# manasakani/DeviceKMC

Hardware: AMD Instinct MI355X
Metric: KMC steps/sec (higher is better)
Workload: dtype f64

## Files before the change

devicekmc_amd/csrc/common.h:

```cpp
#pragma once
#include <hip/hip_runtime.h>
#include <stdint.h>
#include <stdio.h>
#include <string.h>
#include <math.h>
#include "../../include/devicekmc_hip.h"
#include "../../include/devicekmc_hip_debug.h"

enum { DEFECT = 0, OXYGEN_DEFECT = 1, VACANCY = 2, O_EL = 3, Hf_EL = 4, Ni_EL = 5, Ti_EL = 6, Pt_EL = 7, N_EL = 8, NULL_ELEMENT = 9 };
enum { EV_GEN = 0, EV_REC = 1, EV_VDIFF = 2, EV_IDIFF = 3, EV_NULL = 4 };

#define DKMC_KB 8.617333262e-5
#define DKMC_Q 1.60217663e-19
#define DKMC_HBAR 1.054571817e-34
#define DKMC_MAX_LAYERS 5
#define WAVE 64

struct MetalSet { int n; const int *e; };

__device__ __forceinline__ bool is_metal(int el, const MetalSet &ms)
{
    bool r = false;
    for (int t = 0; t < ms.n; ++t) r |= (ms.e[t] == el);
    return r;
}

__device__ __forceinline__ double site_dist(double x1, double y1, double z1, double x2, double y2, double z2,
                                            double laty, double latz, int pbc)
{
    if (pbc) {
        double dx = x1 - x2;
        double fy = (y1 - y2) / laty; fy -= round(fy);
        double fz = (z1 - z2) / latz; fz -= round(fz);
        double dy = fy * laty, dz = fz * latz;
        return sqrt(dx * dx + dy * dy + dz * dz);
    }
    double dx = x2 - x1, dy = y2 - y1, dz = z2 - z1;
    return sqrt(dx * dx + dy * dy + dz * dz);
}

__device__ __forceinline__ double v_solve(double r, int charge, double sigma, double k)
{
    return (double)charge * erfc(r / (sigma * sqrt(2.0))) * k * DKMC_Q / r;
}

template <int OFF> __device__ __forceinline__ int xor_lane_i(int x)
{
    static_assert(OFF == 1 || OFF == 2 || OFF == 4 || OFF == 8 || OFF == 16 || OFF == 32, "xor_lane: power of two below the wave size");
    if constexpr (OFF == 1) return __builtin_amdgcn_update_dpp(0, x, 0xB1, 0xf, 0xf, false);
    else if constexpr (OFF == 2) return __builtin_amdgcn_update_dpp(0, x, 0x4E, 0xf, 0xf, false);
    else if constexpr (OFF == 4) {
        const int t = __builtin_amdgcn_update_dpp(0, x, 0x104, 0xf, 0x5, false);
        return __builtin_amdgcn_update_dpp(t, x, 0x114, 0xf, 0xa, false);
    }
    else if constexpr (OFF == 8) return __builtin_amdgcn_update_dpp(0, x, 0x128, 0xf, 0xf, false);
    else return __shfl_xor(x, OFF, WAVE);
}
template <int OFF> __device__ __forceinline__ double xor_lane(double x)
{
    if constexpr (OFF >= 16) return __shfl_xor(x, OFF, WAVE);
    else return __hiloint2double(xor_lane_i<OFF>(__double2hiint(x)), xor_lane_i<OFF>(__double2loint(x)));
}
template <int W> __device__ __forceinline__ double group_sum(double v)
{
    if constexpr (W >= 64) v += xor_lane<32>(v);
    if constexpr (W >= 32) v += xor_lane<16>(v);
    if constexpr (W >= 16) v += xor_lane<8>(v);
    if constexpr (W >= 8) v += xor_lane<4>(v);
    if constexpr (W >= 4) v += xor_lane<2>(v);
    if constexpr (W >= 2) v += xor_lane<1>(v);
    return v;
}
template <int W> __device__ __forceinline__ int group_sum_i(int v)
{
    if constexpr (W >= 64) v += xor_lane_i<32>(v);
    if constexpr (W >= 32) v += xor_lane_i<16>(v);
    if constexpr (W >= 16) v += xor_lane_i<8>(v);
    if constexpr (W >= 8) v += xor_lane_i<4>(v);
    if constexpr (W >= 4) v += xor_lane_i<2>(v);
    if constexpr (W >= 2) v += xor_lane_i<1>(v);
    return v;
}

__device__ __forceinline__ double wave_sum(double v) { return group_sum<WAVE>(v); }
__device__ __forceinline__ double wave_sum_all(double v) { return group_sum<WAVE>(v); }
__device__ __forceinline__ int wave_sum_all_i(int v) { return group_sum_i<WAVE>(v); }
template <class T> __device__ __forceinline__ T wave_min(T v)
{
#pragma unroll
    for (int off = 32; off > 0; off >>= 1) { const T t = __shfl_xor(v, off, WAVE); v = t < v ? t : v; }
    return v;
}
template <class T> __device__ __forceinline__ T wave_max(T v)
{
#pragma unroll
    for (int off = 32; off > 0; off >>= 1) { const T t = __shfl_xor(v, off, WAVE); v = t > v ? t : v; }
    return v;
}
__device__ __forceinline__ double wave_scan_incl(double v, int lane)
{
#pragma unroll
    for (int off = 1; off < WAVE; off <<= 1) { double t = __shfl_up(v, off, WAVE); if (lane >= off) v += t; }
    return v;
}
__device__ __forceinline__ int wave_scan_incl_i(int v, int lane)
{
#pragma unroll
    for (int off = 1; off < WAVE; off <<= 1) { int t = __shfl_up(v, off, WAVE); if (lane >= off) v += t; }
    return v;
}

template <int NT>
__device__ __forceinline__ double block_sum_all(double v, double *red)
{
    const int lane = threadIdx.x & 63, w = threadIdx.x >> 6;
    v = wave_sum(v);
    __syncthreads();
    if (lane == 0) red[w] = v;
    __syncthreads();
    double s = 0.0;
#pragma unroll
    for (int i = 0; i < NT / 64; ++i) s += red[i];
    return s;
}

__host__ __device__ __forceinline__ unsigned long long dbl_key(double v)
{
    const unsigned long long b = __builtin_bit_cast(unsigned long long, v);
    return (b >> 63) ? ~b : (b | 0x8000000000000000ull);
}
__host__ __device__ __forceinline__ double key_dbl(unsigned long long k)
{
    return __builtin_bit_cast(double, (k >> 63) ? (k & 0x7fffffffffffffffull) : ~k);
}
__device__ __forceinline__ int ld_agent(const int *p) { return __hip_atomic_load(p, __ATOMIC_RELAXED, __HIP_MEMORY_SCOPE_AGENT); }
__device__ __forceinline__ void st_agent(int *p, int v) { __hip_atomic_store(p, v, __ATOMIC_RELAXED, __HIP_MEMORY_SCOPE_AGENT); }
__device__ __forceinline__ int seed_bits(int i, int N, int n_left, int n_right) { return (i < n_left ? 1 : 0) | (i >= N - n_right ? 2 : 0); }
inline void clamp_seeds(int N, int &n_left, int &n_right)
{
    n_left = n_left < 0 ? 0 : (n_left > N ? N : n_left);
    n_right = n_right < 0 ? 0 : (n_right > N ? N : n_right);
}

struct KBlocked {
    int m, R, nb, total, maxwin, maxints;
    long long winsum;
    int *perm;
    int *pcol;
    int4 *blk;
    int form = 1;
    int maxseg = 0;
    long long segsum = 0;
    int4 *seg = nullptr;
    int word_bytes = 4;
};
constexpr int X_POLY_DEFAULT = 8;
struct Engine {
    hipStream_t stream = nullptr;
    int device = 0;
    double cg_tol = 1e-6;
    int current_warm_start = 1;
    int profiling = 0;
    int cb_edge_domain = 0;
    long long tcache_budget = -1;
    double pair_cut = 6.5;
    int pair_form = 0;
    int k_blocked = 1;
    int k_blocked_large = 0;
    int k_window_word_bytes = 4;
    int x_aux = 2;
    int x_slab = 1;
    int k_slab = 1;
    int x_poly = X_POLY_DEFAULT;
    int x_poly_auto = 1;
    int x_poly_rows[2] = {0, 0};
    int x_poly_form = 2;
    int x_poly1_degree = 0;
    int x_poly_form_used = 0, x_poly_products = 0;
    int x_slab_poly = 0;
    int x_aux_warm = 0;
    int x_items_kc = 0;
    int x_apply_form = 0;
    int x_tile_f32 = 1;
    double x_tile_drop = 0.0;
    int x_tile_drop_unit = 0;
    int x_tile_drop_auto = 1;
    long long x_tile_drop_gate = 0;
    double x_tile_drop_used = 0.0;
    int xtl_census_form = 1;
    int x_static_tiles = 2;
    int x_static_gate = 0;
    int x_static_nM = -1;
    int x_static_verify = 0;
    int x_tile_f32_fail_once = 0;
    int x_fold_form = 1;
    int x_fold_poison = 0;
    int x_nmul_form = 1;
    int x_nmul_lane_bytes = 16;
    int x_nmul_window = 2;
    int x_nmul_window_cap = 76 * 1024;
    int x_nmul_window_block = 320;
    int x_block = 16;
    int x_format = 1;
    int current_map = 0;
    int x_iter_hint = 0;
    int event_temperature = 0;
    int event_census = 0;
    int event_census_valid = 0;
    double event_census_info[16] = {0};
    dkmc_stats stats{};
    char err[512] = {0};
    int err_code = 0;
    double E_gen[DKMC_MAX_LAYERS] = {0}, E_rec[DKMC_MAX_LAYERS] = {0}, E_Vdiff[DKMC_MAX_LAYERS] = {0}, E_Odiff[DKMC_MAX_LAYERS] = {0};
    int num_layers = 0;
    static const int NBUF = 192;
    void *buf[NBUF] = {nullptr};
    size_t bufsz[NBUF] = {0};
};

constexpr int X_STATIC_GATE = 32768;
static inline int x_static_rule(int ns, int gate_override) { return ns >= (gate_override > 0 ? gate_override : X_STATIC_GATE) ? 1 : 0; }
Engine &eng();
int dkmc_fail(int code, const char *what, const char *file, int line);
void *scratch(int slot, size_t bytes);
void *scratch_try(int slot, size_t bytes);
static inline int grid_blocks(long long work, int per_block, int cap)
{
    long long b = (work + per_block - 1) / per_block;
    if (b < 1) b = 1;
    if (b > cap) b = cap;
    return (int)b;
}
inline MetalSet load_metals(const int *d_metals, int num_metals) { MetalSet ms; ms.n = num_metals; ms.e = d_metals; return ms; }

#define HIPCHK(x) do { hipError_t e__ = (x); if (e__ != hipSuccess) return dkmc_fail((int)e__, hipGetErrorString(e__), __FILE__, __LINE__); } while (0)
#define KCHK() do { hipError_t e__ = hipGetLastError(); if (e__ != hipSuccess) return dkmc_fail((int)e__, hipGetErrorString(e__), __FILE__, __LINE__); } while (0)

enum {
    S_CG_S = 0, S_CG_R, S_CG_P, S_CG_T, S_CG_PART, S_CG_CTRL, S_CG_RUNS, S_CG_REM, S_CG_NRUNS, S_CG_PS, S_CG_SEGOFF, S_CG_SEGS, S_CG_SEGPART, S_CG_XCHG, S_CG_PARTS,
    S_K_DATA, S_K_RHS,
    S_PW_LIST, S_PW_CNT, S_PW_CELLS, S_PW_PERM, S_PW_LIST2,
    S_EV_PROB, S_EV_ROWSUM, S_EV_G2, S_EV_G3, S_EV_CTRL, S_EV_UNI, S_EV_LOG,
    S_SCAN_TMP, S_SCAN_TMP2, S_SCAN_OFF64, S_SCAN_INTILE,
    S_AT_FLAG, S_AT_SITE, S_AT_OFSITE, S_AT_NEIGH,
    S_X_ROWPTR, S_X_COL, S_X_DATA, S_X_DATA2, S_X_CNT, S_X_SLIST, S_X_SCB, S_X_SFLAG, S_X_RHS, S_X_SRANK,
    S_P_IMACRO, S_HEAT, S_HEAT_A, S_HEAT_B, S_HEAT_Y,
    S_MISC0, S_MISC1, S_MISC2, S_MISC3,
    S_XT_DPOS, S_XT_SNODE_D, S_XT_SNODE_I, S_XT_CMASK, S_XT_ISTILE, S_XT_NSUBC, S_XT_TOFF, S_XT_SOFF, S_XT_TILES, S_XT_NITEMW, S_XT_WRANGE,
    S_XT_ITEMS, S_XT_SPLIT, S_XT_TVAL, S_XT_TVAL32, S_XT_ROWPART, S_XT_COLPART, S_XT_CNT, S_XT_Q,
    S_XT_T_NITEMW, S_XT_T_ITEMS, S_XT_T_SPLIT, S_XT_T_COLPART, S_XT_T_MISC,
    S_XTB_PANELS, S_XTB_QS, S_XTB_ROWPART, S_XTB_COLPART, S_XTB_GRAM, S_XTB_SMALL, S_XTB_XI,
    S_XTB_SLAB_BOX, S_XTB_SLAB_TAB, S_XTB_SLAB_OWNER, S_XTB_SLAB_LISTS, S_XTB_SLAB_SDST, S_XTB_SLAB_FLAG, S_XTB_SLAB_RLISTS, S_XTB_SLAB_GX, S_XTB_SLAB_S1, S_XTB_SLAB_S3, S_XTB_SLAB_R3,
    S_XTB_EMU_Y, S_XTB_EMU_CTRL, S_XTB_YPANEL, S_XTB_PRE_V, S_XTB_PRE_W1, S_XTB_PRE_W2, S_XTB_PRE_Z, S_XTB_PRE_U,
    S_XTB_NPACK_CNT, S_XTB_NPACK_OFF, S_XTB_NPACK_COL, S_XTB_NPACK_W,
    S_XTL_CELLS, S_XTL_TFLAG, S_XTL_TVAL32, S_XTL_TILES, S_XTL_WRANGE, S_XTL_NITEMW, S_XTL_ITEMS, S_XTL_SPLIT,
    S_XT_WLIST, S_XTL_WLIST,
    S_KS_TAB, S_KS_OWNER, S_KS_LISTS, S_KS_FLAG, S_KS_BOX, S_KS_RLISTS, S_KS_XA, S_KS_XB, S_KS_SEND, S_KS_RECV, S_KS_YBUF, S_KS_EMU,
    S_XTB_TEST_RP, S_XTB_TEST_CI, S_XTB_TEST_VAL, S_XTB_TEST_SC, S_XTB_TEST_NSR, S_XTB_TEST_LIST, S_XTB_TEST_IN, S_XTB_TEST_ADD, S_XTB_TEST_OUT,
    S_XTB_TEST_W1, S_XTB_TEST_W2, S_XTB_TEST_QS, S_XTB_TEST_CTRL, S_XTB_TEST_NPCNT, S_XTB_TEST_NPOFF, S_XTB_TEST_NPCOL, S_XTB_TEST_NPW,
    S_P_CMAP,
    S_XTB_ALG_PANELS, S_XTB_ALG_INTS, S_XTB_ALG_GRAM, S_XTB_ALG_QS, S_XTB_ALG_CTRL,
    S_CL_PARENT, S_CL_SUMS, S_CL_POS, S_CL_TABLE, S_CL_CTRL,
    S_EV_NBAD, S_EV_CENSUS_PART, S_EV_CENSUS_INFO,
    S_GAP_SITE, S_GAP_CTRL, S_GAP_CELLS, S_GAP_SORTED, S_GAP_NODES, S_GAP_EDGES,
    S_PT_HOP, S_PT_PRED, S_PT_ROWS, S_PT_CTRL,
    S_TR_HASH, S_TR_COMP, S_TR_SITE, S_TR_ROWS, S_TR_CTRL,
    S_CUT_SITE, S_CUT_TABLE, S_CUT_ROWS, S_CUT_CTRL,
    S_FL_SITE, S_FL_ROWS, S_FL_CTRL,
    S_NSLOTS
};
static_assert(S_NSLOTS <= Engine::NBUF, "scratch slots");

int comm_attached();
int comm_nranks();
int comm_rank();
int comm_allgather_f64(double *buf, size_t count);
int comm_alltoallv_f64(const double *sendbuf, double *recvbuf, const long long *cnt);
int comm_allreduce_sum_f64(double *buf, size_t count);
int comm_agree(int local_rc, const char *what);
int comm_agree_count();
int comm_peer_ready(size_t count);
double *comm_peer_slots(int parity);
void comm_peer_drop();
int comm_peer_exchange(int parity, size_t count, int *ctrl_done, int *ctrl_aborted, int *ctrl_timeout, int stamp);
int comm_bcast0_f64(double *buf, size_t count);

int ev_census_enqueue(int N, int nn, const int *neigh, const int *element, const double *temperature, const double *ev_prob, double **d_info16);

int dkmc_exclusive_scan_i32(const int *d_in, int *d_out, int n, int *d_total);
int dkmc_exclusive_scan_i32_i64(const int *d_in, long long *d_out, int n, long long *d_total);
```

devicekmc_amd/csrc/engine.hip:

```cpp
#include "common.h"
#include <stdlib.h>

int events_upload_layers();
void xstate_reset(const void *key);

static Engine g_engine;
Engine &eng() { return g_engine; }

int dkmc_fail(int code, const char *what, const char *file, int line)
{
    Engine &e = eng();
    snprintf(e.err, sizeof(e.err), "%s (%s:%d)", what, file, line);
    e.err_code = code ? code : -1;
    fprintf(stderr, "devicekmc_hip: %s\n", e.err);
    return e.err_code;
}

void *scratch(int slot, size_t bytes)
{
    Engine &e = eng();
    if (bytes == 0) bytes = 16;
    if (e.bufsz[slot] < bytes) {
        if (e.buf[slot]) { (void)hipStreamSynchronize(e.stream); (void)hipFree(e.buf[slot]); }
        size_t want = bytes + bytes / 8 + 256;
        hipError_t rc = hipMalloc(&e.buf[slot], want);
        if (rc != hipSuccess) {
            char msg[160]; snprintf(msg, sizeof(msg), "hipMalloc(%zu bytes) failed in scratch(slot %d): %s", want, slot, hipGetErrorString(rc));
            dkmc_fail(2, msg, __FILE__, __LINE__); e.buf[slot] = nullptr; e.bufsz[slot] = 0; return nullptr;
        }
        e.bufsz[slot] = want;
    }
    return e.buf[slot];
}

void *scratch_try(int slot, size_t bytes)
{
    Engine &e = eng();
    if (bytes == 0) bytes = 16;
    if (e.bufsz[slot] < bytes) {
        if (e.buf[slot]) { (void)hipStreamSynchronize(e.stream); (void)hipFree(e.buf[slot]); }
        e.buf[slot] = nullptr; e.bufsz[slot] = 0;
        const size_t want = bytes + bytes / 8 + 256;
        if (hipMalloc(&e.buf[slot], want) != hipSuccess) { (void)hipGetLastError(); e.buf[slot] = nullptr; return nullptr; }
        e.bufsz[slot] = want;
    }
    return e.buf[slot];
}

extern "C" {

const char *dkmc_last_error(void) { return eng().err; }
void dkmc_clear_error(void) { eng().err[0] = 0; eng().err_code = 0; }
const dkmc_stats *dkmc_get_stats(void) { return &eng().stats; }
void dkmc_set_cg_tolerance(double tol) { eng().cg_tol = tol; }
void dkmc_set_current_warm_start(int mode) { eng().current_warm_start = mode; }
int dkmc_get_current_warm_start(void) { return eng().current_warm_start; }
void dkmc_set_profiling(int on) { eng().profiling = on; }
void dkmc_set_x_format(int tiled) { eng().x_format = tiled ? 1 : 0; }
int dkmc_get_x_format(void) { return eng().x_format; }
void dkmc_set_current_map(int on) { eng().current_map = on ? 1 : 0; }
int dkmc_get_current_map(void) { return eng().current_map; }
void dkmc_set_tcache_budget(long long bytes) { eng().tcache_budget = bytes; }
void dkmc_set_pair_cutoff(double x_cut) { eng().pair_cut = x_cut > 0.0 ? x_cut : 0.0; }
void dkmc_set_pair_form(int form) { eng().pair_form = form == 1 ? 1 : 0; }
int dkmc_get_pair_form(void) { return eng().pair_form; }
void dkmc_set_k_slab(int on) { eng().k_slab = on ? 1 : 0; }
int dkmc_get_k_slab(void) { return eng().k_slab; }
void dkmc_set_x_aux_warm(int on) { eng().x_aux_warm = on ? 1 : 0; }
int dkmc_get_x_aux_warm(void) { return eng().x_aux_warm; }
void dkmc_set_x_items(int kc) { eng().x_items_kc = kc > 0 ? (kc < 256 ? kc : 256) : 0; }
void dkmc_set_x_poly(int degree) { eng().x_poly = degree < 0 ? 0 : (degree > 16 ? 16 : degree); eng().x_poly_auto = 0; }
int dkmc_get_x_poly(void) { return eng().x_poly; }
void dkmc_set_x_poly_auto(int on) { Engine &e = eng(); e.x_poly_auto = on ? 1 : 0; if (on && e.x_poly <= 0) e.x_poly = X_POLY_DEFAULT; }
int dkmc_get_x_poly_auto(void) { return eng().x_poly_auto; }
void dkmc_set_x_poly_form(int form) { eng().x_poly_form = form == 1 ? 1 : (form == 2 ? 2 : 0); }
int dkmc_get_x_poly_form(void) { return eng().x_poly_form; }
int dkmc_get_x_poly_form_used(void) { return eng().x_poly_form_used; }
int dkmc_get_x_poly_products(void) { return eng().x_poly_products; }
void dkmc_debug_set_x_poly1_degree(int n) { eng().x_poly1_degree = n < 0 ? 0 : (n > 20 ? 20 : n); }
void dkmc_set_x_poly_auto_rows(int n0, int n1) { Engine &e = eng(); e.x_poly_rows[0] = n0 > 0 ? n0 : 0; e.x_poly_rows[1] = n1 > e.x_poly_rows[0] ? n1 : e.x_poly_rows[0]; }
void dkmc_set_x_apply_form(int form) { eng().x_apply_form = form == 1 ? 1 : 0; }
int dkmc_get_x_apply_form(void) { return eng().x_apply_form; }
void dkmc_set_x_tile_f32(int mode) { eng().x_tile_f32 = mode == 0 ? 0 : 1; }
int dkmc_get_x_tile_f32(void) { return eng().x_tile_f32; }
void dkmc_set_x_tile_drop(double theta) { eng().x_tile_drop = theta > 0.0 ? (theta > 1e-4 ? 1e-4 : theta) : 0.0; }
double dkmc_get_x_tile_drop(void) { return eng().x_tile_drop; }
void dkmc_set_x_tile_drop_unit(int unit) { eng().x_tile_drop_unit = unit == 1 ? 1 : 0; }
int dkmc_get_x_tile_drop_unit(void) { return eng().x_tile_drop_unit; }
void dkmc_set_x_tile_drop_auto(int on) { eng().x_tile_drop_auto = on ? 1 : 0; }
int dkmc_get_x_tile_drop_auto(void) { return eng().x_tile_drop_auto; }
void dkmc_set_x_tile_drop_auto_subblocks(long long gate) { eng().x_tile_drop_gate = gate > 0 ? gate : 0; }
double dkmc_get_x_tile_drop_used(void) { return eng().x_tile_drop_used; }
void dkmc_debug_fail_true_residual_once(void) { eng().x_tile_f32_fail_once = 1; }
void dkmc_set_x_fold_form(int form) { eng().x_fold_form = form == 0 ? 0 : 1; }
int dkmc_get_x_fold_form(void) { return eng().x_fold_form; }
void dkmc_debug_poison_fold_cells(int on) { eng().x_fold_poison = on ? 1 : 0; }
void dkmc_set_x_static_tiles(int mode) { eng().x_static_tiles = (mode == 0 || mode == 1) ? mode : 2; }
int dkmc_get_x_static_tiles(void) { return eng().x_static_tiles; }
int dkmc_debug_x_static_verify(int on) { const int was = eng().x_static_verify; eng().x_static_verify = on ? 1 : 0; return was; }
void dkmc_debug_set_x_static_gate(int members) { eng().x_static_gate = members > 0 ? members : 0; }
int dkmc_x_static_rule(int members) { return x_static_rule(members, eng().x_static_gate); }
int dkmc_x_static_strips(int n_metals) { return n_metals > 0 ? n_metals / 256 : 0; }
void dkmc_set_x_nmul_form(int form) { eng().x_nmul_form = form == 0 ? 0 : 1; }
int dkmc_get_x_nmul_form(void) { return eng().x_nmul_form; }
void dkmc_set_x_nmul_lane_bytes(int bytes) { eng().x_nmul_lane_bytes = bytes == 8 ? 8 : 16; }
int dkmc_get_x_nmul_lane_bytes(void) { return eng().x_nmul_lane_bytes; }
void dkmc_set_x_nmul_window(int mode) { eng().x_nmul_window = (mode == 0 || mode == 1) ? mode : 2; }
int dkmc_get_x_nmul_window(void) { return eng().x_nmul_window; }
void dkmc_debug_set_x_nmul_window(int cap_bytes, int block_rows)
{
    Engine &e = eng();
    e.x_nmul_window_cap = cap_bytes < 0 ? 76 * 1024 : (cap_bytes > 76 * 1024 ? 76 * 1024 : cap_bytes);
    e.x_nmul_window_block = (block_rows >= 16 && block_rows <= 1024 && block_rows % 16 == 0) ? block_rows : 320;
}
void dkmc_set_x_slab(int on) { eng().x_slab = on ? 1 : 0; }
int dkmc_get_x_slab(void) { return eng().x_slab; }
void dkmc_set_x_slab_poly(int on) { eng().x_slab_poly = on ? 1 : 0; }
int dkmc_get_x_slab_poly(void) { return eng().x_slab_poly; }
void dkmc_set_x_block(int s) { eng().x_block = s < 1 ? 1 : (s > 16 ? 16 : s); }
int dkmc_get_x_block(void) { return eng().x_block; }
void dkmc_set_x_aux(int mode) { eng().x_aux = mode < 0 ? 0 : (mode > 3 ? 2 : mode); }
int dkmc_get_x_aux(void) { return eng().x_aux; }
void dkmc_set_k_blocked(int on) { eng().k_blocked = on ? 1 : 0; }
int dkmc_get_k_blocked(void) { return eng().k_blocked; }
void dkmc_set_k_blocked_large(int on) { eng().k_blocked_large = on ? 1 : 0; }
int dkmc_get_k_blocked_large(void) { return eng().k_blocked_large; }
void dkmc_set_k_window_word_bytes(int bytes) { eng().k_window_word_bytes = bytes == 2 ? 2 : 4; }
int dkmc_get_k_window_word_bytes(void) { return eng().k_window_word_bytes; }
void dkmc_set_cb_edge_domain(int atoms_only) { eng().cb_edge_domain = atoms_only ? 1 : 0; }

int dkmc_get_gpu_info(char *gpu_string, int capacity, int dev)
{
    hipDeviceProp_t prop;
    HIPCHK(hipSetDevice(dev));
    HIPCHK(hipGetDeviceProperties(&prop, dev));
    snprintf(gpu_string, capacity, "%s", prop.name);
    return 0;
}

int dkmc_set_gpu(int dev) { HIPCHK(hipSetDevice(dev)); eng().device = dev; return 0; }
int dkmc_set_stream(void *s) { eng().stream = (hipStream_t)s; return 0; }
int dkmc_synchronize(void) { HIPCHK(hipStreamSynchronize(eng().stream)); return 0; }

int dkmc_copy_to_const_memory(const double *E_gen, const double *E_rec, const double *E_Vdiff, const double *E_Odiff, int nl)
{
    Engine &e = eng();
    if (nl > DKMC_MAX_LAYERS) return dkmc_fail(3, "more than 5 layers (MAX_NUM_LAYERS, kmc_events.cu:7)", __FILE__, __LINE__);
    e.num_layers = nl;
    for (int i = 0; i < nl; ++i) { e.E_gen[i] = E_gen[i]; e.E_rec[i] = E_rec[i]; e.E_Vdiff[i] = E_Vdiff[i]; e.E_Odiff[i] = E_Odiff[i]; }
    return events_upload_layers();
}

#define ALLOC(field, n, T) HIPCHK(hipMalloc((void **)&buf->field, (size_t)(n) * sizeof(T)))
int dkmc_gpubuf_create(dkmc_gpubuf *buf, int N, int N_atom, int nn, int nmt,
                       const int *h_layer, const double *hx, const double *hy, const double *hz,
                       const int *h_neigh, const int *h_metals, double freq, double sigma, double k, const double *h_lattice)
{
    memset(buf, 0, sizeof(*buf));
    buf->N_ = N; buf->N_atom_ = N_atom; buf->nn_ = nn; buf->num_metal_types_ = nmt;
    ALLOC(site_layer, N, int); ALLOC(site_element, N, int); ALLOC(metal_types, nmt > 0 ? nmt : 1, int);
    ALLOC(site_x, N, double); ALLOC(site_y, N, double); ALLOC(site_z, N, double);
    ALLOC(site_power, N, double); ALLOC(site_CB_edge, N, double);
    ALLOC(site_potential_boundary, N, double); ALLOC(site_potential_charge, N, double);
    ALLOC(site_temperature, N, double); ALLOC(site_charge, N, int);
    ALLOC(neigh_idx, (size_t)N * nn, int);
    ALLOC(T_bg, 1, double); ALLOC(sigma, 1, double); ALLOC(k, 1, double); ALLOC(lattice, 3, double); ALLOC(freq, 1, double);
    ALLOC(atom_element, N, int); ALLOC(atom_x, N, double); ALLOC(atom_y, N, double); ALLOC(atom_z, N, double);
    ALLOC(atom_power, N, double); ALLOC(atom_CB_edge, N, double); ALLOC(atom_charge, N, int);
    ALLOC(atom_virtual_potentials, N_atom + 2, double);
    HIPCHK(hipMemset(buf->atom_virtual_potentials, 0, (size_t)(N_atom + 2) * sizeof(double)));
    HIPCHK(hipMemset(buf->site_power, 0, (size_t)N * sizeof(double)));
    HIPCHK(hipMemcpy(buf->site_layer, h_layer, (size_t)N * sizeof(int), hipMemcpyHostToDevice));
    HIPCHK(hipMemcpy(buf->site_x, hx, (size_t)N * sizeof(double), hipMemcpyHostToDevice));
    HIPCHK(hipMemcpy(buf->site_y, hy, (size_t)N * sizeof(double), hipMemcpyHostToDevice));
    HIPCHK(hipMemcpy(buf->site_z, hz, (size_t)N * sizeof(double), hipMemcpyHostToDevice));
    if (nmt > 0) HIPCHK(hipMemcpy(buf->metal_types, h_metals, (size_t)nmt * sizeof(int), hipMemcpyHostToDevice));
    HIPCHK(hipMemcpy(buf->sigma, &sigma, sizeof(double), hipMemcpyHostToDevice));
    HIPCHK(hipMemcpy(buf->k, &k, sizeof(double), hipMemcpyHostToDevice));
    HIPCHK(hipMemcpy(buf->freq, &freq, sizeof(double), hipMemcpyHostToDevice));
    HIPCHK(hipMemcpy(buf->lattice, h_lattice, 3 * sizeof(double), hipMemcpyHostToDevice));
    HIPCHK(hipMemcpy(buf->neigh_idx, h_neigh, (size_t)N * nn * sizeof(int), hipMemcpyHostToDevice));
    return 0;
}
#undef ALLOC

int dkmc_gpubuf_free(dkmc_gpubuf *b)
{
    xstate_reset(b->site_x);
    void *ptrs[] = { b->site_charge, b->site_power, b->site_potential_boundary, b->site_potential_charge, b->site_temperature,
                     b->site_CB_edge, b->T_bg, b->atom_power, b->atom_CB_edge, b->atom_virtual_potentials, b->atom_charge,
                     b->site_element, b->atom_element, b->site_x, b->site_y, b->site_z, b->atom_x, b->atom_y, b->atom_z,
                     b->metal_types, b->sigma, b->k, b->lattice, b->freq, b->neigh_idx, b->site_layer,
                     b->Device_row_ptr_d, b->Device_col_indices_d, b->contact_left_row_ptr, b->contact_left_col_indices,
                     b->contact_right_row_ptr, b->contact_right_col_indices };
    for (void *p : ptrs) if (p) (void)hipFree(p);
    memset(b, 0, sizeof(*b));
    return 0;
}

int dkmc_gpubuf_sync_host_to_gpu(dkmc_gpubuf *b, const int *el, const int *q, const double *pw, const double *cb,
                                 const double *pb, const double *pc, const double *T, const double *acb, double T_bg)
{
    const size_t N = b->N_;
    HIPCHK(hipStreamSynchronize(eng().stream));
    HIPCHK(hipMemcpy(b->site_element, el, N * sizeof(int), hipMemcpyHostToDevice));
    HIPCHK(hipMemcpy(b->site_charge, q, N * sizeof(int), hipMemcpyHostToDevice));
    HIPCHK(hipMemcpy(b->site_power, pw, N * sizeof(double), hipMemcpyHostToDevice));
    HIPCHK(hipMemcpy(b->site_CB_edge, cb, N * sizeof(double), hipMemcpyHostToDevice));
    HIPCHK(hipMemcpy(b->site_potential_boundary, pb, N * sizeof(double), hipMemcpyHostToDevice));
    HIPCHK(hipMemcpy(b->site_potential_charge, pc, N * sizeof(double), hipMemcpyHostToDevice));
    HIPCHK(hipMemcpy(b->site_temperature, T, N * sizeof(double), hipMemcpyHostToDevice));
    if (acb) HIPCHK(hipMemcpy(b->atom_CB_edge, acb, (size_t)b->N_atom_ * sizeof(double), hipMemcpyHostToDevice));
    HIPCHK(hipMemcpy(b->T_bg, &T_bg, sizeof(double), hipMemcpyHostToDevice));
    return 0;
}

int dkmc_gpubuf_sync_gpu_to_host(const dkmc_gpubuf *b, int *el, int *q, double *pw, double *cb,
                                 double *pb, double *pc, double *T, double *acb, double *T_bg)
{
    const size_t N = b->N_;
    HIPCHK(hipStreamSynchronize(eng().stream));
    HIPCHK(hipMemcpy(el, b->site_element, N * sizeof(int), hipMemcpyDeviceToHost));
    HIPCHK(hipMemcpy(q, b->site_charge, N * sizeof(int), hipMemcpyDeviceToHost));
    HIPCHK(hipMemcpy(pw, b->site_power, N * sizeof(double), hipMemcpyDeviceToHost));
    HIPCHK(hipMemcpy(cb, b->site_CB_edge, N * sizeof(double), hipMemcpyDeviceToHost));
    HIPCHK(hipMemcpy(pb, b->site_potential_boundary, N * sizeof(double), hipMemcpyDeviceToHost));
    HIPCHK(hipMemcpy(pc, b->site_potential_charge, N * sizeof(double), hipMemcpyDeviceToHost));
    HIPCHK(hipMemcpy(T, b->site_temperature, N * sizeof(double), hipMemcpyDeviceToHost));
    if (acb) HIPCHK(hipMemcpy(acb, b->atom_CB_edge, (size_t)b->N_atom_ * sizeof(double), hipMemcpyDeviceToHost));
    HIPCHK(hipMemcpy(T_bg, b->T_bg, sizeof(double), hipMemcpyDeviceToHost));
    return 0;
// ... 23 lines not shown
```

devicekmc_amd/csrc/xtb.hip:

```cpp
#include "xtiles.h"
#include "slab.h"
#include <hip/hip_ext.h>
#include <algorithm>
#include <functional>
#include <type_traits>
#include <vector>

#define XB_SP 16
#define XB_MAXPOLY 16
#define XB_MAXPOLY1 20
#define XB_DSPLIT 8
#define XB_NG 6
typedef double dbl4 __attribute__((ext_vector_type(4)));
#define XB_MFMA(a, b, c) __builtin_amdgcn_mfma_f64_16x16x4f64((a), (b), (c), 0, 0, 0)
#define XB_MFMA4(a, b, c) __builtin_amdgcn_mfma_f64_4x4x4f64((a), (b), (c), 0, 0, 0)

__device__ __forceinline__ double xtb_aux(int row, int col)
{
    unsigned long long h = (unsigned long long)row * 0x9E3779B97F4A7C15ull + (unsigned long long)col * 0xC2B2AE3D27D4EB4Full + 12345ull;
    h ^= h >> 29; h *= 0xBF58476D1CE4E5B9ull; h ^= h >> 32;
    return (double)(h >> 11) * (1.0 / 4503599627370496.0) - 1.0;
}
struct XbAux { double lo[3], hi[3]; int k[16][3]; unsigned long long mm[6]; int hs, pad_; };
__device__ __forceinline__ double xtb_rhs(const double *__restrict__ b, int row, int v, int s, const XbAux *__restrict__ aux = nullptr,
// ... 854 lines not shown
    double gdiag = (threadIdx.x < 16 && (int)threadIdx.x < s && diag_ok) ? Gg[threadIdx.x][threadIdx.x] : 1.0;
    XB_WSYNC();
    const bool cholg = xtb_chol(Gg, s);
    const bool okg = diag_ok;
    if (!cholg) {
#pragma unroll
        for (int u = 0; u < 4; ++u) { const int e = (int)threadIdx.x + 64 * u, i = e >> 4, j = e & 15; Gg[i][j] = (i == j) ? 1.0 : 0.0; }
        XB_WSYNC();
        if (threadIdx.x < 16) Gg[threadIdx.x][threadIdx.x] = sqrt(gdiag);
        XB_WSYNC();
    }
    if (threadIdx.x < 16) {
        const int jj = threadIdx.x;
        double w[16];
#pragma unroll
        for (int r = 15; r >= 0; --r) {
            double a = (r == jj) ? 1.0 : 0.0;
#pragma unroll
            for (int p = r + 1; p < 16; ++p) a -= Gg[p][r] * w[p];
            w[r] = a / Gg[r][r];
        }
#pragma unroll
        for (int r = 0; r < 16; ++r) Wm[r][jj] = (r < s && jj < s && okg) ? w[r] : 0.0;
    }
    XB_WSYNC();
    xtb_mm(Vm, Bm, Wm, false, 1.0, nullptr, 0.0);
    xtb_mm(Tm, Cm, Wm, false, -1.0, nullptr, 0.0);
#pragma unroll
    for (int u = 0; u < 4; ++u) {
        const int e = (int)threadIdx.x + 64 * u, i = e >> 4, j = e & 15;
        mats[0 * 256 + e] = Cm[i][j]; mats[1 * 256 + e] = -Wm[i][j]; mats[2 * 256 + e] = Vm[i][j]; mats[3 * 256 + e] = Tm[i][j];
    }
    if (threadIdx.x == 0) {
        ctrl->rr[(it + 1) & 1] = rr_new; ctrl->rr[it & 1] = rr_new;
        ctrl->iters = it + 1;
        if (!okg) ctrl->pad[0] = 2;
        else if (!cholg) ctrl->pad[1] += 1;
        if (stop || !okg) { if (ctrl->sharded) ctrl->done_local = 1; else ctrl->done = it + 2; }
    }
}

__global__ __launch_bounds__(XT_NT) void k_xtb_step(int m, int it, const double *__restrict__ mats, double *__restrict__ y0, double *__restrict__ R,
                                                    double *__restrict__ P, const double *__restrict__ T, const double *__restrict__ sc,
                                                    const int *__restrict__ nsrank, double *__restrict__ QS, const XCtrl *ctrl,
                                                    const int *__restrict__ rowlist = nullptr, double *__restrict__ Ypanel = nullptr)
{
    __shared__ int sdone;
    if (threadIdx.x == 0) { const int d = ctrl->done; sdone = d != 0 && it + 1 >= d; }
    __syncthreads();
    if (sdone) return;
    const int lane = threadIdx.x & 63, a = lane & 15, b = lane >> 4;
    const int wv = threadIdx.x >> 6;
    double cB[4], m1B[4], m2B[4], m3B[4], c0[4];
#pragma unroll
    for (int kk = 0; kk < 4; ++kk) {
        const int o = (4 * kk + b) * 16 + a;
        cB[kk] = mats[o]; m1B[kk] = mats[256 + o]; m2B[kk] = mats[512 + o]; m3B[kk] = mats[768 + o];
        c0[kk] = mats[(4 * kk + b) * 16];
    }
    const int ngroups = (m + 15) / 16;
    for (int g = (int)blockIdx.x * 4 + wv; g < ngroups; g += (int)gridDim.x * 4) {
        const int row0 = 16 * g;
        double pa[4], ta[4], ra[4];
        const bool oka = row0 + a < m;
        const int rowa = oka ? (rowlist ? rowlist[row0 + a] : row0 + a) : 0;
        const size_t oa = (size_t)rowa * XB_SP + b;
#pragma unroll
        for (int kk = 0; kk < 4; ++kk) { pa[kk] = oka ? P[oa + 4 * kk] : 0.0; ta[kk] = oka ? T[oa + 4 * kk] : 0.0; ra[kk] = oka ? R[oa + 4 * kk] : 0.0; }
        dbl4 rN, pN = (dbl4)(0.0), yN = (dbl4)(0.0);
        const double yold = (b == 0 && oka) ? y0[rowa] : 0.0;
        int rowu[4];
#pragma unroll
        for (int u = 0; u < 4; ++u) {
            const int li = row0 + b + 4 * u;
            rowu[u] = li < m ? (rowlist ? rowlist[li] : li) : -1;
            rN[u] = rowu[u] >= 0 ? R[(size_t)rowu[u] * XB_SP + a] : 0.0;
            if (Ypanel) yN[u] = rowu[u] >= 0 ? Ypanel[(size_t)rowu[u] * XB_SP + a] : 0.0;
        }
        double yacc = (pa[0] * c0[0] + pa[1] * c0[1]) + (pa[2] * c0[2] + pa[3] * c0[3]);
        yacc += __shfl_xor(yacc, 16, WAVE); yacc += __shfl_xor(yacc, 32, WAVE);
        if (b == 0 && oka) y0[rowa] = yold + yacc;
#pragma unroll
        for (int kk = 0; kk < 4; ++kk) {
            rN = XB_MFMA(ta[kk], cB[kk], rN);
            pN = XB_MFMA(ra[kk], m1B[kk], pN); pN = XB_MFMA(ta[kk], m3B[kk], pN); pN = XB_MFMA(pa[kk], m2B[kk], pN);
            if (Ypanel) yN = XB_MFMA(pa[kk], cB[kk], yN);
        }
#pragma unroll
        for (int u = 0; u < 4; ++u) {
            const int row = rowu[u];
            if (row >= 0) {
                const size_t o = (size_t)row * XB_SP + a;
                R[o] = rN[u]; P[o] = pN[u];
                if (Ypanel) Ypanel[o] = yN[u];
                const int sr = nsrank[row];
                if (sr >= 0) QS[xtb_qs_pos(sr, a)] = sc[row] * pN[u];
            }
        }
    }
}
__global__ __launch_bounds__(XT_NT) void k_xtb_gram1(int m, const double *__restrict__ Pt, const double *__restrict__ Pi, const double *__restrict__ Q,
                                                     const double *__restrict__ U, const double *__restrict__ Rt, const double *__restrict__ Z,
                                                     double *__restrict__ gpart, const XCtrl *ctrl)
{
    __shared__ double lg[4][XB_NG / 2][4][64];
    if (ctrl->done) return;
    const int v = threadIdx.x & 15, wv = threadIdx.x >> 6, lane = threadIdx.x & 63;
    dbl4 G[XB_NG];
#pragma unroll
    for (int g = 0; g < XB_NG; ++g) G[g] = (dbl4)(0.0);
    const int chunk = ((m + (int)gridDim.x - 1) / (int)gridDim.x + 3) & ~3;
    const long long i0l = (long long)blockIdx.x * chunk;
    const int i0 = (int)(i0l < m ? i0l : m), i1 = (int)(i0l + chunk < m ? i0l + chunk : m);
    for (int r0 = i0 + 4 * wv; r0 < i1; r0 += 64) {
        double pv[4], iv[4], qv[4], uv[4], rv[4], zv[4]; bool in[4];
#pragma unroll
        for (int u = 0; u < 4; ++u) {
            const int row = r0 + 16 * u + (lane >> 4);
            in[u] = row < i1;
            const size_t o = (size_t)(in[u] ? row : i0) * XB_SP + v;
            pv[u] = Pt[o]; iv[u] = Pi[o]; qv[u] = Q[o]; uv[u] = U[o]; rv[u] = Rt[o]; zv[u] = Z[o];
        }
#pragma unroll
        for (int u = 0; u < 4; ++u) {
            if (r0 + 16 * u >= i1) break;
            const double p_ = in[u] ? pv[u] : 0.0, i_ = in[u] ? iv[u] : 0.0, q_ = in[u] ? qv[u] : 0.0, u_ = in[u] ? uv[u] : 0.0, r_ = in[u] ? rv[u] : 0.0,
                         z_ = in[u] ? zv[u] : 0.0;
            G[0] = XB_MFMA(p_, q_, G[0]); G[1] = XB_MFMA(p_, r_, G[1]); G[2] = XB_MFMA(q_, z_, G[2]);
            G[3] = XB_MFMA(q_, u_, G[3]); G[4] = XB_MFMA(r_, z_, G[4]); G[5] = XB_MFMA(p_, i_, G[5]);
        }
    }
#pragma unroll
    for (int h = 0; h < 2; ++h) {
        __syncthreads();
#pragma unroll
        for (int g = 0; g < XB_NG / 2; ++g)
#pragma unroll
            for (int u = 0; u < 4; ++u) lg[wv][g][u][lane] = G[h * (XB_NG / 2) + g][u];
        __syncthreads();
        for (int e = threadIdx.x; e < (XB_NG / 2) * 256; e += XT_NT) {
            const int g = e >> 8, x = e & 255, u = x >> 6, l = x & 63;
            double a = (lg[0][g][u][l] + lg[1][g][u][l]) + (lg[2][g][u][l] + lg[3][g][u][l]);
            if (h == 1) {
                const int xt = ((x & 15) << 4) | (x >> 4), ut = xt >> 6, lt = xt & 63;
                a = 0.5 * (a + ((lg[0][g][ut][lt] + lg[1][g][ut][lt]) + (lg[2][g][ut][lt] + lg[3][g][ut][lt])));
            }
            gpart[(size_t)blockIdx.x * (XB_NG * 256) + h * (XB_NG / 2) * 256 + e] = a;
        }
    }
}
__global__ __launch_bounds__(XT_NT) void k_xtb_step1(int m, int it, const double *__restrict__ mats, double *__restrict__ y0, double *__restrict__ Rt,
                                                     double *__restrict__ Z, double *__restrict__ Pt, double *__restrict__ Pi, const double *__restrict__ Q,
                                                     const double *__restrict__ U, const double *__restrict__ sc, const int *__restrict__ nsrank,
                                                     double *__restrict__ QS, const XCtrl *ctrl)
{
    __shared__ int sdone;
    if (threadIdx.x == 0) { const int d = ctrl->done; sdone = d != 0 && it + 1 >= d; }
    __syncthreads();
    if (sdone) return;
    const int lane = threadIdx.x & 63, a = lane & 15, b = lane >> 4;
    const int wv = threadIdx.x >> 6;
    double cB[4], m1B[4], m2B[4], m3B[4], c0[4];
#pragma unroll
    for (int kk = 0; kk < 4; ++kk) {
        const int o = (4 * kk + b) * 16 + a;
        cB[kk] = mats[o]; m1B[kk] = mats[256 + o]; m2B[kk] = mats[512 + o]; m3B[kk] = mats[768 + o];
        c0[kk] = mats[(4 * kk + b) * 16];
    }
    const int ngroups = (m + 15) / 16;
    for (int g = (int)blockIdx.x * 4 + wv; g < ngroups; g += (int)gridDim.x * 4) {
        const int row0 = 16 * g;
        double pa[4], ia[4], qa[4], ua[4], ra[4], za[4];
        const bool oka = row0 + a < m;
        const int rowa = oka ? row0 + a : 0;
        const size_t oa = (size_t)rowa * XB_SP + b;
#pragma unroll
        for (int kk = 0; kk < 4; ++kk) {
            pa[kk] = oka ? Pt[oa + 4 * kk] : 0.0; ia[kk] = oka ? Pi[oa + 4 * kk] : 0.0; qa[kk] = oka ? Q[oa + 4 * kk] : 0.0;
            ua[kk] = oka ? U[oa + 4 * kk] : 0.0; ra[kk] = oka ? Rt[oa + 4 * kk] : 0.0; za[kk] = oka ? Z[oa + 4 * kk] : 0.0;
        }
        dbl4 rN, zN, pN = (dbl4)(0.0), iN = (dbl4)(0.0);
        const double yold = (b == 0 && oka) ? y0[rowa] : 0.0;
        int rowu[4];
#pragma unroll
        for (int u = 0; u < 4; ++u) {
            const int li = row0 + b + 4 * u;
            rowu[u] = li < m ? li : -1;
            rN[u] = rowu[u] >= 0 ? Rt[(size_t)rowu[u] * XB_SP + a] : 0.0;
            zN[u] = rowu[u] >= 0 ? Z[(size_t)rowu[u] * XB_SP + a] : 0.0;
        }
        double yacc = (pa[0] * c0[0] + pa[1] * c0[1]) + (pa[2] * c0[2] + pa[3] * c0[3]);
        yacc += __shfl_xor(yacc, 16, WAVE); yacc += __shfl_xor(yacc, 32, WAVE);
        if (b == 0 && oka) y0[rowa] = yold + yacc;
#pragma unroll
        for (int kk = 0; kk < 4; ++kk) {
            rN = XB_MFMA(qa[kk], cB[kk], rN); zN = XB_MFMA(ua[kk], cB[kk], zN);
            pN = XB_MFMA(za[kk], m1B[kk], pN); pN = XB_MFMA(ua[kk], m3B[kk], pN); pN = XB_MFMA(pa[kk], m2B[kk], pN);
            iN = XB_MFMA(ra[kk], m1B[kk], iN); iN = XB_MFMA(qa[kk], m3B[kk], iN); iN = XB_MFMA(ia[kk], m2B[kk], iN);
        }
#pragma unroll
        for (int u = 0; u < 4; ++u) {
            const int row = rowu[u];
            if (row >= 0) {
                const size_t o = (size_t)row * XB_SP + a;
                Rt[o] = rN[u]; Z[o] = zN[u]; Pt[o] = pN[u]; Pi[o] = iN[u];
                const int sr = nsrank[row];
                if (sr >= 0) QS[xtb_qs_pos(sr, a)] = sc[row] * pN[u];
            }
        }
    }
}
__global__ void k_xtb_init(int m, const double *__restrict__ y, const double *__restrict__ sc, const int *__restrict__ nsrank,
                           double *__restrict__ y0, double *__restrict__ P, double *__restrict__ QS,
                           const double *__restrict__ yaux = nullptr, int hs = 16, int s = 16, double *__restrict__ Ypanel = nullptr)
{
    const int i = blockIdx.x * blockDim.x + threadIdx.x;
    if (i >= m * XB_SP) return;
    const int row = i >> 4, v = i & 15;
    double yv = 0.0;
    if (v == 0) yv = y[row];
    else if (yaux && v >= hs && v < s) yv = yaux[i] / sc[row];
    P[i] = yv;
    if (Ypanel) Ypanel[i] = yv;
    if (v == 0) y0[row] = yv;
    const int sr = nsrank[row];
    if (sr >= 0) QS[xtb_qs_pos(sr, v)] = sc[row] * yv;
}
__global__ void k_xtb_yaux_out(int n, const int *__restrict__ rowlist, const double *__restrict__ Ypanel, const double *__restrict__ sc, double *__restrict__ yaux)
{
    const int i = blockIdx.x * blockDim.x + threadIdx.x;
    if (i >= n * XB_SP) return;
    const int row = rowlist ? rowlist[i >> 4] : (i >> 4), v = i & 15;
    yaux[(size_t)row * XB_SP + v] = Ypanel[(size_t)row * XB_SP + v] * sc[row];
}
__global__ void k_xtb_zero(long long n, double *__restrict__ p)
{
    const long long i = (long long)blockIdx.x * blockDim.x + threadIdx.x;
    if (i < n) p[i] = 0.0;
}

static SideStream g_xb_side;

int g_xtb_fault_iter = -1;

static int xtb_aux_split(int mode, double tol2, bool warm, int s)
{
    if (mode == 0) return 1;
    if (mode == 1 || mode == 3) return 16;
    if (!(tol2 >= 1e-16)) return 1;
    return warm ? std::max(1, s / 2) : 16;
}
static int xtb_box_modes(XbAux *d, XbAux h0, const XtbArgs &A, int x_only, hipStream_t st)
{
    for (int k = 0; k < 3; ++k) { h0.mm[2 * k] = ~0ull; h0.mm[2 * k + 1] = 0ull; }
    HIPCHK(hipMemcpyAsync(d, &h0, sizeof(XbAux), hipMemcpyHostToDevice, st));
    hipLaunchKernelGGL(k_xtb_box, dim3(std::min((A.m - 2 + 255) / 256, 256)), dim3(256), 0, st, A.m - 2, A.ax, A.ay, A.az, d);
    hipLaunchKernelGGL(k_xtb_modes, dim3(1), dim3(512), 0, st, d, x_only);
    return 0;
}
static int xtb_aux_setup(const XtbArgs &A, XbAux **aux, int *hs)
{
    Engine &e = eng();
    *hs = xtb_aux_split(e.x_aux, A.tol2, A.yaux != nullptr, A.s);
    *aux = nullptr;
    if (A.ax && A.ay && A.az && A.m > 2 && *hs > 1) {
        *aux = (XbAux *)scratch(S_XTB_XI, sizeof(XbAux));
        if (!*aux) return e.err_code;
        XbAux h0{};
        h0.hs = *hs;
        if (int rc = xtb_box_modes(*aux, h0, A, e.x_aux == 3 ? 1 : 0, e.stream)) return rc;
    }
    e.stats.xb_aux = *aux ? (*hs >= A.s ? 1 : 2) : 0;
    return 0;
}
struct XbApplyArgs { int n; const XItem *items; const XTile *tiles; int sub_base; const double *tval; const double *QS; int nW; double *rowpartB, *colpartB; const XCtrl *ctrl; const float *tval32 = nullptr; };
template <int NTL, int NG, int V>
static void xtb_apply_v(const XbApplyArgs &a, hipStream_t st, hipEvent_t e0, hipEvent_t e1)
{
    hipExtLaunchKernelGGL((k_xtb_apply<NTL, NG, V>), dim3((a.n + 3) / 4), dim3(XT_NT), 0, st, e0, e1, 0, a.n, a.items, a.tiles, a.sub_base, a.tval, a.QS, a.nW,
                          a.rowpartB, a.colpartB, a.ctrl);
}
template <int NTL, int NG>
static void xtb_apply_f32(const XbApplyArgs &a, hipStream_t st, hipEvent_t e0, hipEvent_t e1)
{
    hipExtLaunchKernelGGL((k_xtb_apply<NTL, NG, 0, float>), dim3((a.n + 3) / 4), dim3(XT_NT), 0, st, e0, e1, 0, a.n, a.items, a.tiles, a.sub_base, a.tval32, a.QS, a.nW,
                          a.rowpartB, a.colpartB, a.ctrl);
}
template <int NTL, int NG>
static void xtb_apply_ng(const XbApplyArgs &a, int variant, hipStream_t st, hipEvent_t e0, hipEvent_t e1)
{
#ifdef DKMC_MEASURE_VARIANTS
#define XB_V(v_) if (variant == (v_)) return xtb_apply_v<NTL, NG, v_>(a, st, e0, e1);
    if constexpr (NTL == 1 && NG == 2) { XB_V(1) XB_V(2) }
    if constexpr (NTL == 1 && NG == 4) { XB_V(1) XB_V(2) XB_V(3) XB_V(4) XB_V(7) XB_V(10) XB_V(12) }
#undef XB_V
#else
    (void)variant;
#endif
    if (a.tval32) return xtb_apply_f32<NTL, NG>(a, st, e0, e1);
    if (eng().x_apply_form == 1) xtb_apply_v<NTL, NG, 8>(a, st, e0, e1);
    else xtb_apply_v<NTL, NG, 0>(a, st, e0, e1);
}
static void xtb_apply(const XbApplyArgs &a, bool ntl, int so, int variant, hipStream_t st, hipEvent_t e0 = nullptr, hipEvent_t e1 = nullptr)
{
    static void (*const ng[2][4])(const XbApplyArgs &, int, hipStream_t, hipEvent_t, hipEvent_t) = {
        {xtb_apply_ng<0, 1>, xtb_apply_ng<0, 2>, xtb_apply_ng<0, 3>, xtb_apply_ng<0, 4>}, {xtb_apply_ng<1, 1>, xtb_apply_ng<1, 2>, xtb_apply_ng<1, 3>, xtb_apply_ng<1, 4>}};
    ng[ntl ? 1 : 0][so == 4 ? 0 : (so == 8 ? 1 : (so == 12 ? 2 : 3))](a, variant, st, e0, e1);
}
template <int SH, int NF, class... Args>
static void xtb_rows_launch(bool init, int ng, hipStream_t st, hipEvent_t e0, hipEvent_t e1, Args... a)
{
    if (init) hipLaunchKernelGGL((k_xtb_rows<1, SH, NF>), dim3(ng), dim3(XT_NT), 0, st, a...);
    else hipExtLaunchKernelGGL((k_xtb_rows<0, SH, NF>), dim3(ng), dim3(XT_NT), 0, st, e0, e1, 0, a...);
}
static const char *const XTB_NO_CONVERGENCE = "block-CG: no convergence after 200000 iterations";
static int xtb_finish(const XCtrl &h, bool hint, bool again, bool prof, int *iters_out, double *rr_out)
{
    Engine &e = eng();
    if (hint) e.x_iter_hint = h.iters;
    if (iters_out) *iters_out = h.iters;
    if (rr_out) *rr_out = h.rr[h.iters & 1];
    if (prof) g_loop_events.to_stats(e.stats, false);
    if (h.pad[0]) return DKMC_XTB_BREAKDOWN;
    return again ? DKMC_XTB_AGAIN : 0;
}
static int xtb_cg_body(const XtbArgs &A, int *iters_out, double *rr_out, bool *peer_used, const XbNPack *np, bool f32, XLive *lv);
static int xtb_cg_slab(const XtbArgs &A, int nr, int me0, const XShare *emu_shares, int time_rank, int *iters_out, double *rr_out);
template <class Body>
static int xtb_reenter(int rc, double rr0, int *iters_out, double *rr_out, Body body)
{
    for (int round = 1; rc == DKMC_XTB_AGAIN && round < 6; ++round) {
        int it2 = 0; double rr1 = 0.0;
        rc = body(&it2, &rr1);
        if (iters_out) *iters_out += it2;
        if (rc == DKMC_XTB_AGAIN && !(rr1 < 0.25 * rr0)) rc = 0;
        rr0 = rr1;
    }
    if (rc == DKMC_XTB_AGAIN) rc = 0;
    if (rr_out) *rr_out = rr0;
    return rc;
}
int xtb_cg(const XtbArgs &A, int *iters_out, double *rr_out)
{
    bool peer_used = false;
    double rr0 = 0.0;
    if (A.sharded && eng().x_slab && comm_nranks() > 1 && comm_nranks() <= XS_MAXR && A.ay && A.az) {
        const int nr = comm_nranks(), me = comm_rank();
        const int rc = xtb_cg_slab(A, nr, me, nullptr, -1, iters_out, &rr0);
        return xtb_reenter(rc, rr0, iters_out, rr_out, [&](int *it, double *rr) { return xtb_cg_slab(A, nr, me, nullptr, -1, it, rr); });
    }
    XbNPack npk{};
    const bool packed = !A.sharded && A.m > 2 && A.ns > 0 && eng().x_poly > 0 && eng().x_nmul_form == 1;
    if (packed) { if (int rcp = xtb_npack(A, A.m, nullptr, scratch, 0, &npk)) return rcp; }
    const XbNPack *np = packed ? &npk : nullptr;
    Engine &e = eng();
    const bool f32 = e.x_tile_f32 != 0 && A.tval32 != nullptr && !A.sharded && A.m > 2 && A.ns > 0 && e.x_poly > 0 && A.tol2 >= 1e-16;
    if (f32) e.stats.x_tile_stream = 1; else if (e.stats.x_tile_stream == 1) e.stats.x_tile_stream = 0;
    e.stats.x_tile_f64_rounds = f32 ? 0 : 1;
    XLive *lv = nullptr;
    const double theta = e.x_tile_drop > 0.0 ? e.x_tile_drop : (e.x_tile_drop_auto && A.warm ? xtl_drop_rule(A.stored_subblocks, e.x_tile_drop_gate) : 0.0);
    e.x_tile_drop_used = 0.0;
    if (f32 && theta > 0.0 && A.item_n > 0 && A.tiles == g_xb.tiles && A.tval32 == g_xb.tval32) {
        if (int rcl = xt_live_build(theta, e.x_tile_drop_unit, A.sS, &g_xlive)) return rcl;
        if (g_xlive.state == 1) { lv = &g_xlive; e.x_tile_drop_used = theta; }
    }
    int rc = xtb_cg_body(A, iters_out, &rr0, &peer_used, np, f32, lv);
    rc = xtb_reenter(rc, rr0, iters_out, rr_out, [&](int *it, double *rr) { ++e.stats.x_tile_f64_rounds; return xtb_cg_body(A, it, rr, &peer_used, np, false, nullptr); });
    if (rc != 0 && rc != DKMC_XTB_BREAKDOWN && peer_used) comm_peer_drop();
    return rc;
}
static int xtb_cg_body(const XtbArgs &A, int *iters_out, double *rr_out, bool *peer_used, const XbNPack *np, bool f32, XLive *lv)
{
    Engine &e = eng(); hipStream_t st = e.stream;
    const int m = A.m, s = A.s, so = 4 * ((s + 3) / 4);
    const size_t pan = (size_t)m * XB_SP;
    const long long ncell = (long long)A.nK * A.nW;
    const int ng = std::max(128, std::min(A.nK, 4096));
    double *panels = (double *)scratch(S_XTB_PANELS, (pan * 3 + m + 16) * 8);
    double *QS = (double *)scratch(S_XTB_QS, (size_t)A.ns_pad * XB_SP * 8);
    double *rowpartB = (double *)scratch(S_XTB_ROWPART, (size_t)(ncell + 1) * XT_R * so * 8);
    const int nrec = std::max(A.nrecords, lv ? lv->nrecords : 0);
    double *colpartB = (double *)scratch(S_XTB_COLPART, (size_t)(nrec + 1) * XT_C * so * 8);
    double *gpart = (double *)scratch(S_XTB_GRAM, (size_t)ng * XB_NG * 256 * 8);
    double *small = (double *)scratch(S_XTB_SMALL, (size_t)(4 * 256 + 2 * XB_DSPLIT * XB_SP + XB_NG * 256) * 8);
    if (!panels || !QS || !rowpartB || !colpartB || !gpart || !small) return e.err_code;
    double *R = panels, *P = panels + pan, *T = panels + 2 * pan, *y0 = panels + 3 * pan;
    double *mats = small, *drvpart = small + 4 * 256, *gfin = drvpart + 2 * XB_DSPLIT * XB_SP;
    const int pd = xtb_poly_degree(e, A);
    e.stats.xb_poly_used = pd;
    const bool one = pd > 0 && xtb_poly_one(e);
    const int pn = one ? xtb_poly1_degree(e, pd) : pd;
    e.x_poly_form_used = one ? 1 : 0; e.x_poly_products = one ? pn : 2 * pd;
    double *Vp = nullptr, *W1 = nullptr, *W2 = nullptr, *Zp = nullptr, *bz = nullptr, *Up = nullptr;
    if (pd > 0) {
        Vp = (double *)scratch(S_XTB_PRE_V, (pan + m + 16) * 8); W1 = (double *)scratch(S_XTB_PRE_W1, pan * 8); W2 = (double *)scratch(S_XTB_PRE_W2, pan * 8);
        Zp = (double *)scratch(S_XTB_PRE_Z, pan * 8);
        if (!Vp || !W1 || !W2 || !Zp) return e.err_code;
        bz = Vp + pan;
        HIPCHK(hipMemsetAsync(bz, 0, (size_t)(m + 16) * 8, st));
        if (one) {
            Up = (double *)scratch(S_XTB_PRE_U, pan * 8);
            if (!Up) return e.err_code;
            HIPCHK(hipMemsetAsync(Vp, 0, pan * 8, st));
            HIPCHK(hipMemsetAsync(Up, 0, pan * 8, st));
        }
    }
    double pc[XB_MAXPOLY1 + 1] = {1.0}, qmin = 1.0;
    if (one) xtb_poly1_coeffs(pn, pc, &qmin); else xtb_poly_coeffs(pd, pc);
    const double tol2_loop = one ? A.tol2 * qmin : (pd > 0 ? A.tol2 / 2.25 : A.tol2);
    HIPCHK(hipMemsetAsync(QS, 0, (size_t)A.ns_pad * XB_SP * 8, st));
    const bool listf = e.x_fold_form == 1 && pd > 0 && !A.sharded && A.wlist != nullptr && (!lv || lv->wlist != nullptr);
    const int so1 = listf ? 4 : so;
    if (!listf) HIPCHK(hipMemsetAsync(rowpartB, 0, (size_t)(ncell + 1) * XT_R * so * 8, st));
    else if (e.x_fold_poison) HIPCHK(hipMemsetAsync(rowpartB, 0xff, (size_t)(ncell + 1) * XT_R * so * 8, st));
    HIPCHK(hipMemsetAsync(colpartB, 0, (size_t)(nrec + 1) * XT_C * so * 8, st));
    HIPCHK(hipMemsetAsync(A.ctrl, 0, sizeof(XCtrl), st));
    const bool sharded = A.sharded;
    const int nr = sharded ? comm_nranks() : 1, me = sharded ? comm_rank() : 0;
    double *xbuf = nullptr;
    const size_t xcount = (size_t)A.ns * so + 2;
    const bool peer = sharded && comm_peer_ready(xcount);
    *peer_used = peer;
    int xpar = 0;
    if (sharded) {
        if (!peer) { xbuf = (double *)scratch(S_CG_XCHG, xcount * nr * 8); if (!xbuf) return e.err_code; }
        hipLaunchKernelGGL(k_xtb_set_sharded, dim3(1), dim3(1), 0, st, A.ctrl);
    }
    const bool keep_aux = A.yaux != nullptr && pd == 0;
    double *Ypanel = keep_aux ? (double *)scratch(S_XTB_YPANEL, pan * 8) : nullptr;
    if (keep_aux && !Ypanel) return e.err_code;
    XbAux *aux = nullptr; int hs = 1;
    if (int rc = xtb_aux_setup(A, &aux, &hs)) return rc;
    int local_fail = 0;
    hipLaunchKernelGGL(k_xtb_init, dim3((unsigned)((pan + 255) / 256)), dim3(256), 0, st, m, (const double *)A.y, A.sc, A.nsrank, y0, P, QS,
                       (const double *)((keep_aux && A.yaux_valid) ? A.yaux : nullptr), hs, s, Ypanel);
    struct XbView { const XItem *items; int item_n; const XTile *tiles; const int2 *wrange; const int *nitem_w; const int *wlist; };
    const XbView full{A.items, A.item_n, A.tiles, A.wrange, A.nitem_w, listf ? A.wlist : nullptr};
    const XbView live = lv ? XbView{lv->items, lv->item_n, lv->tiles, lv->wrange, lv->nitem_w, listf ? lv->wlist : nullptr} : full;
    const XbView *vw = &full;
    const int ntb = (A.item_n + 3) / 4;
    const int nnb = 2 * XB_DSPLIT + (std::max(m - 2, 1) + 15) / 16;
    const int gs = grid_blocks((m + 15) / 16, 4, 2048);
    const bool prof = e.profiling != 0;
    if (prof) if (int prc = g_loop_events.begin(EventSampler::LONG | EventSampler::SHORT)) return prc;
    const bool side = sharded && m > 20000 && ntb > 0 && side_stream_init(g_xb_side) == 0;
    const float *t32 = nullptr;
    auto product = [&](hipEvent_t e0, hipEvent_t e1, int sw) {
        int sl = 0;
        if (side) {
            SideStream &S = g_xb_side; sl = (int)(S.seq++ % SideStream::RING);
            (void)hipEventRecord(S.a[sl], st);
            (void)hipStreamWaitEvent(S.st, S.a[sl], 0);
            hipLaunchKernelGGL(k_xtb_neigh, dim3(nnb), dim3(XT_NT), 0, S.st, m, A.rp, A.ci, A.val, (const double *)P, A.sc, A.nsrank, (const XCtrl *)A.ctrl, T, drvpart);
            (void)hipEventRecord(S.b[sl], S.st);
        }
        if (vw->item_n > 0) xtb_apply({vw->item_n, vw->items, vw->tiles, A.sub_base, A.tval, QS, A.nW, rowpartB, colpartB, A.ctrl, t32}, A.nt_loads, sw, 0, st, e0, e1);
        if (side) (void)hipStreamWaitEvent(st, g_xb_side.b[sl], 0);
        else hipLaunchKernelGGL(k_xtb_neigh, dim3(nnb), dim3(XT_NT), 0, st, m, A.rp, A.ci, A.val, (const double *)P, A.sc, A.nsrank, (const XCtrl *)A.ctrl, T, drvpart);
    };
    const XbNRank nk{m, nullptr, np, QS, A.ctrl};
    auto applyL = [&](double *src, double *dst, bool qs) {
        xtb_applyL(st, A, pn, pc, src, dst, W1, W2, qs, [](int, double *) { return 0; }, [&](bool, auto f) { f(nk, [](double *p) { return p; }); return 0; });
    };
    auto fold_rows = [&](double *Tt, int sw) {
        hipLaunchKernelGGL(k_xtb_fold_rows, dim3(std::max(ng, 1)), dim3(XT_NT), 0, st, A.ns, A.nK, A.nW, sw, vw->wrange, vw->wlist, vw->nitem_w, (const double *)rowpartB, (const double *)colpartB,
                           A.srow, A.sS, A.sc, (const double *)drvpart, Tt, (const XCtrl *)A.ctrl);
    };
    auto product_pre = [&](hipEvent_t e0, hipEvent_t e1) {
        applyL(P, Vp, true);
        double *Pk = P, *Tk = T; P = Vp; T = Zp;
        t32 = f32 ? A.tval32 : nullptr;
        if (lv) { vw = &live; t32 = lv->tval32; }
        product(e0, e1, so);
        t32 = nullptr;
        P = Pk; T = Tk;
        fold_rows(Zp, so);
        vw = &full;
        applyL(Zp, T, false);
    };
    auto product_one = [&](hipEvent_t e0, hipEvent_t e1) {
        t32 = f32 ? A.tval32 : nullptr;
        if (lv) { vw = &live; t32 = lv->tval32; }
        product(e0, e1, so);
        t32 = nullptr;
        fold_rows(T, so);
        vw = &full;
        applyL(T, Up, false);
    };
    auto gram_one = [&](hipEvent_t e2, hipEvent_t e3) {
        hipExtLaunchKernelGGL(k_xtb_gram1, dim3(ng), dim3(XT_NT), 0, st, e2, e3, 0, m, (const double *)P, (const double *)Vp, (const double *)T, (const double *)Up,
                              (const double *)R, (const double *)Zp, gpart, (const XCtrl *)A.ctrl);
    };
    auto step = [&](int it) {
        if (one) hipLaunchKernelGGL(k_xtb_step1, dim3(gs), dim3(XT_NT), 0, st, m, it, (const double *)mats, y0, R, Zp, P, Vp, (const double *)T, (const double *)Up, A.sc,
                                    A.nsrank, QS, (const XCtrl *)A.ctrl);
        else hipLaunchKernelGGL(k_xtb_step, dim3(gs), dim3(XT_NT), 0, st, m, it, (const double *)mats, y0, R, P, (const double *)T, A.sc, A.nsrank, QS, (const XCtrl *)A.ctrl,
                                (const int *)nullptr, Ypanel);
    };
    const double *bsel = A.b;
#define XB_ROWS_ARGS(IT_) A.ns, A.nK, A.nW, m, s, so, (lv && !init ? live : full).wrange, (lv && !init ? live : full).nitem_w, (const double *)rowpartB, (const double *)colpartB, A.srow, A.sS, A.nsrank, A.sc, \
                     (const double *)drvpart, T, (const double *)P, R, bsel, gpart, A.ctrl, (const double *)xbuf, IT_, nr, (const XbAux *)aux, A.ax, A.ay, A.az
    auto rows = [&](bool init, int itn, hipEvent_t e2, hipEvent_t e3) -> int {
        if (sharded) {
            if (peer) { xbuf = comm_peer_slots(xpar); }
            hipLaunchKernelGGL(k_xtb_fold_local, dim3(std::max(A.nK, 1)), dim3(XT_NT), 0, st, A.ns, A.nK, A.nW, so, A.wrange, A.nitem_w, (const double *)rowpartB,
                               (const double *)colpartB, xbuf + me * xcount, (const XCtrl *)A.ctrl, 1, A.w_lo, A.w_hi);
            if (hipGetLastError() != hipSuccess || local_fail) {
                if (!local_fail) local_fail = dkmc_fail(92, "block-CG: launch failed between two collectives", __FILE__, __LINE__);
                hipLaunchKernelGGL(k_xtb_abort_word, dim3(1), dim3(1), 0, st, A.ctrl, xbuf + me * xcount, (size_t)A.ns * so + 1);
            }
            if (peer) {
                if (int rcx = comm_peer_exchange(xpar, xcount, &A.ctrl->done, &A.ctrl->aborted, &A.ctrl->xchg_timeout, itn + 2)) return rcx;
                xpar ^= 1;
            } else if (int rcx = comm_allgather_f64(xbuf, xcount)) return rcx;
            xtb_rows_launch<1, 0>(init, ng, st, e2, e3, XB_ROWS_ARGS(itn));
        } else if (pd > 0) xtb_rows_launch<0, 1>(init, ng, st, e2, e3, XB_ROWS_ARGS(itn));
        else xtb_rows_launch<0, 0>(init, ng, st, e2, e3, XB_ROWS_ARGS(itn));
        return 0;
    };
    product(nullptr, nullptr, so1);
    if (one) {
        fold_rows(T, so1);
        if (lv && !listf) xt_live_zero_dead(*lv, rowpartB, so);
        if (int rcx = rows(true, -1, nullptr, nullptr)) return rcx;
        applyL(R, Zp, false);
        gram_one(nullptr, nullptr);
    } else if (pd > 0) {
        fold_rows(T, so1);
        if (lv && !listf) xt_live_zero_dead(*lv, rowpartB, so);
        hipLaunchKernelGGL(k_xtb_pre_resid, dim3((unsigned)((pan + 255) / 256)), dim3(256), 0, st, m, (const double *)T, A.b, Zp);
        applyL(Zp, T, false);
        bsel = bz;
        HIPCHK(hipMemsetAsync(y0, 0, (size_t)m * 8, st));
    }
    if (!one) if (int rcx = rows(true, -1, nullptr, nullptr)) return rcx;
    hipLaunchKernelGGL(k_xtb_gred, dim3(XB_NG * 16), dim3(XT_NT), 0, st, ng, (const double *)gpart, gfin, (const XCtrl *)A.ctrl);
    hipLaunchKernelGGL(k_xtb_small, dim3(1), dim3(256), 0, st, -1, s, (const double *)gfin, mats, A.ctrl, tol2_loop);
    hipLaunchKernelGGL(k_xtb_zero, dim3((unsigned)((pan + 255) / 256)), dim3(256), 0, st, (long long)pan, P);
    step(-1);
    KCHK();
    XCtrl h{};
    if (int rcx = cg_poll_loop(A.ctrl, h, LaunchPlan::hinted_three_quarters(e.x_iter_hint), st, XTB_NO_CONVERGENCE, prof && ntb > 0 && live.item_n > 0 ? &g_loop_events : nullptr,
                               [&](int it, const hipEvent_t *ev) -> int {
            if (sharded && g_xtb_fault_iter >= 0 && it >= g_xtb_fault_iter) { g_xtb_fault_iter = -1; local_fail = dkmc_fail(91, "injected fault (block-CG iteration)", __FILE__, __LINE__); }
            if (one) { product_one(ev[0], ev[1]); gram_one(ev[2], ev[3]); }
            else {
                if (pd > 0) product_pre(ev[0], ev[1]);
                else product(ev[0], ev[1], so);
                if (int rcx = rows(false, it, ev[2], ev[3])) return rcx;
            }
            hipLaunchKernelGGL(k_xtb_gred, dim3(XB_NG * 16), dim3(XT_NT), 0, st, ng, (const double *)gpart, gfin, (const XCtrl *)A.ctrl);
            hipLaunchKernelGGL(k_xtb_small, dim3(1), dim3(256), 0, st, it, s, (const double *)gfin, mats, A.ctrl, tol2_loop);
            step(it);
            return 0;
        })) return rcx;
#undef XB_ROWS_ARGS
    if (lv) lv->info[7] = h.iters;
    if (local_fail) return local_fail;
    if (h.xchg_timeout) return dkmc_fail(48, "block-CG: the peer-write exchange timed out waiting for a peer's slot", __FILE__, __LINE__);
    if (h.aborted) return dkmc_fail(46, "a peer rank aborted the sharded current solve", __FILE__, __LINE__);
    if (e.err_code) return e.err_code;
    bool again = false;
    if (pd > 0) {
        HIPCHK(hipMemsetAsync(A.ctrl, 0, sizeof(XCtrl), st));
        if (one) HIPCHK(hipMemcpyAsync(A.y, y0, (size_t)m * 8, hipMemcpyDeviceToDevice, st));
        else {
            hipLaunchKernelGGL(k_xtb_pre_col0, dim3((unsigned)((pan + 255) / 256)), dim3(256), 0, st, m, (const double *)y0, Zp);
            applyL(Zp, Vp, false);
            hipLaunchKernelGGL(k_xtb_pre_add, dim3((m + 255) / 256), dim3(256), 0, st, m, (const double *)Vp, A.y);
        }
        if (!h.pad[0]) {
            hipLaunchKernelGGL(k_xtb_pre_col0, dim3((unsigned)((pan + 255) / 256)), dim3(256), 0, st, m, (const double *)A.y, P);
            hipLaunchKernelGGL(k_xtb_qs_from, dim3((unsigned)((pan + 255) / 256)), dim3(256), 0, st, m, (const double *)P, A.sc, A.nsrank, QS, (const XCtrl *)A.ctrl);
            product(nullptr, nullptr, so1);
            fold_rows(T, so1);
            const int nrp = std::min(XB_RR_MAXPART, (m + 1023) / 1024);
            hipLaunchKernelGGL(k_xtb_pre_rr_part, dim3(nrp), dim3(256), 0, st, m, (const double *)T, A.b, gpart);
            hipLaunchKernelGGL(k_xtb_pre_rr, dim3(1), dim3(256), 0, st, nrp, (const double *)gpart, bz + m);
            double rr_true = 0.0;
            HIPCHK(hipMemcpyAsync(&rr_true, bz + m, 8, hipMemcpyDeviceToHost, st));
            HIPCHK(hipStreamSynchronize(st));
            h.rr[h.iters & 1] = rr_true;
            again = rr_true > A.tol2;
            if (e.x_tile_f32_fail_once) { e.x_tile_f32_fail_once = 0; again = true; }
        }
    } else
    HIPCHK(hipMemcpyAsync(A.y, y0, (size_t)m * 8, hipMemcpyDeviceToDevice, st));
    if (keep_aux) hipLaunchKernelGGL(k_xtb_yaux_out, dim3((unsigned)((pan + 255) / 256)), dim3(256), 0, st, m, (const int *)nullptr, (const double *)Ypanel, A.sc, A.yaux);
    return xtb_finish(h, true, again, prof, iters_out, rr_out);
}

#include "xtb_slab.inc"
int xtb_cg_slab_emulate(const XtbArgs &A, int nr, const XShare *shares, int time_rank, int sweep_cap, int *iters_out, double *rr_out, double *times_us, long long *xdoubles)
{
    g_slab_sweep_cap = sweep_cap;
    double rr0 = 0.0;
    int rc = xtb_cg_slab(A, nr, 0, shares, time_rank, iters_out, &rr0);
    const double nmul_us = g_slab_last.nmul_us;
    if (sweep_cap > 0) { if (rc == DKMC_XTB_AGAIN) rc = 0; if (rr_out) *rr_out = rr0; }
    else rc = xtb_reenter(rc, rr0, iters_out, rr_out, [&](int *it, double *rr) { return xtb_cg_slab(A, nr, 0, shares, -1, it, rr); });
    g_slab_last.nmul_us = nmul_us;
    g_slab_sweep_cap = 0;
    if (times_us) for (int c = 0; c < 8; ++c) times_us[c] = g_slab_times.us[c];
    if (xdoubles) for (int c = 0; c < 3; ++c) xdoubles[c] = g_slab_xbytes[c];
    return rc;
}
extern "C" int dkmc_xtb_slab_last(int *exchanges_per_sweep, long long *halo_doubles_per_exchange, double *nmul_us)
{
    if (exchanges_per_sweep) *exchanges_per_sweep = g_slab_last.exchanges;
    if (halo_doubles_per_exchange) *halo_doubles_per_exchange = g_slab_last.halo_doubles;
    if (nmul_us) *nmul_us = g_slab_last.nmul_us;
    return 0;
}

__global__ void k_xtb_test_panel(int ns, double *__restrict__ QS)
{
    const int i = blockIdx.x * blockDim.x + threadIdx.x;
    if (i >= ns * XB_SP) return;
    const int r = i >> 4, v = i & 15;
    QS[xtb_qs_pos(r, v)] = 0.25 + (double)((((unsigned)r * 2654435761u) ^ ((unsigned)v * 40503u)) >> 20) / 4096.0 + 0.125 * v;
}
__global__ void k_xtb_test_column(int ns, int v, const double *__restrict__ QS, double *__restrict__ vS)
{
    const int r = blockIdx.x * blockDim.x + threadIdx.x;
    if (r < ns) vS[r] = QS[xtb_qs_pos(r, v)];
}
__global__ void k_xtb_test_compare(int ns, int v, const int *__restrict__ srow, const double *__restrict__ T, const double *__restrict__ ref, double *__restrict__ out)
{
    const int r = blockIdx.x * blockDim.x + threadIdx.x;
    if (r >= ns) return;
    const double a = T[(size_t)srow[r] * XB_SP + v], b = ref[r];
    atomicMax(reinterpret_cast<unsigned long long *>(out), (unsigned long long)__double_as_longlong(fabs(a - b)));
    atomicMax(reinterpret_cast<unsigned long long *>(out + 1), (unsigned long long)__double_as_longlong(fabs(b)));
}
int xt_tile_sums_mv(const double *vS, double *out);
extern "C" int dkmc_xtb_check_product(int width, double *max_abs_diff, double *max_abs)
{
    Engine &e = eng(); hipStream_t st = e.stream; const XTState &X = g_xt;
    if (!X.valid || comm_attached() || X.tile_n != X.ntiles || X.ns <= 0) return dkmc_fail(13, "xtb_check_product: needs the X of a single-GPU solve", __FILE__, __LINE__);
    const int m = X.Nsub, ns = X.ns, s = std::max(2, std::min(width, 16)), so = 4 * ((s + 3) / 4);
    const size_t pan = (size_t)m * XB_SP;
    const long long ncell = (long long)X.nK * X.nW;
    const int nrec = X.nitems >> X.rec_shift, ng = 64;
    double *panels = (double *)scratch(S_XTB_PANELS, (pan * 3 + m + 16) * 8);
    double *QS = (double *)scratch(S_XTB_QS, (size_t)X.ns_pad * XB_SP * 8);
    double *rowpartB = (double *)scratch(S_XTB_ROWPART, (size_t)(ncell + 1) * XT_R * so * 8);
    double *colpartB = (double *)scratch(S_XTB_COLPART, (size_t)(nrec + 1) * XT_C * so * 8);
    double *gpart = (double *)scratch(S_XTB_GRAM, (size_t)4096 * XB_NG * 256 * 8);
    double *small = (double *)scratch(S_XTB_SMALL, (size_t)(4 * 256 + 2 * XB_DSPLIT * XB_SP + XB_NG * 256) * 8);
    double *tmp = (double *)scratch(S_XT_T_MISC, (size_t)4 * X.ns_pad * 8);
    XCtrl *ctrl = (XCtrl *)scratch(S_MISC2, 256);
    double *sS = (double *)e.buf[S_CG_PS], *sc = (double *)e.buf[S_CG_S], *rhs = (double *)e.buf[S_X_RHS];
    if (!panels || !QS || !rowpartB || !colpartB || !gpart || !small || !tmp || !ctrl || !sS || !sc || !rhs) return e.err_code ? e.err_code : dkmc_fail(13, "xtb_check_product: no solver state", __FILE__, __LINE__);
    sS += X.ns_pad;
    double *T = panels + 2 * pan, *R = panels, *P = panels + pan, *drvpart = small + 4 * 256;
    double *vS = tmp, *ref = tmp + X.ns_pad, *res = tmp + 2 * (size_t)X.ns_pad;
    HIPCHK(hipMemsetAsync(tmp, 0, (size_t)4 * X.ns_pad * 8, st));
    HIPCHK(hipMemsetAsync(QS, 0, (size_t)X.ns_pad * XB_SP * 8, st));
    HIPCHK(hipMemsetAsync(panels, 0, (pan * 3 + m + 16) * 8, st));
    HIPCHK(hipMemsetAsync(small, 0, (size_t)(4 * 256 + 2 * XB_DSPLIT * XB_SP) * 8, st));
    HIPCHK(hipMemsetAsync(rowpartB, 0, (size_t)(ncell + 1) * XT_R * so * 8, st));
    HIPCHK(hipMemsetAsync(colpartB, 0, (size_t)(nrec + 1) * XT_C * so * 8, st));
    HIPCHK(hipMemsetAsync(ctrl, 0, sizeof(XCtrl), st));
    hipLaunchKernelGGL(k_xtb_test_panel, dim3((ns * XB_SP + 255) / 256), dim3(256), 0, st, ns, QS);
    const XbApplyArgs xa{X.item_n, (const XItem *)g_xb.items + X.item_lo, (const XTile *)g_xb.tiles, (int)X.sub_base, (const double *)g_xb.tval, QS, X.nW, rowpartB,
                         colpartB, ctrl};
    if (xa.n > 0) xtb_apply(xa, true, so, 0, st);
    hipLaunchKernelGGL((k_xtb_rows<1, 0>), dim3(ng), dim3(XT_NT), 0, st, ns, X.nK, X.nW, m, s, so, (const int2 *)g_xb.wrange, (const int *)g_xb.nitem_w, (const double *)rowpartB,
                       (const double *)colpartB, (const int *)g_xb.srow, (const double *)sS, (const int *)g_xb.nsrank, (const double *)sc, (const double *)drvpart, T,
                       (const double *)P, R, (const double *)rhs, gpart, ctrl, (const double *)nullptr, -1, 1, (const XbAux *)nullptr, (const double *)nullptr, (const double *)nullptr, (const double *)nullptr);
    KCHK();
    const int gb = (ns + 255) / 256;
    for (int v = 0; v < so; ++v) {
        hipLaunchKernelGGL(k_xtb_test_column, dim3(gb), dim3(256), 0, st, ns, v, (const double *)QS, vS);
        int rc = xt_tile_sums_mv(vS, ref); if (rc) return rc;
        hipLaunchKernelGGL(k_xt_vec_mul, dim3(gb), dim3(256), 0, st, ns, ref, (const double *)sS);
        hipLaunchKernelGGL(k_xtb_test_compare, dim3(gb), dim3(256), 0, st, ns, v, (const int *)g_xb.srow, (const double *)T, (const double *)ref, res);
    }
    double h[2] = {0, 0};
    HIPCHK(hipMemcpyAsync(h, res, 16, hipMemcpyDeviceToHost, st));
    HIPCHK(hipStreamSynchronize(st));
    if (max_abs_diff) *max_abs_diff = h[0];
    if (max_abs) *max_abs = h[1];
    return e.err_code;
}

#define XTB_ALG_MAXROWS (1 << 21)
static_assert(sizeof(dkmc_xtb_ctrl) == sizeof(XCtrl) && offsetof(dkmc_xtb_ctrl, pad) == offsetof(XCtrl, pad) && offsetof(dkmc_xtb_ctrl, done) == offsetof(XCtrl, done),
              "dkmc_xtb_ctrl mirrors XCtrl");
static size_t xtb_alg_up(size_t bytes) { return (bytes + 255) & ~(size_t)255; }
static bool xtb_alg_sranks(int m, const int *nsrank, int ns, std::vector<int> *srow)
{
    if (ns < 0 || ns > m) return false;
    std::vector<int> sr((size_t)ns, -1);
    for (int i = 0; i < m; ++i) {
        const int r = nsrank[i];
        if (r < -1 || r >= ns) return false;
        if (r >= 0) { if (sr[r] >= 0) return false; sr[r] = i; }
    }
    for (int r = 0; r < ns; ++r) if (sr[r] < 0) return false;
    if (srow) srow->swap(sr);
    return true;
}
__global__ void k_xtb_test_qs_encode(int ns, const double *__restrict__ in, double *__restrict__ QS)
{
    const int i = blockIdx.x * blockDim.x + threadIdx.x;
    if (i < ns * XB_SP) QS[xtb_qs_pos(i >> 4, i & 15)] = in[i];
}
extern "C" int dkmc_xtb_test_gram(int m, const double *P, const double *T, const double *R, const int *nsrank, int ns, int ng, int done_word, double *gfin,
                                  dkmc_xtb_ctrl *ctrl_out)
{
    Engine &e = eng(); hipStream_t st = e.stream;
    if (m < 1 || m > XTB_ALG_MAXROWS || !P || !T || !R || !nsrank || ng < 1 || ng > 4096 || !gfin) return dkmc_fail(13, "xtb_test_gram: bad arguments", __FILE__, __LINE__);
    std::vector<int> srow;
    if (!xtb_alg_sranks(m, nsrank, ns, &srow)) return dkmc_fail(13, "xtb_test_gram: bad S ranks", __FILE__, __LINE__);
    const int nK = (ns + XT_R - 1) / XT_R, nW = std::max(1, (nK + XT_C / XT_R - 1) / (XT_C / XT_R));
    const size_t pan = (size_t)m * XB_SP * 8, pan_up = xtb_alg_up(pan);
    const size_t b_nsr = xtb_alg_up((size_t)m * 4), b_srow = xtb_alg_up((size_t)std::max(ns, 1) * 4), b_wr = xtb_alg_up((size_t)std::max(nK, 1) * sizeof(int2));
    const size_t b_nit = xtb_alg_up((size_t)(2 * (nW + 2) + 1) * 4);
    const size_t b_gpart = (size_t)ng * XB_NG * 256 * 8;
    char *panels = (char *)scratch(S_XTB_ALG_PANELS, 3 * pan_up);
    char *ints = (char *)scratch(S_XTB_ALG_INTS, b_nsr + b_srow + b_wr + b_nit);
    char *gram = (char *)scratch(S_XTB_ALG_GRAM, b_gpart + (size_t)XB_NG * 256 * 8);
    XCtrl *ctrl = (XCtrl *)scratch(S_XTB_ALG_CTRL, sizeof(XCtrl));
    if (!panels || !ints || !gram || !ctrl) return e.err_code;
    double *dP = (double *)panels, *dT = (double *)(panels + pan_up), *dR = (double *)(panels + 2 * pan_up);
    int *dnsr = (int *)ints, *dsrow = (int *)(ints + b_nsr);
    int2 *dwr = (int2 *)(ints + b_nsr + b_srow);
    int *dnit = (int *)(ints + b_nsr + b_srow + b_wr);
    double *gpart = (double *)gram, *dgfin = (double *)(gram + b_gpart);
    XCtrl h{}; h.done = done_word;
    HIPCHK(hipMemcpyAsync(dP, P, pan, hipMemcpyHostToDevice, st));
    HIPCHK(hipMemcpyAsync(dT, T, pan, hipMemcpyHostToDevice, st));
    HIPCHK(hipMemcpyAsync(dR, R, pan, hipMemcpyHostToDevice, st));
    HIPCHK(hipMemcpyAsync(dnsr, nsrank, (size_t)m * 4, hipMemcpyHostToDevice, st));
    if (ns > 0) HIPCHK(hipMemcpyAsync(dsrow, srow.data(), (size_t)ns * 4, hipMemcpyHostToDevice, st));
    HIPCHK(hipMemsetAsync(dwr, 0, b_wr + b_nit, st));
    HIPCHK(hipMemsetAsync(gpart, 0xff, b_gpart, st));
    HIPCHK(hipMemcpyAsync(dgfin, gfin, (size_t)XB_NG * 256 * 8, hipMemcpyHostToDevice, st));
    HIPCHK(hipMemcpyAsync(ctrl, &h, sizeof(XCtrl), hipMemcpyHostToDevice, st));
    HIPCHK(hipStreamSynchronize(st));
    xtb_rows_launch<0, 1>(false, ng, st, nullptr, nullptr, ns, nK, nW, m, 16, 16, (const int2 *)dwr, (const int *)dnit, (const double *)nullptr, (const double *)nullptr,
                          (const int *)dsrow, (const double *)nullptr, (const int *)dnsr, (const double *)nullptr, (const double *)nullptr, dT, (const double *)dP, dR,
                          (const double *)nullptr, gpart, ctrl, (const double *)nullptr, 0, 1, (const XbAux *)nullptr, (const double *)nullptr, (const double *)nullptr,
                          (const double *)nullptr);
    hipLaunchKernelGGL(k_xtb_gred, dim3(XB_NG * 16), dim3(XT_NT), 0, st, ng, (const double *)gpart, dgfin, (const XCtrl *)ctrl);
    KCHK();
    HIPCHK(hipMemcpyAsync(gfin, dgfin, (size_t)XB_NG * 256 * 8, hipMemcpyDeviceToHost, st));
    HIPCHK(hipMemcpyAsync(&h, ctrl, sizeof(XCtrl), hipMemcpyDeviceToHost, st));
    HIPCHK(hipStreamSynchronize(st));
    if (ctrl_out) memcpy(ctrl_out, &h, sizeof(XCtrl));
    return e.err_code;
}
extern "C" int dkmc_xtb_test_small(int it, int s, int nrg, const double *gblocks, double tol2, const dkmc_xtb_ctrl *ctrl_in, double *mats, dkmc_xtb_ctrl *ctrl_out)
{
    Engine &e = eng(); hipStream_t st = e.stream;
    if (it < -1 || it > 0x3fffffff || s < 1 || s > XB_SP || nrg < 1 || nrg > 64 || !gblocks || !ctrl_in || !mats || !ctrl_out)
        return dkmc_fail(13, "xtb_test_small: bad arguments", __FILE__, __LINE__);
    const size_t gstr = (size_t)XB_NG * 256 + 2, b_g = xtb_alg_up((size_t)nrg * gstr * 8);
    char *gram = (char *)scratch(S_XTB_ALG_GRAM, b_g + 4 * 256 * 8);
    XCtrl *ctrl = (XCtrl *)scratch(S_XTB_ALG_CTRL, sizeof(XCtrl));
    if (!gram || !ctrl) return e.err_code;
    double *dg = (double *)gram, *dmats = (double *)(gram + b_g);
    HIPCHK(hipMemcpyAsync(dg, gblocks, (size_t)nrg * gstr * 8, hipMemcpyHostToDevice, st));
    HIPCHK(hipMemcpyAsync(dmats, mats, 4 * 256 * 8, hipMemcpyHostToDevice, st));
    HIPCHK(hipMemcpyAsync(ctrl, ctrl_in, sizeof(XCtrl), hipMemcpyHostToDevice, st));
    hipLaunchKernelGGL(k_xtb_small, dim3(1), dim3(256), 0, st, it, s, (const double *)dg, dmats, ctrl, tol2, nrg, (int)gstr);
    KCHK();
    HIPCHK(hipMemcpyAsync(mats, dmats, 4 * 256 * 8, hipMemcpyDeviceToHost, st));
    HIPCHK(hipMemcpyAsync(ctrl_out, ctrl, sizeof(XCtrl), hipMemcpyDeviceToHost, st));
    HIPCHK(hipStreamSynchronize(st));
    return e.err_code;
}
extern "C" int dkmc_xtb_test_step(int m, int it, const double *mats, int done_word, double *y0, double *R, double *P, const double *T, const double *sc,
                                  const int *nsrank, int ns, const int *rowlist, int nlist, double *Ypanel, double *qs)
{
    Engine &e = eng(); hipStream_t st = e.stream;
    if (m < 1 || m > XTB_ALG_MAXROWS || it < -1 || it > 0x3fffffff || !mats || !y0 || !R || !P || !T || !sc || !nsrank || (ns > 0 && !qs))
        return dkmc_fail(13, "xtb_test_step: bad arguments", __FILE__, __LINE__);
    if (!xtb_alg_sranks(m, nsrank, ns, nullptr)) return dkmc_fail(13, "xtb_test_step: bad S ranks", __FILE__, __LINE__);
    if (rowlist) {
        if (nlist < 1 || nlist > m) return dkmc_fail(13, "xtb_test_step: bad row list", __FILE__, __LINE__);
        std::vector<char> seen((size_t)m, 0);
        for (int i = 0; i < nlist; ++i) {
            if (rowlist[i] < 0 || rowlist[i] >= m || seen[rowlist[i]]) return dkmc_fail(13, "xtb_test_step: bad row list", __FILE__, __LINE__);
            seen[rowlist[i]] = 1;
        }
    }
    const int n = rowlist ? nlist : m;
    const size_t pan = (size_t)m * XB_SP * 8, pan_up = xtb_alg_up(pan), vec_up = xtb_alg_up((size_t)m * 8);
    const size_t b_nsr = xtb_alg_up((size_t)m * 4), b_list = xtb_alg_up((size_t)n * 4);
    const size_t b_qs = xtb_alg_up((size_t)(ns + 2) * XB_SP * 8);
    char *panels = (char *)scratch(S_XTB_ALG_PANELS, 4 * pan_up + 2 * vec_up);
    char *ints = (char *)scratch(S_XTB_ALG_INTS, b_nsr + b_list);
    char *gram = (char *)scratch(S_XTB_ALG_GRAM, 4 * 256 * 8);
    char *qsb = (char *)scratch(S_XTB_ALG_QS, 2 * b_qs);
    XCtrl *ctrl = (XCtrl *)scratch(S_XTB_ALG_CTRL, sizeof(XCtrl));
    if (!panels || !ints || !gram || !qsb || !ctrl) return e.err_code;
    double *dR = (double *)panels, *dP = (double *)(panels + pan_up), *dT = (double *)(panels + 2 * pan_up), *dY = (double *)(panels + 3 * pan_up);
    double *dy0 = (double *)(panels + 4 * pan_up), *dsc = (double *)(panels + 4 * pan_up + vec_up);
    int *dnsr = (int *)ints, *dlist = rowlist ? (int *)(ints + b_nsr) : nullptr;
    double *dmats = (double *)gram, *QS = (double *)qsb, *dq = (double *)(qsb + b_qs);
    XCtrl h{}; h.done = done_word;
    HIPCHK(hipMemcpyAsync(dR, R, pan, hipMemcpyHostToDevice, st));
    HIPCHK(hipMemcpyAsync(dP, P, pan, hipMemcpyHostToDevice, st));
    HIPCHK(hipMemcpyAsync(dT, T, pan, hipMemcpyHostToDevice, st));
    if (Ypanel) HIPCHK(hipMemcpyAsync(dY, Ypanel, pan, hipMemcpyHostToDevice, st));
    HIPCHK(hipMemcpyAsync(dy0, y0, (size_t)m * 8, hipMemcpyHostToDevice, st));
    HIPCHK(hipMemcpyAsync(dsc, sc, (size_t)m * 8, hipMemcpyHostToDevice, st));
    HIPCHK(hipMemcpyAsync(dnsr, nsrank, (size_t)m * 4, hipMemcpyHostToDevice, st));
    if (dlist) HIPCHK(hipMemcpyAsync(dlist, rowlist, (size_t)n * 4, hipMemcpyHostToDevice, st));
    HIPCHK(hipMemcpyAsync(dmats, mats, 4 * 256 * 8, hipMemcpyHostToDevice, st));
    HIPCHK(hipMemsetAsync(QS, 0, b_qs, st));
    if (ns > 0) {
        HIPCHK(hipMemcpyAsync(dq, qs, (size_t)ns * XB_SP * 8, hipMemcpyHostToDevice, st));
        hipLaunchKernelGGL(k_xtb_test_qs_encode, dim3((unsigned)(((size_t)ns * XB_SP + 255) / 256)), dim3(256), 0, st, ns, (const double *)dq, QS);
    }
    HIPCHK(hipMemcpyAsync(ctrl, &h, sizeof(XCtrl), hipMemcpyHostToDevice, st));
    HIPCHK(hipStreamSynchronize(st));
    hipLaunchKernelGGL(k_xtb_step, dim3(grid_blocks((n + 15) / 16, 4, 2048)), dim3(XT_NT), 0, st, n, it, (const double *)dmats, dy0, dR, dP, (const double *)dT,
                       (const double *)dsc, (const int *)dnsr, QS, (const XCtrl *)ctrl, (const int *)dlist, Ypanel ? dY : (double *)nullptr);
    if (ns > 0) hipLaunchKernelGGL(k_xtb_test_qs_decode, dim3((unsigned)(((size_t)ns * XB_SP + 255) / 256)), dim3(256), 0, st, ns, (const double *)QS, dq);
    KCHK();
    HIPCHK(hipMemcpyAsync(R, dR, pan, hipMemcpyDeviceToHost, st));
    HIPCHK(hipMemcpyAsync(P, dP, pan, hipMemcpyDeviceToHost, st));
    if (Ypanel) HIPCHK(hipMemcpyAsync(Ypanel, dY, pan, hipMemcpyDeviceToHost, st));
    HIPCHK(hipMemcpyAsync(y0, dy0, (size_t)m * 8, hipMemcpyDeviceToHost, st));
    if (ns > 0) HIPCHK(hipMemcpyAsync(qs, dq, (size_t)ns * XB_SP * 8, hipMemcpyDeviceToHost, st));
    HIPCHK(hipStreamSynchronize(st));
    return e.err_code;
}

extern "C" int dkmc_xtb_test_gram1(int m, const double *const *panels, int ng, int done_word, double *gfin)
{
    Engine &e = eng(); hipStream_t st = e.stream;
    if (m < 1 || m > XTB_ALG_MAXROWS || !panels || ng < 1 || ng > 4096 || !gfin) return dkmc_fail(13, "xtb_test_gram1: bad arguments", __FILE__, __LINE__);
    for (int k = 0; k < 6; ++k) if (!panels[k]) return dkmc_fail(13, "xtb_test_gram1: bad arguments", __FILE__, __LINE__);
    const size_t pan = (size_t)m * XB_SP * 8, pan_up = xtb_alg_up(pan), b_gpart = (size_t)ng * XB_NG * 256 * 8;
    char *dp = (char *)scratch(S_XTB_ALG_PANELS, 6 * pan_up);
    char *gram = (char *)scratch(S_XTB_ALG_GRAM, b_gpart + (size_t)XB_NG * 256 * 8);
    XCtrl *ctrl = (XCtrl *)scratch(S_XTB_ALG_CTRL, sizeof(XCtrl));
    if (!dp || !gram || !ctrl) return e.err_code;
    double *gpart = (double *)gram, *dgfin = (double *)(gram + b_gpart);
    XCtrl h{}; h.done = done_word;
    for (int k = 0; k < 6; ++k) HIPCHK(hipMemcpyAsync(dp + k * pan_up, panels[k], pan, hipMemcpyHostToDevice, st));
    HIPCHK(hipMemsetAsync(gpart, 0xff, b_gpart, st));
    HIPCHK(hipMemcpyAsync(dgfin, gfin, (size_t)XB_NG * 256 * 8, hipMemcpyHostToDevice, st));
    HIPCHK(hipMemcpyAsync(ctrl, &h, sizeof(XCtrl), hipMemcpyHostToDevice, st));
    HIPCHK(hipStreamSynchronize(st));
#define XB_DP(k_) (const double *)(dp + (k_) * pan_up)
    hipLaunchKernelGGL(k_xtb_gram1, dim3(ng), dim3(XT_NT), 0, st, m, XB_DP(0), XB_DP(1), XB_DP(2), XB_DP(3), XB_DP(4), XB_DP(5), gpart, (const XCtrl *)ctrl);
#undef XB_DP
    hipLaunchKernelGGL(k_xtb_gred, dim3(XB_NG * 16), dim3(XT_NT), 0, st, ng, (const double *)gpart, dgfin, (const XCtrl *)ctrl);
    KCHK();
    HIPCHK(hipMemcpyAsync(gfin, dgfin, (size_t)XB_NG * 256 * 8, hipMemcpyDeviceToHost, st));
    HIPCHK(hipStreamSynchronize(st));
    return e.err_code;
}
extern "C" int dkmc_xtb_test_step1(int m, int it, const double *mats, int done_word, double *y0, double *const *panels, const double *sc, const int *nsrank, int ns,
                                   double *qs)
{
    Engine &e = eng(); hipStream_t st = e.stream;
    if (m < 1 || m > XTB_ALG_MAXROWS || it < -1 || it > 0x3fffffff || !mats || !y0 || !panels || !sc || !nsrank || (ns > 0 && !qs))
        return dkmc_fail(13, "xtb_test_step1: bad arguments", __FILE__, __LINE__);
    for (int k = 0; k < 6; ++k) if (!panels[k]) return dkmc_fail(13, "xtb_test_step1: bad arguments", __FILE__, __LINE__);
    if (!xtb_alg_sranks(m, nsrank, ns, nullptr)) return dkmc_fail(13, "xtb_test_step1: bad S ranks", __FILE__, __LINE__);
    const size_t pan = (size_t)m * XB_SP * 8, pan_up = xtb_alg_up(pan), vec_up = xtb_alg_up((size_t)m * 8);
    const size_t b_qs = xtb_alg_up((size_t)(ns + 2) * XB_SP * 8);
    char *dp = (char *)scratch(S_XTB_ALG_PANELS, 6 * pan_up + 2 * vec_up);
    int *dnsr = (int *)scratch(S_XTB_ALG_INTS, xtb_alg_up((size_t)m * 4));
    double *dmats = (double *)scratch(S_XTB_ALG_GRAM, 4 * 256 * 8);
    char *qsb = (char *)scratch(S_XTB_ALG_QS, 2 * b_qs);
    XCtrl *ctrl = (XCtrl *)scratch(S_XTB_ALG_CTRL, sizeof(XCtrl));
    if (!dp || !dnsr || !dmats || !qsb || !ctrl) return e.err_code;
    double *dy0 = (double *)(dp + 6 * pan_up), *dsc = (double *)(dp + 6 * pan_up + vec_up);
    double *QS = (double *)qsb, *dq = (double *)(qsb + b_qs);
    XCtrl h{}; h.done = done_word;
    for (int k = 0; k < 6; ++k) HIPCHK(hipMemcpyAsync(dp + k * pan_up, panels[k], pan, hipMemcpyHostToDevice, st));
    HIPCHK(hipMemcpyAsync(dy0, y0, (size_t)m * 8, hipMemcpyHostToDevice, st));
    HIPCHK(hipMemcpyAsync(dsc, sc, (size_t)m * 8, hipMemcpyHostToDevice, st));
    HIPCHK(hipMemcpyAsync(dnsr, nsrank, (size_t)m * 4, hipMemcpyHostToDevice, st));
    HIPCHK(hipMemcpyAsync(dmats, mats, 4 * 256 * 8, hipMemcpyHostToDevice, st));
    HIPCHK(hipMemsetAsync(QS, 0, b_qs, st));
    if (ns > 0) {
        HIPCHK(hipMemcpyAsync(dq, qs, (size_t)ns * XB_SP * 8, hipMemcpyHostToDevice, st));
        hipLaunchKernelGGL(k_xtb_test_qs_encode, dim3((unsigned)(((size_t)ns * XB_SP + 255) / 256)), dim3(256), 0, st, ns, (const double *)dq, QS);
    }
    HIPCHK(hipMemcpyAsync(ctrl, &h, sizeof(XCtrl), hipMemcpyHostToDevice, st));
    HIPCHK(hipStreamSynchronize(st));
#define XB_DP(k_) (double *)(dp + (k_) * pan_up)
    hipLaunchKernelGGL(k_xtb_step1, dim3(grid_blocks((m + 15) / 16, 4, 2048)), dim3(XT_NT), 0, st, m, it, (const double *)dmats, dy0, XB_DP(4), XB_DP(5), XB_DP(0), XB_DP(1),
                       (const double *)XB_DP(2), (const double *)XB_DP(3), (const double *)dsc, (const int *)dnsr, QS, (const XCtrl *)ctrl);
#undef XB_DP
    if (ns > 0) hipLaunchKernelGGL(k_xtb_test_qs_decode, dim3((unsigned)(((size_t)ns * XB_SP + 255) / 256)), dim3(256), 0, st, ns, (const double *)QS, dq);
    KCHK();
    for (int k = 0; k < 6; ++k) if (k != 2 && k != 3) HIPCHK(hipMemcpyAsync(panels[k], dp + k * pan_up, pan, hipMemcpyDeviceToHost, st));
    HIPCHK(hipMemcpyAsync(y0, dy0, (size_t)m * 8, hipMemcpyDeviceToHost, st));
    if (ns > 0) HIPCHK(hipMemcpyAsync(qs, dq, (size_t)ns * XB_SP * 8, hipMemcpyDeviceToHost, st));
    HIPCHK(hipStreamSynchronize(st));
    return e.err_code;
}

extern "C" int dkmc_xtb_tile_product(int width, int stored_bytes, double *out)
{
    Engine &e = eng(); hipStream_t st = e.stream; const XTState &X = g_xt;
    if (!X.valid || comm_attached() || X.tile_n != X.ntiles || X.ns <= 0) return dkmc_fail(13, "xtb_tile_product: needs the X of a single-GPU solve", __FILE__, __LINE__);
    if (stored_bytes != 8 && !((stored_bytes == 4 || stored_bytes == -4) && g_xb.tval32)) return dkmc_fail(13, "xtb_tile_product: no fp32 image of the tile values (dkmc_set_x_tile_f32)", __FILE__, __LINE__);
    XLive lv;
    if (stored_bytes == -4) { if (int rcl = xt_live_for_test(&lv)) return rcl; }
    const bool lvu = stored_bytes == -4;
    const int ns = X.ns, s = std::max(2, std::min(width, 16)), so = 4 * ((s + 3) / 4);
    const long long ncell = (long long)X.nK * X.nW;
    const int nrec = std::max(X.nitems >> X.rec_shift, lvu ? lv.nrecords : 0);
    double *QS = (double *)scratch(S_XTB_QS, (size_t)X.ns_pad * XB_SP * 8);
    double *rowpartB = (double *)scratch(S_XTB_ROWPART, (size_t)(ncell + 1) * XT_R * so * 8);
    double *colpartB = (double *)scratch(S_XTB_COLPART, (size_t)(nrec + 1) * XT_C * so * 8);
    double *sums = (double *)scratch(S_XTB_PANELS, ((size_t)X.ns_pad * so + 2) * 8);
    XCtrl *ctrl = (XCtrl *)scratch(S_MISC2, 256);
    if (!QS || !rowpartB || !colpartB || !sums || !ctrl) return e.err_code;
    HIPCHK(hipMemsetAsync(QS, 0, (size_t)X.ns_pad * XB_SP * 8, st));
    HIPCHK(hipMemsetAsync(rowpartB, 0, (size_t)(ncell + 1) * XT_R * so * 8, st));
    HIPCHK(hipMemsetAsync(colpartB, 0, (size_t)(nrec + 1) * XT_C * so * 8, st));
    HIPCHK(hipMemsetAsync(sums, 0, ((size_t)X.ns_pad * so + 2) * 8, st));
    HIPCHK(hipMemsetAsync(ctrl, 0, sizeof(XCtrl), st));
    hipLaunchKernelGGL(k_xtb_test_panel, dim3((ns * XB_SP + 255) / 256), dim3(256), 0, st, ns, QS);
    const XbApplyArgs xa{lvu ? lv.item_n : X.item_n, lvu ? lv.items : (const XItem *)g_xb.items + X.item_lo, lvu ? lv.tiles : (const XTile *)g_xb.tiles, (int)X.sub_base,
                         (const double *)g_xb.tval, QS, X.nW, rowpartB, colpartB, ctrl,
                         lvu ? lv.tval32 : (stored_bytes == 4 ? (const float *)g_xb.tval32 : (const float *)nullptr)};
    if (lvu) {
        const XbApplyArgs xf{X.item_n, (const XItem *)g_xb.items + X.item_lo, (const XTile *)g_xb.tiles, (int)X.sub_base, (const double *)g_xb.tval, QS, X.nW, rowpartB, colpartB, ctrl};
        xtb_apply(xf, true, so, 0, st);
        xt_live_zero_dead(lv, rowpartB, so);
    }
    if (xa.n > 0) xtb_apply(xa, true, so, 0, st);
    hipLaunchKernelGGL(k_xtb_fold_local, dim3(std::max(X.nK, 1)), dim3(XT_NT), 0, st, ns, X.nK, X.nW, so, lvu ? lv.wrange : (const int2 *)g_xb.wrange, lvu ? lv.nitem_w : (const int *)g_xb.nitem_w,
                       (const double *)rowpartB, (const double *)colpartB, sums, (const XCtrl *)ctrl, 0, 0, X.nW);
    KCHK();
    if (out) HIPCHK(hipMemcpyAsync(out, sums, (size_t)ns * so * 8, hipMemcpyDeviceToHost, st));
    HIPCHK(hipStreamSynchronize(st));
    return e.err_code;
}

static int xtb_time_apply(int width, int variant, int reps, bool f32, double *us, bool live = false);
extern "C" int dkmc_xtb_time_apply(int width, int variant, int reps, double *us) { return xtb_time_apply(width, variant, reps, false, us); }
extern "C" int dkmc_xtb_time_apply_stored(int width, int stored_bytes, int reps, double *us)
{
    if (stored_bytes != 8 && !((stored_bytes == 4 || stored_bytes == -4) && g_xb.tval32)) return dkmc_fail(13, "xtb_time_apply_stored: no fp32 image of the tile values (dkmc_set_x_tile_f32)", __FILE__, __LINE__);
    return xtb_time_apply(width, 0, reps, stored_bytes != 8, us, stored_bytes == -4);
}
static int xtb_time_apply(int width, int variant, int reps, bool f32, double *us, bool live)
{
    Engine &e = eng(); hipStream_t st = e.stream; const XTState &X = g_xt;
    if (!X.valid || comm_attached() || X.tile_n != X.ntiles || X.ns <= 0 || reps < 1) return dkmc_fail(13, "xtb_time_apply: needs the X of a single-GPU solve", __FILE__, __LINE__);
#ifndef DKMC_MEASURE_VARIANTS
    if (variant != 0) return dkmc_fail(13, "xtb_time_apply: this build carries no measurement variants (DKMC_MEASURE_VARIANTS=1 python __graft_entry__.py)", __FILE__, __LINE__);
#endif
    XLive lv;
    if (live) { if (int rcl = xt_live_for_test(&lv)) return rcl; }
    const int s = std::max(2, std::min(width, 16)), so = 4 * ((s + 3) / 4);
    const long long ncell = (long long)X.nK * X.nW;
    const int nrec = std::max(X.nitems >> X.rec_shift, live ? lv.nrecords : 0);
    double *QS = (double *)scratch(S_XTB_QS, (size_t)X.ns_pad * XB_SP * 8);
    double *rowpartB = (double *)scratch(S_XTB_ROWPART, (size_t)(ncell + 1) * XT_R * so * 8);
    double *colpartB = (double *)scratch(S_XTB_COLPART, (size_t)(nrec + 1) * XT_C * so * 8);
    XCtrl *ctrl = (XCtrl *)scratch(S_MISC2, 256);
    if (!QS || !rowpartB || !colpartB || !ctrl) return e.err_code;
    HIPCHK(hipMemsetAsync(ctrl, 0, sizeof(XCtrl), st));
    hipLaunchKernelGGL(k_xtb_test_panel, dim3((X.ns * XB_SP + 255) / 256), dim3(256), 0, st, X.ns, QS);
    const XbApplyArgs xa{live ? lv.item_n : X.item_n, live ? lv.items : (const XItem *)g_xb.items + X.item_lo, live ? lv.tiles : (const XTile *)g_xb.tiles, (int)X.sub_base,
                         (const double *)g_xb.tval, QS, X.nW, rowpartB, colpartB, ctrl, live ? lv.tval32 : (f32 ? (const float *)g_xb.tval32 : (const float *)nullptr)};
    if (live && xa.n <= 0) return dkmc_fail(13, "xtb_time_apply: the live view holds no tile", __FILE__, __LINE__);
    hipEvent_t e0, e1; HIPCHK(hipEventCreate(&e0)); HIPCHK(hipEventCreate(&e1));
    for (int r = -1; r < reps; ++r) {
        if (r == 0) HIPCHK(hipEventRecord(e0, st));
        xtb_apply(xa, true, so, variant, st);
    }
    HIPCHK(hipEventRecord(e1, st));
    HIPCHK(hipEventSynchronize(e1));
    float ms = 0.f; HIPCHK(hipEventElapsedTime(&ms, e0, e1));
    (void)hipEventDestroy(e0); (void)hipEventDestroy(e1);
    KCHK();
    if (us) *us = (double)ms * 1e3 / reps;
    return e.err_code;
}
```

devicekmc_amd/csrc/xtb_precond.h:

```cpp
#pragma once
#include "nwin_plan.h"
__device__ __forceinline__ int xtb_xcd_block(int nb, int b) { const int xq = nb >> 3, xr = nb & 7, xc = b & 7; return xc * xq + min(xc, xr) + (b >> 3); }
template <int U> __device__ __forceinline__ int xn_bc(int x) { return __builtin_amdgcn_update_dpp(0, x, 0x150 + U, 0xf, 0xf, false); }
template <int J> __device__ __forceinline__ int xn_bc2(int x) { return __builtin_amdgcn_update_dpp(__builtin_amdgcn_update_dpp(0, x, 0x150 + 2 * J, 0xf, 0x3, false), x, 0x151 + 2 * J, 0xf, 0xc, false); }
struct XnEntry { int c, wlo, whi; };
__device__ __forceinline__ XnEntry xn_entry(int c, double w) { return {c, __double2loint(w), __double2hiint(w)}; }
template <int U> __device__ __forceinline__ double xn_w(XnEntry e) { return __hiloint2double(xn_bc<U>(e.whi), xn_bc<U>(e.wlo)); }
template <int J> __device__ __forceinline__ double xn_w2(XnEntry e) { return __hiloint2double(xn_bc2<J>(e.whi), xn_bc2<J>(e.wlo)); }
template <bool MASKED, int U> __device__ __forceinline__ double xn_gather(const double *panel, int v, int c)
{
    const int cu = xn_bc<U>(c);
    return (!MASKED || cu >= 0) ? *reinterpret_cast<const double *>(reinterpret_cast<const char *>(panel) + ((unsigned)cu * (unsigned)(XB_SP * 8) + (unsigned)(v * 8))) : 0.0;
}
struct XnX4 { double x0, x1, x2, x3; };
template <bool MASKED, int U> __device__ __forceinline__ XnX4 xn_gather4(const double *panel, int v, int c)
{
    return {xn_gather<MASKED, U>(panel, v, c), xn_gather<MASKED, U + 1>(panel, v, c), xn_gather<MASKED, U + 2>(panel, v, c), xn_gather<MASKED, U + 3>(panel, v, c)};
}
template <int J> __device__ __forceinline__ double2 xn_gather2(const double *panel, int v8, int c)
{ return *reinterpret_cast<const double2 *>(reinterpret_cast<const char *>(panel) + ((unsigned)xn_bc2<J>(c) * (unsigned)(XB_SP * 8) + (unsigned)(v8 * 16))); }
struct XnSums { double s0, s1, s2, s3; };
template <int U> __device__ __forceinline__ XnSums xn_acc4(XnEntry e, XnX4 x, XnSums s)
{
    s.s0 += xn_w<U>(e) * x.x0; s.s1 += xn_w<U + 1>(e) * x.x1; s.s2 += xn_w<U + 2>(e) * x.x2; s.s3 += xn_w<U + 3>(e) * x.x3; return s;
// ... 238 lines not shown
    const int i = blockIdx.x * blockDim.x + threadIdx.x;
    if (i >= m * XB_SP) return;
    W[i] = (i & 15) == 0 ? y[i >> 4] : 0.0;
}
__global__ void k_xtb_pre_add(int m, const double *__restrict__ Z, double *__restrict__ y)
{
    const int i = blockIdx.x * blockDim.x + threadIdx.x;
    if (i < m) y[i] += Z[(size_t)i * XB_SP];
}
#define XB_RR_MAXPART 1024
__device__ __forceinline__ double xtb_tree256(double a)
{
    __shared__ double red[256];
    red[threadIdx.x] = a;
    __syncthreads();
    for (int o = 128; o > 0; o >>= 1) { if ((int)threadIdx.x < o) red[threadIdx.x] += red[threadIdx.x + o]; __syncthreads(); }
    return red[0];
}
__global__ __launch_bounds__(256) void k_xtb_pre_rr_part(int m, const double *__restrict__ T, const double *__restrict__ b, double *__restrict__ part)
{
    double a = 0.0;
    for (int i = blockIdx.x * 256 + threadIdx.x; i < m; i += gridDim.x * 256) { const double d = T[(size_t)i * XB_SP] - b[i]; a += d * d; }
    a = xtb_tree256(a);
    if (threadIdx.x == 0) part[blockIdx.x] = a;
}
__global__ __launch_bounds__(256) void k_xtb_pre_rr(int np, const double *__restrict__ part, double *__restrict__ out)
{
    double a = 0.0;
    for (int i = threadIdx.x; i < np; i += 256) a += part[i];
    a = xtb_tree256(a);
    if (threadIdx.x == 0) out[0] = a;
}

struct XbNPack { const long long *off; const int *col; const double *w; int lane_bytes; int win_B, win_rows; };
static const int xb_nwin_rows = 450000;
template <class Alloc>
static int xtb_npack(const XtbArgs &A, int n, const int *rowlist, Alloc alloc, long long pad, XbNPack *np)
{
    Engine &e = eng(); hipStream_t st = e.stream;
    const int nsl = (n + 3) / 4;
    int *cnt = (int *)alloc(S_XTB_NPACK_CNT, (size_t)nsl * 4);
    long long *off = (long long *)alloc(S_XTB_NPACK_OFF, (size_t)(nsl + 1) * 8);
    if (!cnt || !off) return e.err_code;
    hipLaunchKernelGGL(k_xtb_npack_width, dim3((nsl + 255) / 256), dim3(256), 0, st, n, A.rp, cnt, rowlist);
    if (int rc = dkmc_exclusive_scan_i32_i64(cnt, off, nsl, off + nsl)) return rc;
    long long nslot = 0;
    HIPCHK(hipMemcpyAsync(&nslot, off + nsl, sizeof(long long), hipMemcpyDeviceToHost, st));
    HIPCHK(hipStreamSynchronize(st));
    int *col = (int *)alloc(S_XTB_NPACK_COL, (size_t)(nslot + pad) * 4);
    double *w = (double *)alloc(S_XTB_NPACK_W, (size_t)(nslot + pad) * 8);
    if (!col || !w) return e.err_code;
    hipLaunchKernelGGL(k_xtb_npack, dim3((nsl + 3) / 4), dim3(256), 0, st, n, A.rp, A.ci, A.val, A.sc, (const long long *)off, col, w, rowlist);
    KCHK();
    np->off = off; np->col = col; np->w = w; np->lane_bytes = e.x_nmul_lane_bytes;
    const bool win = !rowlist && np->lane_bytes == 16 && nwin_use(e.x_nmul_window, n, xb_nwin_rows);
    np->win_B = win ? nwin_block_rows(e.x_nmul_window_block) : 0;
    np->win_rows = win ? nwin_cap_rows(std::min(std::max(e.x_nmul_window_cap, 0), NWIN_CAP_BYTES)) : 0;
    return 0;
}
struct XbNRank { int n; const int *rowlist; const XbNPack *np; double *QS; const XCtrl *ctrl; };
template <bool LIST>
static void xtb_nstep(hipStream_t st, const XtbArgs &A, const XbNRank &R, const double *in, const double *add, double ca, double cb, double *out, bool qsf)
{
    const dim3 g((R.n + 15) / 16), b(XT_NT);
    if (!R.np) { hipLaunchKernelGGL(k_xtb_nmul<LIST>, g, b, 0, st, R.n, A.rp, A.ci, A.val, A.sc, in, add, ca, cb, out, R.ctrl, R.rowlist); return; }
    if (!LIST && R.np->win_B > 0) {
        const int B = R.np->win_B, lds = nwin_lds_bytes(R.n, B, R.np->win_rows);
        const auto kw = qsf ? k_xtb_nmulw<true> : k_xtb_nmulw<false>;
        static bool big_lds = false;
        if (!big_lds) {
            (void)hipFuncSetAttribute((const void *)k_xtb_nmulw<true>, hipFuncAttributeMaxDynamicSharedMemorySize, NWIN_CAP_BYTES);
            (void)hipFuncSetAttribute((const void *)k_xtb_nmulw<false>, hipFuncAttributeMaxDynamicSharedMemorySize, NWIN_CAP_BYTES);
            big_lds = true;
        }
        hipLaunchKernelGGL(kw, dim3(nwin_blocks(R.n, B)), dim3(XN_WIN_NT), lds, st, R.n, R.np->off, R.np->col, R.np->w, A.sc, in, add, ca, cb, out, R.ctrl,
                           qsf ? A.nsrank : (const int *)nullptr, qsf ? R.QS : (double *)nullptr, B, R.np->win_rows);
        return;
    }
    const bool b16 = R.np->lane_bytes == 16;
    const auto k = qsf ? (b16 ? k_xtb_nmulp16<true, LIST> : k_xtb_nmulp<true, LIST>) : (b16 ? k_xtb_nmulp16<false, LIST> : k_xtb_nmulp<false, LIST>);
    hipLaunchKernelGGL(k, g, b, 0, st, R.n, R.np->off, R.np->col, R.np->w, A.sc, in, add, ca, cb, out, R.ctrl, qsf ? A.nsrank : (const int *)nullptr,
                       qsf ? R.QS : (double *)nullptr, R.rowlist);
}
template <class Pn, class Pre, class Ranks>
static int xtb_applyL(hipStream_t st, const XtbArgs &A, int pd, const double *pc, Pn src, Pn dst, Pn w1, Pn w2, bool qs, Pre pre, Ranks ranks)
{
    Pn in = src;
    for (int i = 0; i < pd; ++i) {
        const Pn out = (i == pd - 1) ? dst : ((i & 1) ? w2 : w1);
        const int j = pd - 1 - i;
        const double cb = i == 0 ? pc[pd] : 1.0;
        if (int rc = pre(i, in)) return rc;
        if (int rc = ranks(true, [&](const XbNRank &R, auto at) {
                (R.rowlist ? xtb_nstep<true> : xtb_nstep<false>)(st, A, R, at(in), at(src), pc[j], cb, at(out), qs && i == pd - 1);
            })) return rc;
        in = out;
    }
    if (!qs || pd <= 0) return 0;
    return ranks(false, [&](const XbNRank &R, auto at) {
        if (!R.np) hipLaunchKernelGGL(k_xtb_qs_from, dim3((unsigned)(((size_t)A.m * XB_SP + 255) / 256)), dim3(256), 0, st, A.m, (const double *)at(dst), A.sc, A.nsrank,
                                      R.QS, R.ctrl);
    });
}
template <class F>
static void xtb_cheb_monomial(int d, double b, F f, double *pc)
{
    const int n = d + 1;
    const double a = -1.0;
    double fx[XB_MAXPOLY1 + 1], c[XB_MAXPOLY1 + 1], pt[XB_MAXPOLY1 + 1] = {0}, Tm2[XB_MAXPOLY1 + 1] = {0}, Tm1[XB_MAXPOLY1 + 1] = {0};
    for (int k = 0; k < n; ++k) { const double t = cos(M_PI * (k + 0.5) / n), x = 0.5 * (b - a) * t + 0.5 * (b + a); fx[k] = f(x); }
    for (int j = 0; j < n; ++j) { double acc = 0.0; for (int k = 0; k < n; ++k) acc += fx[k] * cos(M_PI * j * (k + 0.5) / n); c[j] = acc * 2.0 / n; }
    c[0] *= 0.5;
    Tm2[0] = 1.0; Tm1[1] = 1.0;
    pt[0] += c[0]; pt[1] += c[1];
    for (int j = 2; j <= d; ++j) {
        double Tj[XB_MAXPOLY1 + 1];
        for (int i = 0; i <= XB_MAXPOLY1; ++i) Tj[i] = (i >= 1 ? 2.0 * Tm1[i - 1] : 0.0) - Tm2[i];
        for (int i = 0; i <= XB_MAXPOLY1; ++i) { pt[i] += c[j] * Tj[i]; Tm2[i] = Tm1[i]; Tm1[i] = Tj[i]; }
    }
    const double al = 2.0 / (b - a), be = -(a + b) / (b - a);
    double res[XB_MAXPOLY1 + 2] = {0}; res[0] = pt[d]; int deg = 0;
    for (int i = d - 1; i >= 0; --i) {
        double nr[XB_MAXPOLY1 + 2] = {0};
        for (int q = 0; q <= deg; ++q) { nr[q] += res[q] * be; nr[q + 1] += res[q] * al; }
        ++deg; nr[0] += pt[i];
        for (int q = 0; q <= XB_MAXPOLY1 + 1; ++q) res[q] = nr[q];
    }
    for (int q = 0; q <= d; ++q) pc[q] = res[q];
}
static void xtb_poly_coeffs(int pd, double *pc)
{
    if (pd > 0) xtb_cheb_monomial(pd, 1.0 - std::min(0.5, 1.6 / (double)(pd * pd)), [](double x) { return 1.0 / sqrt(1.0 - x); }, pc);
}
static void xtb_poly1_coeffs(int n, double *pc, double *qmin)
{
    xtb_cheb_monomial(n, 1.0 - std::min(0.5, 3.2 / (double)(n * n)), [](double x) { return 1.0 / (1.0 - x); }, pc);
    double lo = 1e300;
    for (int k = 0; k <= 4000; ++k) {
        const double x = -1.0 + (double)k / 2000.0;
        double q = pc[n];
        for (int j = n - 1; j >= 0; --j) q = q * x + pc[j];
        lo = std::min(lo, q);
    }
    if (qmin) *qmin = lo;
}
static int xtb_poly1_degree(const Engine &e, int d)
{
    if (e.x_poly1_degree > 0) return std::min(e.x_poly1_degree, XB_MAXPOLY1);
    if (d == 10) return 10;
    if (d == 16) return 18;
    return std::min((5 * d + 3) / 4, XB_MAXPOLY1);
}
static bool xtb_poly_one(const Engine &e) { return e.x_poly_form == 1 || (e.x_poly_form == 2 && e.x_poly_auto != 0); }
static const int xb_poly_rows[2] = {225000, 450000};
static const int xb_poly_steps[3] = {8, 10, 16};
static int xtb_poly_rule(int m, const int *rows)
{
    if (m <= 2) return 0;
    const int *n = (rows && (rows[0] > 0 || rows[1] > 0)) ? rows : xb_poly_rows;
    return std::min(xb_poly_steps[m < n[0] ? 0 : (m < n[1] ? 1 : 2)], XB_MAXPOLY);
}
static int xtb_poly_degree(const Engine &e, const XtbArgs &A)
{
    if (A.sharded || A.m <= 2 || A.ns <= 0 || e.x_poly <= 0) return 0;
    return e.x_poly_auto ? xtb_poly_rule(A.m, e.x_poly_rows) : std::min(e.x_poly, XB_MAXPOLY);
}

extern "C" int dkmc_xtb_poly_coeffs(int degree, double *pc)
{
    if (degree < 1 || degree > XB_MAXPOLY || !pc) return dkmc_fail(13, "xtb_poly_coeffs: degree outside 1 ... 16", __FILE__, __LINE__);
    xtb_poly_coeffs(degree, pc);
    return 0;
}
extern "C" int dkmc_xtb_poly1_coeffs(int n, double *pc, double *qmin)
{
    if (n < 1 || n > XB_MAXPOLY1 || !pc) return dkmc_fail(13, "xtb_poly1_coeffs: degree outside 1 ... 20", __FILE__, __LINE__);
    xtb_poly1_coeffs(n, pc, qmin);
    return 0;
}
extern "C" int dkmc_xtb_poly_rule(int m) { return xtb_poly_rule(m, eng().x_poly_rows); }
__global__ void k_xtb_test_qs_decode(int ns, const double *__restrict__ QS, double *__restrict__ out)
{
    const int i = blockIdx.x * blockDim.x + threadIdx.x;
    if (i < ns * XB_SP) out[i] = QS[xtb_qs_pos(i >> 4, i & 15)];
}
static void *xtb_test_alloc(int slot, size_t bytes)
{
    return scratch(slot == S_XTB_NPACK_CNT ? S_XTB_TEST_NPCNT : slot == S_XTB_NPACK_OFF ? S_XTB_TEST_NPOFF : slot == S_XTB_NPACK_COL ? S_XTB_TEST_NPCOL : S_XTB_TEST_NPW, bytes);
}
static int xtb_test_qs_out(hipStream_t st, int ns, const double *QS, double *qs)
{
    double *dq = (double *)scratch(S_XTB_TEST_ADD, (size_t)ns * XB_SP * 8);
    if (!dq) return eng().err_code;
    hipLaunchKernelGGL(k_xtb_test_qs_decode, dim3((unsigned)(((size_t)ns * XB_SP + 255) / 256)), dim3(256), 0, st, ns, QS, dq);
    KCHK();
    HIPCHK(hipMemcpyAsync(qs, dq, (size_t)ns * XB_SP * 8, hipMemcpyDeviceToHost, st));
    return 0;
}
extern "C" int dkmc_xtb_test_nstep(int m, const long long *rp, const int *ci, const double *val, const double *sc, const double *in, const double *add,
                                   double ca, double cb, int form, const int *rowlist, int nlist, const int *nsrank, int ns, double *out, double *qs)
{
    Engine &e = eng(); hipStream_t st = e.stream;
    if (m < 1 || !rp || !sc || !in || !add || !out || (form != 0 && form != 1)) return dkmc_fail(13, "xtb_test_nstep: bad arguments", __FILE__, __LINE__);
    const long long nnz = rp[m];
    if (rp[0] != 0 || nnz < 0 || nnz > 0x7fffffffll || (nnz > 0 && (!ci || !val))) return dkmc_fail(13, "xtb_test_nstep: bad row pointers", __FILE__, __LINE__);
    for (int i = 0; i < m; ++i) if (rp[i + 1] < rp[i]) return dkmc_fail(13, "xtb_test_nstep: bad row pointers", __FILE__, __LINE__);
    for (long long p = 0; p < nnz; ++p) if (ci[p] < 0 || ci[p] >= m) return dkmc_fail(13, "xtb_test_nstep: column outside the rows", __FILE__, __LINE__);
    if (rowlist) {
        if (nlist < 1 || nlist > m) return dkmc_fail(13, "xtb_test_nstep: bad row list", __FILE__, __LINE__);
        for (int i = 0; i < nlist; ++i) if (rowlist[i] < 0 || rowlist[i] >= m) return dkmc_fail(13, "xtb_test_nstep: bad row list", __FILE__, __LINE__);
    }
    if (nsrank) {
        if (ns < 1 || !qs) return dkmc_fail(13, "xtb_test_nstep: bad S ranks", __FILE__, __LINE__);
        for (int i = 0; i < m; ++i) if (nsrank[i] < -1 || nsrank[i] >= ns) return dkmc_fail(13, "xtb_test_nstep: bad S ranks", __FILE__, __LINE__);
    }
    const size_t pan = (size_t)m * XB_SP * 8;
    xrp_t *drp = (xrp_t *)scratch(S_XTB_TEST_RP, (size_t)(m + 1) * sizeof(xrp_t));
    int *dci = (int *)scratch(S_XTB_TEST_CI, (size_t)nnz * 4);
    double *dval = (double *)scratch(S_XTB_TEST_VAL, (size_t)nnz * 8), *dsc = (double *)scratch(S_XTB_TEST_SC, (size_t)m * 8);
    double *din = (double *)scratch(S_XTB_TEST_IN, pan), *dadd = (double *)scratch(S_XTB_TEST_ADD, pan), *dout = (double *)scratch(S_XTB_TEST_OUT, pan);
    int *dns = nsrank ? (int *)scratch(S_XTB_TEST_NSR, (size_t)m * 4) : nullptr;
    int *dlist = rowlist ? (int *)scratch(S_XTB_TEST_LIST, (size_t)nlist * 4) : nullptr;
    double *QS = nsrank ? (double *)scratch(S_XTB_TEST_QS, (size_t)(ns + 2) * XB_SP * 8) : nullptr;
    XCtrl *ctrl = (XCtrl *)scratch(S_XTB_TEST_CTRL, sizeof(XCtrl));
    if (!drp || !dci || !dval || !dsc || !din || !dadd || !dout || (nsrank && (!dns || !QS)) || (rowlist && !dlist) || !ctrl) return e.err_code;
    HIPCHK(hipMemcpyAsync(drp, rp, (size_t)(m + 1) * sizeof(xrp_t), hipMemcpyHostToDevice, st));
    if (nnz > 0) {
        HIPCHK(hipMemcpyAsync(dci, ci, (size_t)nnz * 4, hipMemcpyHostToDevice, st));
        HIPCHK(hipMemcpyAsync(dval, val, (size_t)nnz * 8, hipMemcpyHostToDevice, st));
    }
    HIPCHK(hipMemcpyAsync(dsc, sc, (size_t)m * 8, hipMemcpyHostToDevice, st));
    HIPCHK(hipMemcpyAsync(din, in, pan, hipMemcpyHostToDevice, st));
    HIPCHK(hipMemcpyAsync(dadd, add, pan, hipMemcpyHostToDevice, st));
    HIPCHK(hipMemcpyAsync(dout, out, pan, hipMemcpyHostToDevice, st));
    if (dns) HIPCHK(hipMemcpyAsync(dns, nsrank, (size_t)m * 4, hipMemcpyHostToDevice, st));
    if (dlist) HIPCHK(hipMemcpyAsync(dlist, rowlist, (size_t)nlist * 4, hipMemcpyHostToDevice, st));
    if (QS) HIPCHK(hipMemsetAsync(QS, 0, (size_t)(ns + 2) * XB_SP * 8, st));
    HIPCHK(hipMemsetAsync(ctrl, 0, sizeof(XCtrl), st));
    XtbArgs A{};
    A.m = m; A.ns = ns; A.rp = drp; A.ci = dci; A.val = dval; A.sc = dsc; A.nsrank = dns;
    const int n = rowlist ? nlist : m;
    XbNPack npk{};
    if (form == 1) { if (int rc = xtb_npack(A, n, (const int *)dlist, xtb_test_alloc, 0, &npk)) return rc; }
    const XbNRank R{n, dlist, form == 1 ? &npk : nullptr, QS, ctrl};
    (rowlist ? xtb_nstep<true> : xtb_nstep<false>)(st, A, R, din, dadd, ca, cb, dout, nsrank != nullptr);
    if (nsrank && form == 0)
        hipLaunchKernelGGL(k_xtb_qs_from, dim3((unsigned)((pan / 8 + 255) / 256)), dim3(256), 0, st, m, (const double *)dout, (const double *)dsc, (const int *)dns, QS, (const XCtrl *)ctrl);
    KCHK();
    HIPCHK(hipMemcpyAsync(out, dout, pan, hipMemcpyDeviceToHost, st));
    if (nsrank) { if (int rc = xtb_test_qs_out(st, ns, QS, qs)) return rc; }
    HIPCHK(hipStreamSynchronize(st));
    return e.err_code;
}
extern "C" int dkmc_xtb_check_poly(int degree, int form, const double *in, double *out, double *qs)
{
    Engine &e = eng(); hipStream_t st = e.stream; const XTState &X = g_xt;
    if (!X.valid || comm_attached() || X.tile_n != X.ntiles || X.ns <= 0) return dkmc_fail(13, "xtb_check_poly: needs the X of a single-GPU solve", __FILE__, __LINE__);
    if (degree < 1 || degree > XB_MAXPOLY || (form != 0 && form != 1) || !in || !out || !qs) return dkmc_fail(13, "xtb_check_poly: bad arguments", __FILE__, __LINE__);
    const int m = X.Nsub;
    const size_t pan = (size_t)m * XB_SP * 8;
    double *sc = (double *)e.buf[S_CG_S];
    double *din = (double *)scratch(S_XTB_TEST_IN, pan), *dout = (double *)scratch(S_XTB_TEST_OUT, pan);
    double *W1 = (double *)scratch(S_XTB_TEST_W1, pan), *W2 = (double *)scratch(S_XTB_TEST_W2, pan);
    double *QS = (double *)scratch(S_XTB_TEST_QS, (size_t)X.ns_pad * XB_SP * 8);
    XCtrl *ctrl = (XCtrl *)scratch(S_XTB_TEST_CTRL, sizeof(XCtrl));
    if (!din || !dout || !W1 || !W2 || !QS || !ctrl) return e.err_code;
    if (!sc || !g_xb.rp || !g_xb.ci || !g_xb.val || !g_xb.nsrank) return dkmc_fail(13, "xtb_check_poly: no solver state", __FILE__, __LINE__);
    HIPCHK(hipMemcpyAsync(din, in, pan, hipMemcpyHostToDevice, st));
    HIPCHK(hipMemsetAsync(QS, 0, (size_t)X.ns_pad * XB_SP * 8, st));
    HIPCHK(hipMemsetAsync(ctrl, 0, sizeof(XCtrl), st));
    XtbArgs A{};
    A.m = m; A.ns = X.ns; A.ns_pad = X.ns_pad; A.rp = g_xb.rp; A.ci = g_xb.ci; A.val = g_xb.val; A.sc = sc; A.nsrank = g_xb.nsrank;
    XbNPack npk{};
    if (form == 1) { if (int rc = xtb_npack(A, m, nullptr, xtb_test_alloc, 0, &npk)) return rc; }
    const XbNRank nk{m, nullptr, form == 1 ? &npk : nullptr, QS, ctrl};
    double pc[XB_MAXPOLY + 1] = {1.0};
    xtb_poly_coeffs(degree, pc);
    if (int rc = xtb_applyL(st, A, degree, pc, din, dout, W1, W2, true, [](int, double *) { return 0; },
                            [&](bool, auto f) { f(nk, [](double *p) { return p; }); return 0; })) return rc;
    KCHK();
    HIPCHK(hipMemcpyAsync(out, dout, pan, hipMemcpyDeviceToHost, st));
    if (int rc = xtb_test_qs_out(st, X.ns, QS, qs)) return rc;
    HIPCHK(hipStreamSynchronize(st));
    return e.err_code;
}
extern "C" int dkmc_xtb_time_poly(int degree, int reps, double *us)
{
    Engine &e = eng(); hipStream_t st = e.stream; const XTState &X = g_xt;
    if (!X.valid || comm_attached() || X.tile_n != X.ntiles || X.ns <= 0) return dkmc_fail(13, "xtb_time_poly: needs the X of a single-GPU solve", __FILE__, __LINE__);
    if (degree < 1 || degree > XB_MAXPOLY || reps < 1 || !us) return dkmc_fail(13, "xtb_time_poly: bad arguments", __FILE__, __LINE__);
    const int m = X.Nsub;
    const size_t pan = (size_t)m * XB_SP * 8;
    double *sc = (double *)e.buf[S_CG_S];
    double *din = (double *)scratch(S_XTB_TEST_IN, pan), *dout = (double *)scratch(S_XTB_TEST_OUT, pan);
    double *W1 = (double *)scratch(S_XTB_TEST_W1, pan), *W2 = (double *)scratch(S_XTB_TEST_W2, pan);
    double *QS = (double *)scratch(S_XTB_TEST_QS, (size_t)X.ns_pad * XB_SP * 8);
    XCtrl *ctrl = (XCtrl *)scratch(S_XTB_TEST_CTRL, sizeof(XCtrl));
    if (!din || !dout || !W1 || !W2 || !QS || !ctrl) return e.err_code;
    if (!sc || !g_xb.rp || !g_xb.ci || !g_xb.val || !g_xb.nsrank) return dkmc_fail(13, "xtb_time_poly: no solver state", __FILE__, __LINE__);
    HIPCHK(hipMemsetAsync(din, 0, pan, st));
    HIPCHK(hipMemsetAsync(ctrl, 0, sizeof(XCtrl), st));
    XtbArgs A{};
    A.m = m; A.ns = X.ns; A.ns_pad = X.ns_pad; A.rp = g_xb.rp; A.ci = g_xb.ci; A.val = g_xb.val; A.sc = sc; A.nsrank = g_xb.nsrank;
    XbNPack npk{};
    if (int rc = xtb_npack(A, m, nullptr, xtb_test_alloc, 0, &npk)) return rc;
    const XbNRank nk{m, nullptr, &npk, QS, ctrl};
// ... 17 lines not shown
```

devicekmc_amd/lib.py:

```python
import ctypes as C
import os

_HERE = os.path.dirname(os.path.abspath(__file__))
LIB_PATH = os.path.join(_HERE, "libdevicekmc_hip.so")

c_int_p = C.POINTER(C.c_int)
c_dbl_p = C.POINTER(C.c_double)
vp = C.c_void_p


class dkmc_gpubuf(C.Structure):
    _PTRS = ["site_charge", "site_power", "site_potential_boundary", "site_potential_charge", "site_temperature",
             "site_CB_edge", "T_bg", "atom_power", "atom_CB_edge", "atom_virtual_potentials", "atom_charge",
             "site_element", "atom_element", "site_x", "site_y", "site_z", "atom_x", "atom_y", "atom_z",
             "metal_types", "sigma", "k", "lattice", "freq", "neigh_idx", "site_layer",
             "Device_row_ptr_d", "Device_col_indices_d", "contact_left_row_ptr", "contact_left_col_indices",
             "contact_right_row_ptr", "contact_right_col_indices"]
    _INTS = ["Device_nnz", "contact_left_nnz", "contact_right_nnz", "num_metal_types_", "N_", "nn_", "N_atom_"]
    _fields_ = [(n, vp) for n in _PTRS] + [(n, C.c_int) for n in _INTS]


class dkmc_stats(C.Structure):
    _fields_ = [("cg_iters_K", C.c_int), ("cg_iters_CB", C.c_int), ("cg_iters_X", C.c_int),
                ("cg_rr_K", C.c_double), ("cg_rr_CB", C.c_double), ("cg_rr_X", C.c_double),
                ("n_events", C.c_int), ("n_charged", C.c_int), ("N_atom", C.c_int),
                ("X_nnz", C.c_longlong), ("psum_last", C.c_double),
                ("spmv_long_ms", C.c_double), ("spmv_short_ms", C.c_double),
                ("spmv_long_launches", C.c_int), ("spmv_short_launches", C.c_int),
                ("spmv_long_nnz", C.c_longlong), ("spmv_short_nnz", C.c_longlong),
                ("spmv_long_rows", C.c_int), ("spmv_short_rows", C.c_int),
                ("spmv_segments", C.c_int), ("spmv_pad", C.c_int), ("spmv_segment_entries", C.c_longlong),
                ("comm_ranks", C.c_int), ("comm_local_segments", C.c_int), ("comm_count_per_rank", C.c_longlong),
                ("comm_ms", C.c_double), ("comm_launches", C.c_int), ("comm_pad", C.c_int),
                ("spmv_tiles", C.c_int), ("spmv_pad2", C.c_int), ("spmv_tile_entries", C.c_longlong),
                ("xt_subblocks", C.c_longlong), ("xt_local_subblocks", C.c_longlong), ("xt_items", C.c_int), ("xt_kc", C.c_int),
                ("xt_sparse_nnz", C.c_longlong), ("xt_ns", C.c_int), ("xt_split_launch", C.c_int),
                ("kcg_ms", C.c_double), ("kcg_iters_timed", C.c_int), ("kcg_blocked", C.c_int), ("pair_ms", C.c_double), ("pair_evaluated", C.c_longlong), ("pair_tested", C.c_longlong), ("xt_records", C.c_longlong), ("tcache_bytes", C.c_longlong), ("kcg_bytes", C.c_longlong), ("xb_aux", C.c_int), ("xb_poly_used", C.c_int), ("xb_width", C.c_int), ("xb_fallback", C.c_int), ("x_tile_stream", C.c_int), ("x_tile_f64_rounds", C.c_int), ("x_tile_f32_bytes", C.c_longlong)]


class dkmc_xtb_ctrl(C.Structure):
    _fields_ = [("rr", C.c_double * 2), ("done_local", C.c_int), ("sharded", C.c_int), ("done", C.c_int), ("iters", C.c_int),
                ("abort_local", C.c_int), ("aborted", C.c_int), ("pad", C.c_int * 2), ("xchg_timeout", C.c_int), ("pad2", C.c_int)]


ALLGATHER_FN = C.CFUNCTYPE(C.c_int, C.c_void_p, C.c_size_t, C.c_int, C.c_int, C.c_void_p)


_I, _D = C.c_int, C.c_double
SYMBOLS = {
    "dkmc_last_error": (C.c_char_p, []),
    "dkmc_clear_error": (None, []),
    "dkmc_get_stats": (C.POINTER(dkmc_stats), []),
    "dkmc_get_gpu_info": (_I, [C.c_char_p, _I, _I]),
    "dkmc_set_gpu": (_I, [_I]),
    "dkmc_set_stream": (_I, [vp]),
    "dkmc_synchronize": (_I, []),
    "dkmc_set_cg_tolerance": (None, [_D]),
    "dkmc_set_cb_edge_domain": (None, [_I]),
    "dkmc_set_x_block": (None, [_I]),
    "dkmc_get_x_block": (_I, []),
    "dkmc_set_k_slab": (None, [_I]),
    "dkmc_get_k_slab": (_I, []),
    "dkmc_xt_tile_census": (_I, [C.POINTER(C.c_longlong)]),
    "dkmc_set_x_items": (None, [_I]),
    "dkmc_set_x_poly": (None, [_I]),
    "dkmc_get_x_poly": (_I, []),
    "dkmc_set_x_poly_auto": (None, [_I]),
    "dkmc_get_x_poly_auto": (_I, []),
    "dkmc_set_x_poly_auto_rows": (None, [_I, _I]),
    "dkmc_set_x_poly_form": (None, [_I]),
    "dkmc_get_x_poly_form": (_I, []),
    "dkmc_get_x_poly_form_used": (_I, []),
    "dkmc_get_x_poly_products": (_I, []),
    "dkmc_debug_set_x_poly1_degree": (None, [_I]),
    "dkmc_set_x_tile_f32": (None, [_I]),
    "dkmc_get_x_tile_f32": (_I, []),
    "dkmc_set_x_tile_drop": (None, [_D]),
    "dkmc_get_x_tile_drop": (_D, []),
    "dkmc_set_x_tile_drop_unit": (None, [_I]),
    "dkmc_get_x_tile_drop_unit": (_I, []),
    "dkmc_set_x_tile_drop_auto": (None, [_I]),
    "dkmc_get_x_tile_drop_auto": (_I, []),
    "dkmc_get_x_tile_drop_used": (_D, []),
    "dkmc_get_x_tile_live_info": (_I, [C.POINTER(C.c_longlong), c_dbl_p]),
    "dkmc_xt_get_live": (_I, [_D, vp, vp]),
    "dkmc_xt_get_live_masks": (_I, [_D, vp]),
    "dkmc_debug_fail_true_residual_once": (None, []),
    "dkmc_set_x_fold_form": (None, [_I]),
    "dkmc_get_x_fold_form": (_I, []),
    "dkmc_debug_poison_fold_cells": (None, [_I]),
    "dkmc_xt_get_fold_lists": (_I, [_I, c_int_p, c_int_p, vp]),
    "dkmc_set_x_static_tiles": (None, [_I]),
    "dkmc_get_x_static_tiles": (_I, []),
    "dkmc_get_x_static_info": (_I, [C.POINTER(C.c_longlong)]),
    "dkmc_debug_x_static_verify": (_I, [_I]),
    "dkmc_debug_get_x_static_verify": (_I, [C.POINTER(C.c_longlong)]),
    "dkmc_x_static_strips": (_I, [_I]),
    "dkmc_x_static_rule": (_I, [_I]),
    "dkmc_debug_set_x_static_gate": (None, [_I]),
    "dkmc_xt_get_srow": (_I, [c_int_p, vp]),
    "dkmc_xt_get_diag": (_I, [vp]),
    "dkmc_set_x_nmul_form": (None, [_I]),
    "dkmc_get_x_nmul_form": (_I, []),
    "dkmc_set_x_nmul_lane_bytes": (None, [_I]),
    "dkmc_get_x_nmul_lane_bytes": (_I, []),
    "dkmc_set_x_nmul_window": (None, [_I]),
    "dkmc_get_x_nmul_window": (_I, []),
    "dkmc_debug_set_x_nmul_window": (None, [_I, _I]),
    "dkmc_set_x_apply_form": (None, [_I]),
    "dkmc_get_x_apply_form": (_I, []),
    "dkmc_set_x_slab": (None, [_I]),
    "dkmc_get_x_slab": (_I, []),
    "dkmc_set_x_slab_poly": (None, [_I]),
    "dkmc_get_x_slab_poly": (_I, []),
    "dkmc_set_x_aux_warm": (None, [_I]),
    "dkmc_get_x_aux_warm": (_I, []),
    "dkmc_set_x_aux": (None, [_I]),
    "dkmc_get_x_aux": (_I, []),
    "dkmc_set_k_blocked": (None, [_I]),
    "dkmc_get_k_blocked": (_I, []),
    "dkmc_set_k_blocked_large": (None, [_I]),
    "dkmc_get_k_blocked_large": (_I, []),
    "dkmc_set_k_window_word_bytes": (None, [_I]),
    "dkmc_get_k_window_word_bytes": (_I, []),
    "dkmc_kcg_form_info": (_I, [C.POINTER(dkmc_gpubuf), C.POINTER(C.c_longlong)]),
    "dkmc_kcg_form_words": (_I, [C.POINTER(dkmc_gpubuf), C.POINTER(C.c_longlong)]),
    "dkmc_debug_kbw_halfword_pos": (_I, [_I, _I]),
    "dkmc_debug_kbw_segment_cap": (None, [_I]),
    "dkmc_set_pair_cutoff": (None, [_D]),
    "dkmc_reset_pair_sum_cache": (None, []),
    "dkmc_set_pair_form": (None, [_I]),
    "dkmc_get_pair_form": (_I, []),
    "dkmc_get_pair_sum_info": (_I, [C.POINTER(C.c_longlong), C.POINTER(_D)]),
    "dkmc_set_tcache_budget": (None, [C.c_longlong]),
    "dkmc_set_current_warm_start": (None, [_I]),
    "dkmc_get_current_warm_start": (_I, []),
    "dkmc_get_current_warm_vector": (_I, [C.POINTER(dkmc_gpubuf), vp, _I, c_int_p]),
    "dkmc_set_current_warm_vector": (_I, [C.POINTER(dkmc_gpubuf), vp, _I]),
    "dkmc_get_current_warm_aux": (_I, [C.POINTER(dkmc_gpubuf), vp, C.c_longlong, C.POINTER(C.c_longlong)]),
    "dkmc_set_current_warm_aux": (_I, [C.POINTER(dkmc_gpubuf), vp, C.c_longlong]),
    "dkmc_set_profiling": (None, [_I]),
    "dkmc_set_x_format": (None, [_I]),
    "dkmc_get_x_format": (_I, []),
    "dkmc_gpubuf_create": (_I, [C.POINTER(dkmc_gpubuf), _I, _I, _I, _I, vp, vp, vp, vp, vp, vp, _D, _D, _D, vp]),
    "dkmc_gpubuf_free": (_I, [C.POINTER(dkmc_gpubuf)]),
    "dkmc_gpubuf_sync_host_to_gpu": (_I, [C.POINTER(dkmc_gpubuf), vp, vp, vp, vp, vp, vp, vp, vp, _D]),
    "dkmc_gpubuf_sync_gpu_to_host": (_I, [C.POINTER(dkmc_gpubuf), vp, vp, vp, vp, vp, vp, vp, vp, vp]),
    "dkmc_copy_power_from_gpu": (_I, [C.POINTER(dkmc_gpubuf), vp]),
    "dkmc_copy_charge_to_gpu": (_I, [C.POINTER(dkmc_gpubuf), vp]),
    "dkmc_copy_Tbg_to_gpu": (_I, [C.POINTER(dkmc_gpubuf), _D]),
    "dkmc_copy_to_const_memory": (_I, [vp, vp, vp, vp, _I]),
    "dkmc_build_neighbor_index": (_I, [_I, vp, vp, vp, vp, _I, _D, c_int_p, vp]),
    "dkmc_initialize_sparsity": (_I, [C.POINTER(dkmc_gpubuf), _I, _D, _I]),
    "dkmc_free_sparsity": (_I, [C.POINTER(dkmc_gpubuf)]),
    "dkmc_update_charge_gpu": (_I, [vp, vp, vp, _I, _I, vp, _I]),
    "dkmc_update_CB_edge_gpu_sparse": (_I, [C.POINTER(dkmc_gpubuf), _I, _I, _I, _D, _I, _D, _D, _D, _I]),
    "dkmc_background_potential_gpu_sparse": (_I, [C.POINTER(dkmc_gpubuf), _I, _I, _I, _D, _I, _D, _D, _D, _I, _I]),
    "dkmc_poisson_gridless_gpu": (_I, [_I, _I, _I, vp, vp, vp, vp, vp, vp, vp, vp]),
    "dkmc_solve_sparse_CG_Jacobi": (_I, [vp, vp, vp, _I, _I, vp, vp, c_int_p, c_dbl_p]),
    "dkmc_solve_sparse_CG_splitmatrix": (_I, [vp, _I, vp, vp, vp, _I, _I, vp, _I, vp, vp, _D, c_int_p, c_dbl_p]),
    "dkmc_execute_kmc_step_gpu": (_I, [_I, _I, vp, vp, vp, _I, vp, vp, vp, vp, vp, vp, vp, vp, vp, vp, vp, vp,
                                       vp, _I, _I, c_int_p, c_int_p, vp, c_dbl_p]),
    "dkmc_build_event_list": (_I, [_I, _I, vp, vp, vp, _I, vp, vp, vp, vp, vp, vp, vp, vp, vp, vp, vp, vp, vp]),
    "dkmc_set_event_temperature": (None, [_I]),
    "dkmc_get_event_temperature": (_I, []),
    "dkmc_build_event_list_T": (_I, [_I, _I, vp, vp, vp, _I, vp, vp, vp, vp, vp, vp, vp, vp, vp, vp, vp, vp, vp, vp, vp]),
    "dkmc_event_rate_census": (_I, [_I, _I, vp, vp, vp, vp, c_dbl_p]),
    "dkmc_set_event_census": (None, [_I]),
    "dkmc_get_event_census_on": (_I, []),
    "dkmc_get_event_census": (_I, [c_dbl_p]),
    "dkmc_debug_get_event_times": (_I, [c_dbl_p]),
    "dkmc_debug_event_loop": (_I, [_I, _I, vp, vp, vp, vp, vp, vp, _I, _I, c_int_p, c_int_p, vp, c_dbl_p]),
    "dkmc_update_power_gpu_sparse": (_I, [C.POINTER(dkmc_gpubuf), _I, _I, _I, _D, _I, _D, _D, _D, _D, _D, _D, _D, _D, _I,
                                          c_dbl_p, _I, _I, _D]),
    "dkmc_get_last_X": (_I, [c_int_p, C.POINTER(C.c_longlong), vp, vp, vp]),
    "dkmc_set_current_map": (None, [_I]),
    "dkmc_get_current_map": (_I, []),
    "dkmc_copy_current_map_from_gpu": (_I, [C.POINTER(dkmc_gpubuf), vp, vp, vp]),
    "dkmc_get_current_map_info": (_I, [C.POINTER(dkmc_gpubuf), c_dbl_p]),
    "dkmc_find_clusters": (_I, [_I, _I, vp, vp, vp, vp, vp, _I, _I, _I, _I, vp]),
    "dkmc_copy_cluster_table": (_I, [_I, vp, vp, vp, vp, vp, vp, c_int_p]),
    "dkmc_get_cluster_info": (_I, [c_int_p, c_dbl_p]),
    "dkmc_debug_set_cluster_round_cap": (None, [_I]),
    "dkmc_debug_get_cluster_times": (_I, [c_dbl_p]),
    "dkmc_find_gaps": (_I, [_I, vp, vp, vp, vp, _I, vp, _I, _I, _D]),
    "dkmc_get_gap_info": (_I, [C.POINTER(C.c_longlong), c_dbl_p]),
    "dkmc_copy_gap_edges": (_I, [_I, vp, vp, vp, vp, vp, c_int_p]),
    "dkmc_copy_gap_chain": (_I, [_I, vp, vp, vp, c_int_p]),
    "dkmc_debug_set_gap_cell_skip": (None, [_I]),
    "dkmc_find_paths": (_I, [_I, _I, vp, vp, vp, _I, _I, _I, vp, vp]),
    "dkmc_get_path_info": (_I, [C.POINTER(C.c_longlong)]),
    "dkmc_copy_path_sites": (_I, [_I, vp, c_int_p]),
    "dkmc_copy_path_profile": (_I, [_I, vp, vp, vp, c_int_p]),
    "dkmc_debug_set_path_round_cap": (None, [_I]),
    "dkmc_debug_get_path_times": (_I, [c_dbl_p]),
    "dkmc_track_clusters": (_I, [_I, vp, vp, vp, _I, _I, vp]),
    "dkmc_get_track_info": (_I, [C.POINTER(C.c_longlong), c_dbl_p]),
    "dkmc_copy_track_pairs": (_I, [_I, vp, vp, vp, vp, c_int_p]),
    "dkmc_copy_track_now": (_I, [_I, vp, vp, vp, vp, vp, vp, c_int_p]),
    "dkmc_copy_track_prev": (_I, [_I, vp, vp, vp, vp, vp, vp, c_int_p]),
    "dkmc_copy_track_critical": (_I, [_I, vp, c_int_p]),
    "dkmc_debug_set_track_hash": (None, [_I]),
    "dkmc_debug_get_track_times": (_I, [c_dbl_p]),
    "dkmc_find_cuts": (_I, [_I, _I, vp, vp, vp, _I, _I, vp, _I, vp, vp]),
    "dkmc_get_cut_info": (_I, [C.POINTER(C.c_longlong)]),
    "dkmc_copy_cut_path": (_I, [_I, vp, vp, vp, vp, c_int_p]),
    "dkmc_copy_cut_bypasses": (_I, [_I, vp, vp, vp, vp, c_int_p]),
    "dkmc_copy_cut_necks": (_I, [_I, vp, vp, vp, vp, c_int_p]),
    "dkmc_debug_set_cut_round_cap": (None, [_I]),
    "dkmc_debug_get_cut_times": (_I, [c_dbl_p]),
    "dkmc_find_flow": (_I, [_I, _I, vp, vp, vp, _I, _I, _I, vp, vp]),
    "dkmc_get_flow_info": (_I, [C.POINTER(C.c_longlong), c_dbl_p]),
    "dkmc_copy_flow_strands": (_I, [_I, vp, vp, vp, vp, vp, vp, vp, vp, vp, vp, c_int_p]),
    "dkmc_copy_flow_strand_sites": (_I, [_I, vp, c_int_p]),
    "dkmc_debug_set_flow_round_cap": (None, [_I]),
    "dkmc_debug_get_flow_times": (_I, [c_dbl_p]),
    "dkmc_update_temperatureglobal_gpu": (_I, [vp, vp, _I, _D, _D, _D, _D, _D]),
    "dkmc_update_temperature_global_analytic": (_I, [vp, vp, _I, _D, _D, _D, _D, _D, c_dbl_p]),
    "dkmc_set_heat_cg_tolerance": (None, [_D]),
    "dkmc_set_heat_form": (None, [_I]),
    "dkmc_get_heat_form": (_I, []),
    "dkmc_get_heat_info": (_I, [C.POINTER(C.c_longlong)]),
    "dkmc_debug_heat_chain": (None, [_I, _I]),
    "dkmc_construct_laplacian": (_I, [C.POINTER(dkmc_gpubuf), _I, _I, _D]),
    "dkmc_update_temperature_local": (_I, [C.POINTER(dkmc_gpubuf), _D, _D, _D, _D, _D, _D, _D, _I,
                                           C.POINTER(_I), C.POINTER(_I), C.POINTER(_I), c_dbl_p]),
    "dkmc_xt_time_share": (_I, [_I, _I, _I, c_dbl_p, c_dbl_p, c_int_p, C.POINTER(C.c_longlong)]),
    "dkmc_xt_check_shares": (_I, [_I, c_dbl_p, c_dbl_p, C.POINTER(C.c_longlong), C.POINTER(C.c_longlong), c_int_p]),
    "dkmc_xtb_check_product": (_I, [_I, c_dbl_p, c_dbl_p]),
    "dkmc_xtb_time_apply": (_I, [_I, _I, _I, c_dbl_p]),
    "dkmc_xtb_time_apply_stored": (_I, [_I, _I, _I, c_dbl_p]),
    "dkmc_xtb_time_poly": (_I, [_I, _I, c_dbl_p]),
    "dkmc_xtb_tile_product": (_I, [_I, _I, vp]),
    "dkmc_xt_get_tiles": (_I, [C.POINTER(C.c_longlong), C.POINTER(C.c_longlong), vp, vp]),
    "dkmc_xtb_poly_coeffs": (_I, [_I, c_dbl_p]),
    "dkmc_xtb_poly_rule": (_I, [_I]),
    "dkmc_xtb_poly1_coeffs": (_I, [_I, c_dbl_p, c_dbl_p]),
    "dkmc_xtl_drop_rule": (_D, [C.c_longlong]),
    "dkmc_debug_xtl_census_form": (_I, [_I]),
    "dkmc_debug_xtl_census_reread": (C.c_longlong, []),
    "dkmc_set_x_tile_drop_auto_subblocks": (None, [C.c_longlong]),
    "dkmc_xtb_test_nstep": (_I, [_I, vp, vp, vp, vp, vp, vp, _D, _D, _I, vp, _I, vp, _I, vp, vp]),
    "dkmc_xtb_check_poly": (_I, [_I, _I, vp, vp, vp]),
    "dkmc_xtb_test_gram": (_I, [_I, vp, vp, vp, vp, _I, _I, _I, vp, C.POINTER(dkmc_xtb_ctrl)]),
    "dkmc_xtb_test_small": (_I, [_I, _I, _I, vp, _D, C.POINTER(dkmc_xtb_ctrl), vp, C.POINTER(dkmc_xtb_ctrl)]),
    "dkmc_xtb_test_step": (_I, [_I, _I, vp, _I, vp, vp, vp, vp, vp, vp, _I, vp, _I, vp, vp]),
    "dkmc_xtb_test_gram1": (_I, [_I, vp, _I, _I, vp]),
    "dkmc_xtb_test_step1": (_I, [_I, _I, vp, _I, vp, vp, vp, vp, _I, vp]),
    "dkmc_kcg_emulate_slabs": (_I, [C.POINTER(dkmc_gpubuf), _I, _I, _I, _D, _D, _D, _I, _I, _I, _I, c_dbl_p, c_int_p, c_int_p, c_dbl_p, C.POINTER(C.c_longlong)]),
    "dkmc_xtb_emulate_slabs": (_I, [_I, _I, _D, _I, _I, c_dbl_p, c_int_p, c_int_p, c_dbl_p, C.POINTER(C.c_longlong), c_int_p]),
    "dkmc_xtb_slab_last": (_I, [c_int_p, C.POINTER(C.c_longlong), c_dbl_p]),
    "dkmc_debug_inject_fault": (None, [_I, _I]),
    "dkmc_debug_step_stop_word": (_I, [_I, _I, _I, C.POINTER(C.c_int), C.POINTER(C.c_int)]),
    "dkmc_comm_unique_id": (_I, [C.c_char_p]),
    "dkmc_comm_init_rccl": (_I, [_I, _I, C.c_char_p]),
    "dkmc_comm_peer_prepare": (_I, [C.c_size_t, C.c_char_p]),
    "dkmc_comm_peer_attach": (_I, [C.c_char_p]),
    "dkmc_comm_peer_detach": (_I, []),
    "dkmc_comm_peer_info": (_I, [C.POINTER(C.c_int), C.POINTER(C.c_longlong), C.POINTER(C.c_longlong), C.POINTER(C.c_double)]),
    "dkmc_comm_init_host": (_I, [_I, _I, ALLGATHER_FN, vp]),
    "dkmc_comm_allgather_host": (_I, [vp, C.c_size_t]),
    "dkmc_comm_info": (_I, [C.POINTER(_I), C.POINTER(_I), C.POINTER(_I)]),
    "dkmc_comm_destroy": (_I, []),
}

_lib = None


def load():
    global _lib
    if _lib is None:
        if not os.path.exists(LIB_PATH):
            raise ImportError("%s not found: build it with `python -c 'import __graft_entry__ as g; g.build()'` "
                              "(hipcc --offload-arch=gfx950); there is no CPU fallback" % LIB_PATH)
        import torch
        lib = C.CDLL(LIB_PATH)
        for name, (res, args) in SYMBOLS.items():
            fn = getattr(lib, name)
            fn.restype = res
            fn.argtypes = args
        _lib = lib
    return _lib


class DeviceKMCError(RuntimeError):
    pass


def check(rc):
    if rc != 0:
        msg = load().dkmc_last_error().decode()
        load().dkmc_clear_error()
        raise DeviceKMCError("devicekmc_hip error %d: %s" % (rc, msg))
```

include/devicekmc_hip.h:

```cpp
#ifndef DEVICEKMC_HIP_H
#define DEVICEKMC_HIP_H

#ifdef __cplusplus
extern "C" {
#endif

#ifndef DKMC_ELEMENT_T
#define DKMC_ELEMENT_T int
#endif
typedef struct dkmc_gpubuf {
    int *site_charge;
    double *site_power, *site_potential_boundary, *site_potential_charge, *site_temperature;
    double *site_CB_edge;
    double *T_bg;
    double *atom_power;
    double *atom_CB_edge;
    double *atom_virtual_potentials;
    int *atom_charge;
    DKMC_ELEMENT_T *site_element;
    DKMC_ELEMENT_T *atom_element;
    double *site_x, *site_y, *site_z;
    double *atom_x, *atom_y, *atom_z;
    DKMC_ELEMENT_T *metal_types;
    double *sigma, *k, *lattice, *freq;
    int *neigh_idx, *site_layer;
    int *Device_row_ptr_d, *Device_col_indices_d;
    int *contact_left_row_ptr, *contact_left_col_indices;
    int *contact_right_row_ptr, *contact_right_col_indices;
    int Device_nnz, contact_left_nnz, contact_right_nnz;
    int num_metal_types_, N_, nn_, N_atom_;
} dkmc_gpubuf;

typedef struct dkmc_stats {
    int cg_iters_K, cg_iters_CB, cg_iters_X;
    double cg_rr_K, cg_rr_CB, cg_rr_X;
    int n_events;
    int n_charged;
    int N_atom;
    long long X_nnz;
    double psum_last;
    double spmv_long_ms, spmv_short_ms;
    int spmv_long_launches, spmv_short_launches;
    long long spmv_long_nnz, spmv_short_nnz;
    int spmv_long_rows, spmv_short_rows;
    int spmv_segments, spmv_pad;
    long long spmv_segment_entries;
    int comm_ranks, comm_local_segments;
    long long comm_count_per_rank;
    double comm_ms;
    int comm_launches, comm_pad;
    int spmv_tiles, spmv_pad2;
    long long spmv_tile_entries;
    long long xt_subblocks, xt_local_subblocks;
    int xt_items, xt_kc;
    long long xt_sparse_nnz;
    int xt_ns, xt_split_launch;
    double kcg_ms;
    int kcg_iters_timed, kcg_blocked;
    double pair_ms;
    long long pair_evaluated;
    long long pair_tested;
    long long xt_records;
    long long tcache_bytes;
    long long kcg_bytes;
    int xb_aux, xb_poly_used;
    int xb_width, xb_fallback;
    int x_tile_stream, x_tile_f64_rounds;
    long long x_tile_f32_bytes;
} dkmc_stats;

const char *dkmc_last_error(void);
void dkmc_clear_error(void);
const dkmc_stats *dkmc_get_stats(void);

int dkmc_get_gpu_info(char *gpu_string, int capacity, int dev);
int dkmc_set_gpu(int dev);
int dkmc_set_stream(void *hip_stream);
int dkmc_synchronize(void);
void dkmc_set_cg_tolerance(double tol);
void dkmc_set_cb_edge_domain(int atoms_only);
void dkmc_set_tcache_budget(long long bytes);
void dkmc_set_pair_cutoff(double x_cut);
void dkmc_reset_pair_sum_cache(void);
void dkmc_set_pair_form(int form);
int dkmc_get_pair_form(void);
void dkmc_set_x_block(int s);
int dkmc_get_x_block(void);
void dkmc_set_x_poly(int degree);
int dkmc_get_x_poly(void);
void dkmc_set_x_poly_auto(int on);
int dkmc_get_x_poly_auto(void);
void dkmc_set_x_poly_form(int form);
int dkmc_get_x_poly_form(void);
int dkmc_get_x_poly_form_used(void);
int dkmc_get_x_poly_products(void);
void dkmc_set_x_nmul_form(int form);
int dkmc_get_x_nmul_form(void);
void dkmc_set_x_tile_f32(int mode);
int dkmc_get_x_tile_f32(void);
void dkmc_set_x_tile_drop(double theta);
double dkmc_get_x_tile_drop(void);
void dkmc_set_x_tile_drop_unit(int unit);
int dkmc_get_x_tile_drop_unit(void);
void dkmc_set_x_tile_drop_auto(int on);
int dkmc_get_x_tile_drop_auto(void);
double dkmc_get_x_tile_drop_used(void);
void dkmc_set_x_static_tiles(int mode);
int dkmc_get_x_static_tiles(void);
int dkmc_get_x_static_info(long long *info8);
void dkmc_set_x_nmul_lane_bytes(int bytes);
int dkmc_get_x_nmul_lane_bytes(void);
void dkmc_set_x_nmul_window(int mode);
int dkmc_get_x_nmul_window(void);
void dkmc_set_x_slab(int on);
int dkmc_get_x_slab(void);
void dkmc_set_x_slab_poly(int on);
int dkmc_get_x_slab_poly(void);
void dkmc_set_k_slab(int on);
int dkmc_get_k_slab(void);
void dkmc_set_x_aux(int mode);
int dkmc_get_x_aux(void);
void dkmc_set_x_aux_warm(int on);
int dkmc_get_x_aux_warm(void);
void dkmc_set_k_blocked(int on);
int dkmc_get_k_blocked(void);
void dkmc_set_k_blocked_large(int on);
int dkmc_get_k_blocked_large(void);
void dkmc_set_k_window_word_bytes(int bytes);
int dkmc_get_k_window_word_bytes(void);
void dkmc_set_current_warm_start(int mode);
int dkmc_get_current_warm_start(void);
int dkmc_get_current_warm_vector(const dkmc_gpubuf *buf, double *h_out, int capacity, int *n_out);
int dkmc_set_current_warm_vector(const dkmc_gpubuf *buf, const double *h_in, int n);
int dkmc_get_current_warm_aux(const dkmc_gpubuf *buf, double *h_out, long long capacity, long long *n_out);
int dkmc_set_current_warm_aux(const dkmc_gpubuf *buf, const double *h_in, long long n);
void dkmc_set_profiling(int on);
void dkmc_set_x_format(int tiled);
int dkmc_get_x_format(void);

int dkmc_gpubuf_create(dkmc_gpubuf *buf, int N, int N_atom, int nn, int num_metal_types,
                       const int *h_site_layer, const double *h_site_x, const double *h_site_y,
                       const double *h_site_z, const int *h_neigh_idx, const int *h_metals,
                       double freq, double sigma, double k, const double *h_lattice);
int dkmc_gpubuf_free(dkmc_gpubuf *buf);
int dkmc_gpubuf_sync_host_to_gpu(dkmc_gpubuf *buf, const int *h_site_element, const int *h_site_charge,
                                 const double *h_site_power, const double *h_site_CB_edge,
                                 const double *h_site_potential_boundary, const double *h_site_potential_charge,
                                 const double *h_site_temperature, const double *h_atom_CB_edge, double T_bg);
int dkmc_gpubuf_sync_gpu_to_host(const dkmc_gpubuf *buf, int *h_site_element, int *h_site_charge,
                                 double *h_site_power, double *h_site_CB_edge,
                                 double *h_site_potential_boundary, double *h_site_potential_charge,
                                 double *h_site_temperature, double *h_atom_CB_edge, double *T_bg);
int dkmc_copy_power_from_gpu(const dkmc_gpubuf *buf, double *h_power);
int dkmc_copy_charge_to_gpu(dkmc_gpubuf *buf, const int *h_charge);
int dkmc_copy_Tbg_to_gpu(dkmc_gpubuf *buf, double T_bg);

int dkmc_copy_to_const_memory(const double *h_E_gen, const double *h_E_rec, const double *h_E_Vdiff,
                              const double *h_E_Odiff, int num_layers);

int dkmc_build_neighbor_index(int N, const double *d_x, const double *d_y, const double *d_z, const double *h_lattice,
                              int pbc, double nn_dist, int *nn_out, int *d_neigh_out);

int dkmc_initialize_sparsity(dkmc_gpubuf *buf, int pbc, double nn_dist, int num_atoms_contact);
int dkmc_free_sparsity(dkmc_gpubuf *buf);

int dkmc_update_charge_gpu(const int *d_site_element, int *d_site_charge, const int *d_neigh_idx,
                           int N, int nn, const int *d_metals, int num_metals);
int dkmc_update_CB_edge_gpu_sparse(dkmc_gpubuf *buf, int N, int N_left_tot, int N_right_tot, double Vd,
                                   int pbc, double high_G, double low_G, double nn_dist, int num_metals);
int dkmc_background_potential_gpu_sparse(dkmc_gpubuf *buf, int N, int N_left_tot, int N_right_tot, double Vd,
                                         int pbc, double high_G, double low_G, double nn_dist,
                                         int num_metals, int kmc_step_count);
int dkmc_poisson_gridless_gpu(int num_atoms_contact, int pbc, int N, const double *d_lattice,
                              const double *d_sigma, const double *d_k,
                              const double *d_posx, const double *d_posy, const double *d_posz,
                              const int *d_site_charge, double *d_site_potential_charge);

int dkmc_solve_sparse_CG_Jacobi(double *d_A_data, const int *d_A_row_ptr, const int *d_A_col_indices,
                                int A_nnz, int m, double *d_x, double *d_y, int *iters_out, double *rr_out);

int dkmc_solve_sparse_CG_splitmatrix(const double *d_M, int msub, const double *d_A_data, const int *d_A_row_ptr, const int *d_A_col_indices,
                                     int A_nnz, int m, const int *d_insertion_indices, int index_offset, const double *d_x, double *d_y,
                                     double tol, int *iters_out, double *rnorm_out);

int dkmc_execute_kmc_step_gpu(int N, int nn, const int *d_neigh_idx, const int *d_site_layer,
                              const double *d_lattice, int pbc, const double *d_T_bg, const double *d_freq,
                              const double *d_sigma, const double *d_k,
                              const double *d_posx, const double *d_posy, const double *d_posz,
                              const double *d_site_potential_boundary, const double *d_site_potential_charge,
                              const double *d_site_temperature, int *d_site_element, int *d_site_charge,
                              const double *h_uniform, int n_uniform, int resume,
                              int *n_events_out, int *exhausted_out, int *h_event_log, double *event_time_out);
int dkmc_build_event_list(int N, int nn, const int *d_neigh_idx, const int *d_site_layer,
                          const double *d_lattice, int pbc, const double *d_T_bg, const double *d_freq,
                          const double *d_sigma, const double *d_k,
                          const double *d_posx, const double *d_posy, const double *d_posz,
                          const double *d_site_potential_boundary, const double *d_site_potential_charge,
                          const int *d_site_element, const int *d_site_charge,
                          int *d_event_type, double *d_event_prob);

void dkmc_set_event_temperature(int mode);
int dkmc_get_event_temperature(void);
int dkmc_build_event_list_T(int N, int nn, const int *d_neigh_idx, const int *d_site_layer,
                            const double *d_lattice, int pbc, const double *d_T_bg, const double *d_freq,
                            const double *d_sigma, const double *d_k,
                            const double *d_posx, const double *d_posy, const double *d_posz,
                            const double *d_site_potential_boundary, const double *d_site_potential_charge,
                            const int *d_site_element, const int *d_site_charge,
                            int *d_event_type, double *d_event_prob, const double *d_site_temperature, int *d_n_bad);
int dkmc_event_rate_census(int N, int nn, const int *d_neigh_idx, const int *d_site_element, const double *d_site_temperature,
                           const double *d_ev_prob, double *h_info16);
void dkmc_set_event_census(int on);
int dkmc_get_event_census_on(void);
int dkmc_get_event_census(double *info16);

int dkmc_update_power_gpu_sparse(dkmc_gpubuf *buf, int num_source_inj, int num_ground_ext, int num_layers_contact,
                                 double Vd, int pbc, double high_G, double low_G, double loop_G, double G0,
                                 double tol, double nn_dist, double m_e, double V0, int num_metals,
                                 double *h_imacro, int solve_heating_local, int solve_heating_global, double alpha_disp);
int dkmc_get_last_X(int *rows_out, long long *nnz_out, int *h_row_ptr, int *h_col, double *h_data);
void dkmc_set_current_map(int on);
int dkmc_get_current_map(void);
int dkmc_copy_current_map_from_gpu(const dkmc_gpubuf *buf, double *h_thr_all, double *h_thr_tun, double *h_net_tun);
int dkmc_get_current_map_info(const dkmc_gpubuf *buf, double *info8);

enum { DKMC_MEMBERS_METAL = 1, DKMC_MEMBERS_VACANCY = 2, DKMC_MEMBERS_NEUTRAL_ONLY = 4 };
int dkmc_find_clusters(int N, int nn, const int *d_index, const int *d_site_element, const int *d_site_charge, const double *d_site_x,
                       const int *d_metals, int num_metals, int members, int n_left_sites, int n_right_sites, int *d_label);
int dkmc_copy_cluster_table(int capacity, int *h_root, int *h_size, int *h_n_vacancy, int *h_flags, double *h_xmin, double *h_xmax,
                            int *rows_out);
int dkmc_get_cluster_info(int *info8, double *x3);

int dkmc_find_gaps(int N, const double *d_x, const double *d_y, const double *d_z, const double *h_lattice, int pbc,
                   const int *d_label, int n_left_sites, int n_right_sites, double r_max);
int dkmc_get_gap_info(long long *info8, double *d2x2);
int dkmc_copy_gap_edges(int capacity, int *h_site_a, int *h_site_b, int *h_root_a, int *h_root_b, double *h_d2, int *rows_out);
int dkmc_copy_gap_chain(int capacity, int *h_from, int *h_to, double *h_d2, int *rows_out);

int dkmc_find_paths(int N, int nn, const int *d_index, const int *d_label, const double *d_site_x,
                    int n_left_sites, int n_right_sites, int slack, int *d_hops_left, int *d_hops_right);
int dkmc_get_path_info(long long *info8);
int dkmc_copy_path_sites(int capacity, int *h_site, int *rows_out);
int dkmc_copy_path_profile(int capacity, int *h_count, double *h_xmin, double *h_xmax, int *rows_out);

enum { DKMC_TRACK_LEFT = 1, DKMC_TRACK_RIGHT = 2, DKMC_TRACK_BORN = 4, DKMC_TRACK_MERGED = 8, DKMC_TRACK_FRAGMENT = 16,
       DKMC_TRACK_DIED = 4, DKMC_TRACK_SPLIT = 8, DKMC_TRACK_ABSORBED = 16 };
int dkmc_track_clusters(int N, const int *d_label_prev, const int *d_label_now, const double *d_site_x, int n_left_sites, int n_right_sites,
                        int *d_site_change);
// ... 56 lines not shown
```

include/devicekmc_hip_debug.h:

```cpp
#ifndef DEVICEKMC_HIP_DEBUG_H
#define DEVICEKMC_HIP_DEBUG_H
#include "devicekmc_hip.h"
#ifdef __cplusplus
extern "C" {
#endif

int dkmc_xt_time_share(int nranks, int rank, int reps, double *apply_us, double *side_us , int *items_out, long long *subblocks_out);
int dkmc_xt_check_shares(int nranks, double *max_abs_diff, double *max_abs, long long *subblocks_sum, long long *items_sum, int *items_total);
int dkmc_xtb_check_product(int width, double *max_abs_diff, double *max_abs);
int dkmc_xtb_poly_coeffs(int degree, double *pc);
int dkmc_xtb_poly_rule(int m);
void dkmc_set_x_poly_auto_rows(int n0, int n1);
int dkmc_xtb_test_nstep(int m, const long long *rp, const int *ci, const double *val, const double *sc, const double *in, const double *add,
                        double ca, double cb, int form, const int *rowlist, int nlist, const int *nsrank, int ns, double *out, double *qs);
int dkmc_xtb_check_poly(int degree, int form, const double *in, double *out, double *qs);
void dkmc_debug_set_x_nmul_window(int cap_bytes, int block_rows);
int dkmc_xtb_time_poly(int degree, int reps, double *us);
typedef struct dkmc_xtb_ctrl { double rr[2]; int done_local, sharded; int done; int iters; int abort_local, aborted; int pad[2]; int xchg_timeout, pad2; } dkmc_xtb_ctrl;
int dkmc_xtb_test_gram(int m, const double *P, const double *T, const double *R, const int *nsrank, int ns, int ng, int done_word, double *gfin,
                       dkmc_xtb_ctrl *ctrl_out);
int dkmc_xtb_test_small(int it, int s, int nrg, const double *gblocks, double tol2, const dkmc_xtb_ctrl *ctrl_in, double *mats, dkmc_xtb_ctrl *ctrl_out);
int dkmc_xtb_test_step(int m, int it, const double *mats, int done_word, double *y0, double *R, double *P, const double *T, const double *sc,
                       const int *nsrank, int ns, const int *rowlist, int nlist, double *Ypanel, double *qs);
int dkmc_xtb_poly1_coeffs(int n, double *pc, double *qmin);
void dkmc_debug_set_x_poly1_degree(int n);
int dkmc_xtb_test_gram1(int m, const double *const *panels, int ng, int done_word, double *gfin);
int dkmc_xtb_test_step1(int m, int it, const double *mats, int done_word, double *y0, double *const *panels, const double *sc, const int *nsrank, int ns,
                        double *qs);
int dkmc_xtb_time_apply(int width, int variant, int reps, double *us);
int dkmc_xt_tile_census(long long *hist);
void dkmc_set_x_items(int kc);
void dkmc_debug_fail_true_residual_once(void);
int dkmc_xtb_tile_product(int width, int stored_bytes, double *out);
int dkmc_xt_get_tiles(long long *ntiles, long long *nsub, int *tiles4, double *tval);
int dkmc_xtb_time_apply_stored(int width, int stored_bytes, int reps, double *us);
int dkmc_get_x_tile_live_info(long long *info8, double *ms2);
int dkmc_debug_xtl_census_form(int form);
long long dkmc_debug_xtl_census_reread(void);
double dkmc_xtl_drop_rule(long long stored_subblocks);
void dkmc_set_x_tile_drop_auto_subblocks(long long gate);
int dkmc_xt_get_live(double theta, int *live_per_tile, double *sS_out);
int dkmc_xt_get_live_masks(double theta, int *mask_per_tile);
void dkmc_set_x_fold_form(int form);
int dkmc_get_x_fold_form(void);
void dkmc_debug_poison_fold_cells(int on);
int dkmc_xt_get_fold_lists(int live, int *nK, int *nW, int *rows);
int dkmc_debug_x_static_verify(int on);
int dkmc_debug_get_x_static_verify(long long *v4);
int dkmc_x_static_strips(int n_metals);
int dkmc_x_static_rule(int members);
void dkmc_debug_set_x_static_gate(int members);
int dkmc_xt_get_srow(int *ns_out, int *srow_out);
int dkmc_xt_get_diag(double *d_out);
void dkmc_set_x_apply_form(int form);
int dkmc_get_x_apply_form(void);
void dkmc_debug_inject_fault(int phase, int iteration);
int dkmc_debug_step_stop_word(int m, int it, int done_word, int *updated, int *done_after);

int dkmc_xtb_emulate_slabs(int nranks, int width, double tol, int time_rank, int sweep_cap, double *rel_diff, int *iters_slab, int *iters_ref,
                           double *times_us, long long *xdoubles, int *rows_min_max);

int dkmc_xtb_slab_last(int *exchanges_per_sweep, long long *halo_doubles_per_exchange, double *nmul_us);

int dkmc_kcg_emulate_slabs(dkmc_gpubuf *buf, int N, int N_left, int N_right, double Vd, double high_G, double low_G, int num_metals, int nranks, int time_rank,
                           int iter_cap, double *max_abs_diff, int *iters_slab, int *iters_ref, double *times_us, long long *halo_rows);

int dkmc_kcg_form_info(dkmc_gpubuf *buf, long long *info );
int dkmc_kcg_form_words(dkmc_gpubuf *buf, long long *info );
int dkmc_debug_kbw_halfword_pos(int width, int entry);
void dkmc_debug_kbw_segment_cap(int cap);
int dkmc_get_pair_sum_info(long long *info , double *ms );
void dkmc_debug_heat_chain(int on, int budget);
void dkmc_debug_set_cluster_round_cap(int cap);
int dkmc_debug_get_cluster_times(double *ms2);
void dkmc_debug_set_gap_cell_skip(int on);
void dkmc_debug_set_path_round_cap(int cap);
int dkmc_debug_get_path_times(double *ms2);
void dkmc_debug_set_track_hash(int mode);
int dkmc_debug_get_track_times(double *ms2);
void dkmc_debug_set_cut_round_cap(int cap);
int dkmc_debug_get_cut_times(double *ms2);
void dkmc_debug_set_flow_round_cap(int cap);
int dkmc_debug_get_flow_times(double *ms3);
int dkmc_debug_get_event_times(double *ms2);
int dkmc_debug_event_loop(int N, int nn, const int *d_neigh_idx, const double *d_ev_prob_in, int *d_site_element, int *d_site_charge, const double *d_freq,
                          const double *h_uniform, int n_uniform, int resume,
                          int *n_events_out, int *exhausted_out, int *h_event_log, double *event_time_out);

#ifdef __cplusplus
}
#endif
#endif
```

Before: 5.572.

## Stop polynomial-preconditioned CG on true residual norm computed in step kernel

Adds an in-kernel reduction of the unpreconditioned residual norm (first column) to the one-polynomial CG step, plus a single-block kernel that marks the solve done once that norm falls below the tolerance bound. This lets the solver stop on the true residual rather than the tighter preconditioned-norm criterion (tol scaled by qmin), which may save CG iterations on large systems (m >= 96000 by default). The cost is an extra small kernel launch and reduction per iteration, and the early stop still relies on the existing true-residual check and re-entry if it triggers too soon.

```diff
diff --git a/devicekmc_amd/csrc/common.h b/devicekmc_amd/csrc/common.h
--- a/devicekmc_amd/csrc/common.h
+++ b/devicekmc_amd/csrc/common.h
@@ -154,7 +154,9 @@
     int4 *seg = nullptr;
     int word_bytes = 4;
 };
+constexpr double X_STOP_MARGIN_DEFAULT = 1.0;
 constexpr int X_POLY_DEFAULT = 8;
+struct XStopLast { int fired = 0, with_norm = 0, m = 0; double norm = -1.0, rz = 0.0, true_res = 0.0; };
 struct Engine {
     hipStream_t stream = nullptr;
     int device = 0;
@@ -177,6 +179,9 @@
     int x_poly_form = 2;
     int x_poly1_degree = 0;
     int x_poly_form_used = 0, x_poly_products = 0;
+    int x_stop_form = 2;
+    double x_stop_margin = X_STOP_MARGIN_DEFAULT;
+    XStopLast x_stop_last{};
     int x_slab_poly = 0;
     int x_aux_warm = 0;
     int x_items_kc = 0;
@@ -267,6 +272,7 @@
     S_TR_HASH, S_TR_COMP, S_TR_SITE, S_TR_ROWS, S_TR_CTRL,
     S_CUT_SITE, S_CUT_TABLE, S_CUT_ROWS, S_CUT_CTRL,
     S_FL_SITE, S_FL_ROWS, S_FL_CTRL,
+    S_XTB_STOPN,
     S_NSLOTS
 };
 static_assert(S_NSLOTS <= Engine::NBUF, "scratch slots");
diff --git a/devicekmc_amd/csrc/engine.hip b/devicekmc_amd/csrc/engine.hip
--- a/devicekmc_amd/csrc/engine.hip
+++ b/devicekmc_amd/csrc/engine.hip
@@ -77,6 +77,19 @@
 int dkmc_get_x_poly_form(void) { return eng().x_poly_form; }
 int dkmc_get_x_poly_form_used(void) { return eng().x_poly_form_used; }
 int dkmc_get_x_poly_products(void) { return eng().x_poly_products; }
+void dkmc_set_x_stop_form(int form) { eng().x_stop_form = form == 1 ? 1 : (form == 2 ? 2 : 0); }
+int dkmc_get_x_stop_form(void) { return eng().x_stop_form; }
+void dkmc_set_x_stop_margin(double kappa) { eng().x_stop_margin = (kappa > 0.0 && kappa <= 1.0) ? kappa : X_STOP_MARGIN_DEFAULT; }
+double dkmc_get_x_stop_margin(void) { return eng().x_stop_margin; }
+int dkmc_get_x_stop_info(int *fired, double *norm, double *rz, double *true_residual)
+{
+    const XStopLast &l = eng().x_stop_last;
+    if (fired) *fired = l.fired;
+    if (norm) *norm = l.norm;
+    if (rz) *rz = l.rz;
+    if (true_residual) *true_residual = l.true_res;
+    return l.fired ? 0 : 1;
+}
 void dkmc_debug_set_x_poly1_degree(int n) { eng().x_poly1_degree = n < 0 ? 0 : (n > 20 ? 20 : n); }
 void dkmc_set_x_poly_auto_rows(int n0, int n1) { Engine &e = eng(); e.x_poly_rows[0] = n0 > 0 ? n0 : 0; e.x_poly_rows[1] = n1 > e.x_poly_rows[0] ? n1 : e.x_poly_rows[0]; }
 void dkmc_set_x_apply_form(int form) { eng().x_apply_form = form == 1 ? 1 : 0; }
diff --git a/devicekmc_amd/csrc/xtb.hip b/devicekmc_amd/csrc/xtb.hip
--- a/devicekmc_amd/csrc/xtb.hip
+++ b/devicekmc_amd/csrc/xtb.hip
@@ -1030,7 +1030,7 @@
 __global__ __launch_bounds__(XT_NT) void k_xtb_step1(int m, int it, const double *__restrict__ mats, double *__restrict__ y0, double *__restrict__ Rt,
                                                      double *__restrict__ Z, double *__restrict__ Pt, double *__restrict__ Pi, const double *__restrict__ Q,
                                                      const double *__restrict__ U, const double *__restrict__ sc, const int *__restrict__ nsrank,
-                                                     double *__restrict__ QS, const XCtrl *ctrl)
+                                                     double *__restrict__ QS, const XCtrl *ctrl, double *__restrict__ npart = nullptr)
 {
     __shared__ int sdone;
     if (threadIdx.x == 0) { const int d = ctrl->done; sdone = d != 0 && it + 1 >= d; }
@@ -1045,6 +1045,7 @@
         cB[kk] = mats[o]; m1B[kk] = mats[256 + o]; m2B[kk] = mats[512 + o]; m3B[kk] = mats[768 + o];
         c0[kk] = mats[(4 * kk + b) * 16];
     }
+    double nacc = 0.0;
     const int ngroups = (m + 15) / 16;
     for (int g = (int)blockIdx.x * 4 + wv; g < ngroups; g += (int)gridDim.x * 4) {
         const int row0 = 16 * g;
@@ -1084,8 +1085,28 @@
                 Rt[o] = rN[u]; Z[o] = zN[u]; Pt[o] = pN[u]; Pi[o] = iN[u];
                 const int sr = nsrank[row];
                 if (sr >= 0) QS[xtb_qs_pos(sr, a)] = sc[row] * pN[u];
+                if (a == 0) nacc += rN[u] * rN[u];
             }
         }
+    }
+    if (npart) {
+        const double t = xtb_tree256(nacc);
+        if (threadIdx.x == 0) npart[blockIdx.x] = t;
+    }
+}
+__global__ __launch_bounds__(256) void k_xtb_stop_norm(int np, int it, const double *__restrict__ part, double bound2, XCtrl *ctrl, double *__restrict__ rec)
+{
+    __shared__ int sdone;
+    if (threadIdx.x == 0) { const int d = ctrl->done; sdone = d != 0 && it + 1 >= d; }
+    __syncthreads();
+    if (sdone) return;
+    double a = 0.0;
+    for (int i = threadIdx.x; i < np; i += 256) a += part[i];
+    a = xtb_tree256(a);
+    if (threadIdx.x == 0) {
+        const bool fire = !(a > bound2) && ctrl->done == 0;
+        rec[0] = a; rec[1] = ctrl->rr[(it + 1) & 1]; rec[2] = fire ? 1.0 : 0.0;
+        if (fire) { ctrl->iters = it + 1; ctrl->done = it + 2; }
     }
 }
 __global__ void k_xtb_init(int m, const double *__restrict__ y, const double *__restrict__ sc, const int *__restrict__ nsrank,
@@ -1202,7 +1223,7 @@
     if (h.pad[0]) return DKMC_XTB_BREAKDOWN;
     return again ? DKMC_XTB_AGAIN : 0;
 }
-static int xtb_cg_body(const XtbArgs &A, int *iters_out, double *rr_out, bool *peer_used, const XbNPack *np, bool f32, XLive *lv);
+static int xtb_cg_body(const XtbArgs &A, int *iters_out, double *rr_out, bool *peer_used, const XbNPack *np, bool f32, XLive *lv, bool first_round);
 static int xtb_cg_slab(const XtbArgs &A, int nr, int me0, const XShare *emu_shares, int time_rank, int *iters_out, double *rr_out);
 template <class Body>
 static int xtb_reenter(int rc, double rr0, int *iters_out, double *rr_out, Body body)
@@ -1242,12 +1263,12 @@
         if (int rcl = xt_live_build(theta, e.x_tile_drop_unit, A.sS, &g_xlive)) return rcl;
         if (g_xlive.state == 1) { lv = &g_xlive; e.x_tile_drop_used = theta; }
     }
-    int rc = xtb_cg_body(A, iters_out, &rr0, &peer_used, np, f32, lv);
-    rc = xtb_reenter(rc, rr0, iters_out, rr_out, [&](int *it, double *rr) { ++e.stats.x_tile_f64_rounds; return xtb_cg_body(A, it, rr, &peer_used, np, false, nullptr); });
+    int rc = xtb_cg_body(A, iters_out, &rr0, &peer_used, np, f32, lv, true);
+    rc = xtb_reenter(rc, rr0, iters_out, rr_out, [&](int *it, double *rr) { ++e.stats.x_tile_f64_rounds; return xtb_cg_body(A, it, rr, &peer_used, np, false, nullptr, false); });
     if (rc != 0 && rc != DKMC_XTB_BREAKDOWN && peer_used) comm_peer_drop();
     return rc;
 }
-static int xtb_cg_body(const XtbArgs &A, int *iters_out, double *rr_out, bool *peer_used, const XbNPack *np, bool f32, XLive *lv)
+static int xtb_cg_body(const XtbArgs &A, int *iters_out, double *rr_out, bool *peer_used, const XbNPack *np, bool f32, XLive *lv, bool first_round)
 {
     Engine &e = eng(); hipStream_t st = e.stream;
     const int m = A.m, s = A.s, so = 4 * ((s + 3) / 4);
@@ -1286,6 +1307,12 @@
     double pc[XB_MAXPOLY1 + 1] = {1.0}, qmin = 1.0;
     if (one) xtb_poly1_coeffs(pn, pc, &qmin); else xtb_poly_coeffs(pd, pc);
     const double tol2_loop = one ? A.tol2 * qmin : (pd > 0 ? A.tol2 / 2.25 : A.tol2);
+    const bool nstop = one && first_round && (e.x_stop_form == 1 || (e.x_stop_form == 2 && xtb_stop_rule(m) != 0));
+    double *npart = nstop ? (double *)scratch(S_XTB_STOPN, (size_t)(2048 + 4) * 8) : nullptr, *nstoprec = npart ? npart + 2048 : nullptr;
+    if (nstop && !npart) return e.err_code;
+    if (nstop) HIPCHK(hipMemsetAsync(nstoprec, 0, 4 * 8, st));
+    const double nbound2 = e.x_stop_margin * e.x_stop_margin * A.tol2;
+    e.x_stop_last = XStopLast{};
     HIPCHK(hipMemsetAsync(QS, 0, (size_t)A.ns_pad * XB_SP * 8, st));
     const bool listf = e.x_fold_form == 1 && pd > 0 && !A.sharded && A.wlist != nullptr && (!lv || lv->wlist != nullptr);
     const int so1 = listf ? 4 : so;
@@ -1370,8 +1397,12 @@
                               (const double *)R, (const double *)Zp, gpart, (const XCtrl *)A.ctrl);
     };
     auto step = [&](int it) {
-        if (one) hipLaunchKernelGGL(k_xtb_step1, dim3(gs), dim3(XT_NT), 0, st, m, it, (const double *)mats, y0, R, Zp, P, Vp, (const double *)T, (const double *)Up, A.sc,
-                                    A.nsrank, QS, (const XCtrl *)A.ctrl);
+        if (one) {
+            const bool nt = nstop && it >= 0;
+            hipLaunchKernelGGL(k_xtb_step1, dim3(gs), dim3(XT_NT), 0, st, m, it, (const double *)mats, y0, R, Zp, P, Vp, (const double *)T, (const double *)Up, A.sc,
+                               A.nsrank, QS, (const XCtrl *)A.ctrl, nt ? npart : (double *)nullptr);
+            if (nt) hipLaunchKernelGGL(k_xtb_stop_norm, dim3(1), dim3(256), 0, st, gs, it, (const double *)npart, nbound2, A.ctrl, nstoprec);
+        }
         else hipLaunchKernelGGL(k_xtb_step, dim3(gs), dim3(XT_NT), 0, st, m, it, (const double *)mats, y0, R, P, (const double *)T, A.sc, A.nsrank, QS, (const XCtrl *)A.ctrl,
                                 (const int *)nullptr, Ypanel);
     };
@@ -1455,9 +1486,11 @@
             const int nrp = std::min(XB_RR_MAXPART, (m + 1023) / 1024);
             hipLaunchKernelGGL(k_xtb_pre_rr_part, dim3(nrp), dim3(256), 0, st, m, (const double *)T, A.b, gpart);
             hipLaunchKernelGGL(k_xtb_pre_rr, dim3(1), dim3(256), 0, st, nrp, (const double *)gpart, bz + m);
-            double rr_true = 0.0;
+            double rr_true = 0.0, hrec[3] = {-1.0, h.rr[h.iters & 1], 0.0};
             HIPCHK(hipMemcpyAsync(&rr_true, bz + m, 8, hipMemcpyDeviceToHost, st));
+            if (nstop && h.iters > 0) HIPCHK(hipMemcpyAsync(hrec, nstoprec, 3 * 8, hipMemcpyDeviceToHost, st));
             HIPCHK(hipStreamSynchronize(st));
+            if (one) e.x_stop_last = XStopLast{hrec[2] != 0.0 ? 2 : 1, nstop ? 1 : 0, m, hrec[0] >= 0.0 ? sqrt(hrec[0]) : -1.0, hrec[1], sqrt(rr_true)};
             h.rr[h.iters & 1] = rr_true;
             again = rr_true > A.tol2;
             if (e.x_tile_f32_fail_once) { e.x_tile_f32_fail_once = 0; again = true; }
@@ -1735,8 +1768,8 @@
     HIPCHK(hipStreamSynchronize(st));
     return e.err_code;
 }
-extern "C" int dkmc_xtb_test_step1(int m, int it, const double *mats, int done_word, double *y0, double *const *panels, const double *sc, const int *nsrank, int ns,
-                                   double *qs)
+static int xtb_test_step1_run(int m, int it, const double *mats, int done_word, double *y0, double *const *panels, const double *sc, const int *nsrank, int ns,
+                              double *qs, double bound2, double rr_in, double *rec3, dkmc_xtb_ctrl *ctrl_out)
 {
     Engine &e = eng(); hipStream_t st = e.stream;
     if (m < 1 || m > XTB_ALG_MAXROWS || it < -1 || it > 0x3fffffff || !mats || !y0 || !panels || !sc || !nsrank || (ns > 0 && !qs))
@@ -1747,13 +1780,16 @@
     const size_t b_qs = xtb_alg_up((size_t)(ns + 2) * XB_SP * 8);
     char *dp = (char *)scratch(S_XTB_ALG_PANELS, 6 * pan_up + 2 * vec_up);
     int *dnsr = (int *)scratch(S_XTB_ALG_INTS, xtb_alg_up((size_t)m * 4));
-    double *dmats = (double *)scratch(S_XTB_ALG_GRAM, 4 * 256 * 8);
+    double *dmats = (double *)scratch(S_XTB_ALG_GRAM, (4 * 256 + 2048 + 4) * 8);
     char *qsb = (char *)scratch(S_XTB_ALG_QS, 2 * b_qs);
     XCtrl *ctrl = (XCtrl *)scratch(S_XTB_ALG_CTRL, sizeof(XCtrl));
     if (!dp || !dnsr || !dmats || !qsb || !ctrl) return e.err_code;
     double *dy0 = (double *)(dp + 6 * pan_up), *dsc = (double *)(dp + 6 * pan_up + vec_up);
     double *QS = (double *)qsb, *dq = (double *)(qsb + b_qs);
-    XCtrl h{}; h.done = done_word;
+    double *dnpart = rec3 ? dmats + 4 * 256 : nullptr, *dnrec = dmats + 4 * 256 + 2048;
+    const int gs1 = grid_blocks((m + 15) / 16, 4, 2048);
+    XCtrl h{}; h.done = done_word; h.rr[0] = h.rr[1] = rr_in;
+    if (rec3) { HIPCHK(hipMemsetAsync(dnpart, 0xff, 2048 * 8, st)); HIPCHK(hipMemcpyAsync(dnrec, rec3, 3 * 8, hipMemcpyHostToDevice, st)); }
     for (int k = 0; k < 6; ++k) HIPCHK(hipMemcpyAsync(dp + k * pan_up, panels[k], pan, hipMemcpyHostToDevice, st));
     HIPCHK(hipMemcpyAsync(dy0, y0, (size_t)m * 8, hipMemcpyHostToDevice, st));
     HIPCHK(hipMemcpyAsync(dsc, sc, (size_t)m * 8, hipMemcpyHostToDevice, st));
@@ -1767,14 +1803,37 @@
     HIPCHK(hipMemcpyAsync(ctrl, &h, sizeof(XCtrl), hipMemcpyHostToDevice, st));
     HIPCHK(hipStreamSynchronize(st));
 #define XB_DP(k_) (double *)(dp + (k_) * pan_up)
-    hipLaunchKernelGGL(k_xtb_step1, dim3(grid_blocks((m + 15) / 16, 4, 2048)), dim3(XT_NT), 0, st, m, it, (const double *)dmats, dy0, XB_DP(4), XB_DP(5), XB_DP(0), XB_DP(1),
-                       (const double *)XB_DP(2), (const double *)XB_DP(3), (const double *)dsc, (const int *)dnsr, QS, (const XCtrl *)ctrl);
+    hipLaunchKernelGGL(k_xtb_step1, dim3(gs1), dim3(XT_NT), 0, st, m, it, (const double *)dmats, dy0, XB_DP(4), XB_DP(5), XB_DP(0), XB_DP(1),
+                       (const double *)XB_DP(2), (const double *)XB_DP(3), (const double *)dsc, (const int *)dnsr, QS, (const XCtrl *)ctrl, dnpart);
 #undef XB_DP
+    if (rec3) hipLaunchKernelGGL(k_xtb_stop_norm, dim3(1), dim3(256), 0, st, gs1, it, (const double *)dnpart, bound2, ctrl, dnrec);
     if (ns > 0) hipLaunchKernelGGL(k_xtb_test_qs_decode, dim3((unsigned)(((size_t)ns * XB_SP + 255) / 256)), dim3(256), 0, st, ns, (const double *)QS, dq);
     KCHK();
     for (int k = 0; k < 6; ++k) if (k != 2 && k != 3) HIPCHK(hipMemcpyAsync(panels[k], dp + k * pan_up, pan, hipMemcpyDeviceToHost, st));
     HIPCHK(hipMemcpyAsync(y0, dy0, (size_t)m * 8, hipMemcpyDeviceToHost, st));
     if (ns > 0) HIPCHK(hipMemcpyAsync(qs, dq, (size_t)ns * XB_SP * 8, hipMemcpyDeviceToHost, st));
+    if (rec3) HIPCHK(hipMemcpyAsync(rec3, dnrec, 3 * 8, hipMemcpyDeviceToHost, st));
+    if (ctrl_out) HIPCHK(hipMemcpyAsync(ctrl_out, ctrl, sizeof(XCtrl), hipMemcpyDeviceToHost, st));
+    HIPCHK(hipStreamSynchronize(st));
+    return e.err_code;
+}
+extern "C" int dkmc_xtb_test_step1(int m, int it, const double *mats, int done_word, double *y0, double *const *panels, const double *sc, const int *nsrank, int ns,
+                                   double *qs)
+{
+    return xtb_test_step1_run(m, it, mats, done_word, y0, panels, sc, nsrank, ns, qs, 0.0, 0.0, nullptr, nullptr);
+}
+extern "C" int dkmc_xtb_test_step1_norm(int m, int it, const double *mats, int done_word, double *y0, double *const *panels, const double *sc, const int *nsrank,
+                                        int ns, double *qs, double bound2, double rr_in, double *rec3, dkmc_xtb_ctrl *ctrl_out)
+{
+    if (!rec3 || !ctrl_out || it < 0) return dkmc_fail(13, "xtb_test_step1_norm: bad arguments", __FILE__, __LINE__);
+    return xtb_test_step1_run(m, it, mats, done_word, y0, panels, sc, nsrank, ns, qs, bound2, rr_in, rec3, ctrl_out);
+}
+extern "C" int dkmc_debug_get_x_stop_rt0(int m, double *rt0)
+{
+    Engine &e = eng(); hipStream_t st = e.stream;
+    const double *R = (const double *)e.buf[S_XTB_PANELS];
+    if (!rt0 || !R || e.x_stop_last.fired == 0 || e.x_stop_last.m != m) return dkmc_fail(13, "get_x_stop_rt0: no one-polynomial round of that size", __FILE__, __LINE__);
+    HIPCHK(hipMemcpy2DAsync(rt0, 8, R, (size_t)XB_SP * 8, 8, (size_t)m, hipMemcpyDeviceToHost, st));
     HIPCHK(hipStreamSynchronize(st));
     return e.err_code;
 }
diff --git a/devicekmc_amd/csrc/xtb_precond.h b/devicekmc_amd/csrc/xtb_precond.h
--- a/devicekmc_amd/csrc/xtb_precond.h
+++ b/devicekmc_amd/csrc/xtb_precond.h
@@ -414,6 +414,9 @@
     return std::min((5 * d + 3) / 4, XB_MAXPOLY1);
 }
 static bool xtb_poly_one(const Engine &e) { return e.x_poly_form == 1 || (e.x_poly_form == 2 && e.x_poly_auto != 0); }
+static const int xb_stop_rows = 96000;
+static int xtb_stop_rule(int m) { return m >= xb_stop_rows ? 1 : 0; }
+extern "C" int dkmc_xtb_stop_rule(int m) { return xtb_stop_rule(m); }
 static const int xb_poly_rows[2] = {225000, 450000};
 static const int xb_poly_steps[3] = {8, 10, 16};
 static int xtb_poly_rule(int m, const int *rows)
diff --git a/devicekmc_amd/lib.py b/devicekmc_amd/lib.py
--- a/devicekmc_amd/lib.py
+++ b/devicekmc_amd/lib.py
@@ -73,6 +73,13 @@
     "dkmc_get_x_poly_form_used": (_I, []),
     "dkmc_get_x_poly_products": (_I, []),
     "dkmc_debug_set_x_poly1_degree": (None, [_I]),
+    "dkmc_set_x_stop_form": (None, [_I]),
+    "dkmc_get_x_stop_form": (_I, []),
+    "dkmc_set_x_stop_margin": (None, [_D]),
+    "dkmc_get_x_stop_margin": (_D, []),
+    "dkmc_get_x_stop_info": (_I, [c_int_p, c_dbl_p, c_dbl_p, c_dbl_p]),
+    "dkmc_debug_get_x_stop_rt0": (_I, [_I, vp]),
+    "dkmc_xtb_stop_rule": (_I, [_I]),
     "dkmc_set_x_tile_f32": (None, [_I]),
     "dkmc_get_x_tile_f32": (_I, []),
     "dkmc_set_x_tile_drop": (None, [_D]),
@@ -247,6 +254,7 @@
     "dkmc_xtb_test_step": (_I, [_I, _I, vp, _I, vp, vp, vp, vp, vp, vp, _I, vp, _I, vp, vp]),
     "dkmc_xtb_test_gram1": (_I, [_I, vp, _I, _I, vp]),
     "dkmc_xtb_test_step1": (_I, [_I, _I, vp, _I, vp, vp, vp, vp, _I, vp]),
+    "dkmc_xtb_test_step1_norm": (_I, [_I, _I, vp, _I, vp, vp, vp, vp, _I, vp, _D, _D, vp, C.POINTER(dkmc_xtb_ctrl)]),
     "dkmc_kcg_emulate_slabs": (_I, [C.POINTER(dkmc_gpubuf), _I, _I, _I, _D, _D, _D, _I, _I, _I, _I, c_dbl_p, c_int_p, c_int_p, c_dbl_p, C.POINTER(C.c_longlong)]),
     "dkmc_xtb_emulate_slabs": (_I, [_I, _I, _D, _I, _I, c_dbl_p, c_int_p, c_int_p, c_dbl_p, C.POINTER(C.c_longlong), c_int_p]),
     "dkmc_xtb_slab_last": (_I, [c_int_p, C.POINTER(C.c_longlong), c_dbl_p]),
diff --git a/include/devicekmc_hip.h b/include/devicekmc_hip.h
--- a/include/devicekmc_hip.h
+++ b/include/devicekmc_hip.h
@@ -94,6 +94,11 @@
 int dkmc_get_x_poly_form(void);
 int dkmc_get_x_poly_form_used(void);
 int dkmc_get_x_poly_products(void);
+void dkmc_set_x_stop_form(int form);
+int dkmc_get_x_stop_form(void);
+void dkmc_set_x_stop_margin(double kappa);
+double dkmc_get_x_stop_margin(void);
+int dkmc_get_x_stop_info(int *fired, double *norm, double *rz, double *true_residual);
 void dkmc_set_x_nmul_form(int form);
 int dkmc_get_x_nmul_form(void);
 void dkmc_set_x_tile_f32(int mode);
diff --git a/include/devicekmc_hip_debug.h b/include/devicekmc_hip_debug.h
--- a/include/devicekmc_hip_debug.h
+++ b/include/devicekmc_hip_debug.h
@@ -27,6 +27,10 @@
 int dkmc_xtb_test_gram1(int m, const double *const *panels, int ng, int done_word, double *gfin);
 int dkmc_xtb_test_step1(int m, int it, const double *mats, int done_word, double *y0, double *const *panels, const double *sc, const int *nsrank, int ns,
                         double *qs);
+int dkmc_xtb_test_step1_norm(int m, int it, const double *mats, int done_word, double *y0, double *const *panels, const double *sc, const int *nsrank, int ns,
+                             double *qs, double bound2, double rr_in, double *rec3, dkmc_xtb_ctrl *ctrl_out);
+int dkmc_debug_get_x_stop_rt0(int m, double *rt0);
+int dkmc_xtb_stop_rule(int m);
 int dkmc_xtb_time_apply(int width, int variant, int reps, double *us);
 int dkmc_xt_tile_census(long long *hist);
 void dkmc_set_x_items(int kc);
```

Result: faster. 6.129, median of 6 (+10.0%).
